# nsp5488/go_raytracer

Measured on AMD Instinct MI355X. Metric: Msamples/sec (pixels×spp/s) + wall-clock, Cornell Box 800×800×1024spp, higher is better.
Workload: dtype f32

## Files before the change

### go_raytracer_amd/__init__.py

```python
import ctypes as C
import weakref

import numpy as np

from . import _lib
from ._lib import (RT_FT_ALL, RT_FT_BOX, RT_NOISE_MARBLE, RT_NOISE_PERLIN,
                   RT_NOISE_TURBULENT, RtAccumInfo, RtAov, RtCamera, RtDenoiseOpts,
                   RtDenoiseVarOpts, RtCameraDerived, RtError, RtRenderOpts, RtSceneInfo, RtStats, RtTreeView,
                   check, lib)

__all__ = ["Tree", "Camera", "Scene", "Accumulator", "quantize", "format_ppm", "device_count", "RtError",
           "tune", "untune", "tuning", "tune_knobs", "tune_from_env",
           "demo_scene", "DEMO_SCENES", "LoadObjOptions", "DefaultLoadOptions", "quantize_device",
           "format_ppm_device", "denoise", "denoise_device", "denoise_var", "denoise_var_device",
           "RtDenoiseVarOpts"]

DEMO_SCENES = ("book1", "book2", "book3", "simple_light", "quads", "cornell", "cornell_smoke",
               "model")


def _d3(v):
    return _lib.D3(*[float(x) for x in v])


# ... 250 lines not shown
        self.MaxDepth = 0
        self.MaxThreads = 0
        self.VerticalFOV = 0.0
        self.DefocusAngle = 0.0
        self.FocusDistance = 0.0
        self.Background = (0.0, 0.0, 0.0)
        self.MaxContribution = 0.0
        self._pos = None
        for k, v in kw.items():
            if k not in self._FIELDS:
                raise AttributeError(k)
            setattr(self, k, v)

    def PositionCamera(self, lookFrom=None, lookAt=None, vup=None):
        self._pos = (tuple(lookFrom) if lookFrom is not None else (0.0, 0.0, 0.0),
                     tuple(lookAt) if lookAt is not None else (0.0, 0.0, -1.0),
                     tuple(vup) if vup is not None else (0.0, 1.0, 0.0))

    def to_c(self):
        c = RtCamera()
        c.aspect_ratio = self.AspectRatio
        c.width = int(self.Width)
        c.samples_per_pixel = int(self.SamplesPerPixel)
        c.max_depth = int(self.MaxDepth)
        c.max_threads = int(self.MaxThreads)
        c.vertical_fov = self.VerticalFOV
        c.defocus_angle = self.DefocusAngle
        c.focus_distance = self.FocusDistance
        c.background = _d3(self.Background)
        c.max_contribution = self.MaxContribution
        if self._pos is not None:
            c.positioned = 1
            c.look_from, c.look_at, c.vup = (_d3(x) for x in self._pos)
        return c

    @classmethod
    def from_c(cls, c):
        cam = cls()
        cam.AspectRatio = c.aspect_ratio
        cam.Width = c.width
        cam.SamplesPerPixel = c.samples_per_pixel
        cam.MaxDepth = c.max_depth
        cam.MaxThreads = c.max_threads
        cam.VerticalFOV = c.vertical_fov
        cam.DefocusAngle = c.defocus_angle
        cam.FocusDistance = c.focus_distance
        cam.Background = tuple(c.background)
        cam.MaxContribution = c.max_contribution
        if c.positioned:
            cam._pos = (tuple(c.look_from), tuple(c.look_at), tuple(c.vup))
        return cam

    def derived(self):
        d = RtCameraDerived()
        c = self.to_c()
        check(lib().rt_camera_derive(C.byref(c), C.byref(d)))
        return d

    def image_size(self):
        d = self.derived()
        return d.width, d.height, d.spp_sqrt

    def Render(self, tree, world, lights, seed=1, device=0):
        with Scene(tree, world, lights) as sc:
            img, _ = sc.render(self, seed=seed, device=device)
        return img


class Scene:

    def __init__(self, tree, world, lights=-1):
        p = C.c_void_p()
        check(lib().rt_scene_create(tree.ptr, world, lights, C.byref(p)))
        self._p = p
        self._destroy = lib().rt_scene_destroy
        self.tree = tree
        self._accums = weakref.WeakSet()

    def close(self):
        if getattr(self, "_p", None):
            for a in list(self._accums):
                a._p = None
            self._destroy(self._p)
            self._p = None

    __del__ = close

    def __enter__(self):
        return self

    def __exit__(self, *a):
        self.close()

    def progress(self):
        d, t = C.c_uint64(0), C.c_uint64(0)
        check(lib().rt_progress(self._p, C.byref(d), C.byref(t)))
        return d.value, t.value

    def info(self):
        i = RtSceneInfo()
        check(lib().rt_scene_info_get(self._p, C.byref(i)))
        return {f: getattr(i, f) for f, _ in RtSceneInfo._fields_}

    def export_bvh(self):
        nn, nr, root = C.c_int32(), C.c_int32(), C.c_uint32()
        check(lib().rt_scene_export_bvh(self._p, None, C.byref(nn), None, C.byref(nr), C.byref(root)))
        nodes = np.zeros((max(nn.value, 0), 16), np.float32)
        refs = np.zeros(max(nr.value, 0), np.uint32)
        check(lib().rt_scene_export_bvh(self._p, nodes.ctypes.data or None, C.byref(nn),
                                        refs.ctypes.data or None, C.byref(nr), C.byref(root)))
        n = C.c_int32()
        check(lib().rt_scene_export_prim_bounds(self._p, None, C.byref(n)))
        bounds = np.zeros((n.value, 6), np.float32)
        check(lib().rt_scene_export_prim_bounds(self._p, bounds.ctypes.data or None, C.byref(n)))
        return nodes, refs, int(root.value), bounds

    def export_bvh8(self):
        nn, nr = C.c_int32(), C.c_int32()
        check(lib().rt_scene_export_bvh8(self._p, None, C.byref(nn), None, C.byref(nr)))
        nodes = np.zeros((max(nn.value, 0), 32), np.uint32)
        refs = np.zeros(max(nr.value, 0), np.uint32)
        check(lib().rt_scene_export_bvh8(self._p, nodes.ctypes.data or None, C.byref(nn),
                                         refs.ctypes.data or None, C.byref(nr)))
        return nodes, refs

    def export_qbvh(self):
        ni, nn, root = C.c_int32(), C.c_int32(), C.c_uint32()
        check(lib().rt_scene_export_qbvh(self._p, None, C.byref(ni), None, C.byref(nn), C.byref(root)))
        items = np.zeros((max(ni.value, 0), 16), np.uint32)
        nodes = np.zeros((max(nn.value, 0), 32), np.uint32)
        check(lib().rt_scene_export_qbvh(self._p, items.ctypes.data or None, C.byref(ni),
                                         nodes.ctypes.data or None, C.byref(nn), C.byref(root)))
        return items, nodes, int(root.value)

    def export_records(self, fill=True):
        ns, sn, nb, counts = C.c_int32(), C.c_int32(), C.c_int32(), (C.c_int32 * 7)()
        check(lib().rt_scene_export_records(self._p, None, C.byref(ns), counts, C.byref(sn), C.byref(nb)))
        pairs = np.zeros((4 * ns.value + sn.value, 4), np.uint32)
        if fill:
            check(lib().rt_scene_export_records(self._p, pairs.ctypes.data or None, C.byref(ns), counts,
                                                C.byref(sn), C.byref(nb)))
        return pairs, ns.value, tuple(counts), sn.value, nb.value

    def lean_light(self):
        k, n = C.c_int32(), C.c_int32()
        check(lib().rt_scene_lean_light(self._p, C.byref(k), None, C.byref(n)))
        block = np.zeros(n.value, np.uint32)
        check(lib().rt_scene_lean_light(self._p, C.byref(k), block.ctypes.data or None, C.byref(n)))
        return k.value, block

    def plan_light(self, device=0):
        k = C.c_int32()
        check(lib().rt_scene_plan_light(self._p, device, C.byref(k)))
        return k.value

    MODES = {"auto": 0, "wavefront": 1, "fused": 2}

    @staticmethod
    def _opts(seed, device, rank, nranks, path_slots, chunk, profile, stream, mode="auto"):
        o = RtRenderOpts()
        o.mode = Scene.MODES[mode]
        o.seed = seed
        o.device = device
        o.rank = rank
        o.nranks = nranks
        o.path_slots = path_slots
        o.chunk = chunk
        o.flags = _lib.RT_FLAG_PROFILE if profile else 0
        o.stream = stream
        return o

    def render(self, camera, seed=1, device=0, rank=0, nranks=1, path_slots=0, chunk=0,
               profile=False, trace=None, mode="auto", progress_slices=0):
        d = camera.derived()
        rows = len(range(rank, d.height, nranks))
        out = np.zeros((rows, d.width, 3), np.float32)
        st = RtStats()
        c = camera.to_c()
        o = self._opts(seed, device, rank, nranks, path_slots, chunk, profile, None, mode)
        o.progress_slices = progress_slices
        tbuf = None
        if trace is not None:
            tbuf = np.zeros((d.max_depth + 1, 12), np.float32)
            o.trace_pixel, o.trace_sample = int(trace[0]), int(trace[1])
            o.trace_cap = tbuf.shape[0]
            o.trace_out = tbuf.ctypes.data
        check(lib().rt_render(self._p, C.byref(c), C.byref(o), out.ctypes.data, C.byref(st)))
        res = {f: getattr(st, f) for f, _ in RtStats._fields_}
        if tbuf is not None:
            res["trace"] = tbuf[tbuf[:, 7] >= 0]
        return out, res

    def render_multi(self, camera, devices, seed=1, path_slots=0, chunk=0, profile=False,
                     mode="auto", rccl=False):
        d = camera.derived()
        out = np.zeros((d.height, d.width, 3), np.float32)
        st = _multi(self, camera, devices, (out.ctypes.data, False), seed, path_slots, chunk,
                    profile, mode, rccl)
        return out, st

    def render_multi_device(self, camera, devices, out_ptr, seed=1, path_slots=0, chunk=0,
                            profile=False, mode="auto", rccl=False):
        return _multi(self, camera, devices, (out_ptr, True), seed, path_slots, chunk, profile,
                      mode, rccl)

    def render_device(self, camera, out_ptr, seed=1, device=0, rank=0, nranks=1, path_slots=0,
                      chunk=0, profile=False, stream=None, mode="auto"):
        st = RtStats()
        c = camera.to_c()
        o = self._opts(seed, device, rank, nranks, path_slots, chunk, profile, stream, mode)
        check(lib().rt_render_device(self._p, C.byref(c), C.byref(o), C.c_void_p(out_ptr),
                                     C.byref(st)))
        return {f: getattr(st, f) for f, _ in RtStats._fields_}

    def render_aov(self, camera, n_samples=1, seed=1, device=0, rank=0, nranks=1):
        d = camera.derived()
        rows = len(range(rank, d.height, nranks))
        res = {"albedo": np.zeros((rows, d.width, 3), np.float32),
               "normal": np.zeros((rows, d.width, 3), np.float32),
               "depth": np.zeros((rows, d.width), np.float32),
               "material": np.full((rows, d.width), -1, np.int32)}
        a = RtAov(*[res[k].ctypes.data for k in ("albedo", "normal", "depth", "material")])
        st = RtStats()
        c = camera.to_c()
        o = self._opts(seed, device, rank, nranks, 0, 0, False, None)
        check(lib().rt_render_aov(self._p, C.byref(c), C.byref(o), n_samples, C.byref(a),
                                  C.byref(st)))
        res["stats"] = {f: getattr(st, f) for f, _ in RtStats._fields_}
        return res

    def render_aov_device(self, camera, albedo=None, normal=None, depth=None, material=None,
                          n_samples=1, seed=1, device=0, rank=0, nranks=1, stream=None):
        a = RtAov(albedo, normal, depth, material)
        st = RtStats()
        c = camera.to_c()
        o = self._opts(seed, device, rank, nranks, 0, 0, False, stream)
        check(lib().rt_render_aov_device(self._p, C.byref(c), C.byref(o), n_samples, C.byref(a),
                                         C.byref(st)))
        return {f: getattr(st, f) for f, _ in RtStats._fields_}

    def accumulator(self, camera, max_passes=0, device=0, rank=0, nranks=1, path_slots=0, chunk=0,
                    profile=False, stream=None, mode="auto", progress_slices=0):
        return Accumulator(self, camera, max_passes, device, rank, nranks, path_slots, chunk,
                           profile, stream, mode, progress_slices)


class Accumulator:

    def __init__(self, scene, camera, max_passes=0, device=0, rank=0, nranks=1, path_slots=0,
                 chunk=0, profile=False, stream=None, mode="auto", progress_slices=0):
        self._p = None
        self._device, self._mean, self._var = device, None, None
        d = camera.derived()
        self.shape = (len(range(rank, d.height, nranks)), d.width)
        c = camera.to_c()
        o = Scene._opts(0, device, rank, nranks, path_slots, chunk, profile, stream, mode)
        o.progress_slices = progress_slices
        p = C.c_void_p()
        check(lib().rt_accum_create(scene._p, C.byref(c), C.byref(o), max_passes, C.byref(p)))
        self._p = p
        self._destroy = lib().rt_accum_destroy
        self.scene = scene
        scene._accums.add(self)

    def close(self):
        if getattr(self, "_p", None):
            self._destroy(self._p)
            self._p = None

    __del__ = close

    def __enter__(self):
        return self

    def __exit__(self, *a):
        self.close()

    def _h(self):
        if not self._p:
            raise ValueError("Accumulator is closed")
        return self._p

    def add(self, seed):
        st = RtStats()
        check(lib().rt_accum_add(self._h(), seed, C.byref(st)))
        return {f: getattr(st, f) for f, _ in RtStats._fields_}

    def resolve(self):
        rgb = np.zeros(self.shape + (3,), np.float32)
        var = np.zeros(self.shape, np.float32)
        check(lib().rt_accum_resolve(self._h(), rgb.ctypes.data, var.ctypes.data))
        return rgb, var

    def resolve_device(self, rgb_tensor, var_tensor=None):
        import torch
        for t, shape in ((rgb_tensor, self.shape + (3,)), (var_tensor, self.shape)):
            if t is not None and (t.dtype != torch.float32 or not t.is_contiguous()
                                  or tuple(t.shape) != shape or not t.is_cuda):
                raise ValueError(f"resolve_device: needs a contiguous float32 device tensor of shape {shape}")
        check(lib().rt_accum_resolve_device(
            self._h(), None if rgb_tensor is None else rgb_tensor.data_ptr(),
            None if var_tensor is None else var_tensor.data_ptr()))

    def denoise_device(self, aov, out=None, var_out=None, **opts):
        import torch
        if self.passes < 2:
# ... 318 lines not shown
```

### go_raytracer_amd/_lib.py

```python
import ctypes as C
import os

_HERE = os.path.dirname(os.path.abspath(__file__))
LIB_PATH = os.environ.get("RT_AMD_LIB") or os.path.join(_HERE, "librt_amd.so")

RT_OK = 0
RT_ERR_INVALID = -1
RT_ERR_UNSUPPORTED = -2
RT_ERR_DEVICE = -3
RT_ERR_OOM = -4
RT_ERR_IO = -5

RT_TEX_SOLID, RT_TEX_CHECKER, RT_TEX_IMAGE, RT_TEX_NOISE = range(4)
RT_NOISE_PERLIN, RT_NOISE_MARBLE, RT_NOISE_TURBULENT = 1, 2, 3
(RT_MAT_LAMBERTIAN, RT_MAT_METAL, RT_MAT_DIELECTRIC, RT_MAT_DIFFUSE_LIGHT,
 RT_MAT_ISOTROPIC) = range(5)
(RT_NODE_LIST, RT_NODE_BVH, RT_NODE_SPHERE, RT_NODE_QUAD, RT_NODE_TRIANGLE,
 RT_NODE_TRANSLATE, RT_NODE_ROTATE_Y, RT_NODE_MEDIUM) = range(8)
RT_FLAG_PROFILE = 1
RT_FLAG_GATHER_RCCL = 2
RT_FT_SPHERE, RT_FT_TRI, RT_FT_METAL, RT_FT_DIEL = 1, 2, 4, 8
RT_FT_MEDIA, RT_FT_CHECKER, RT_FT_IMAGE, RT_FT_NOISE = 16, 32, 64, 128
RT_FT_BOX = 256
RT_FT_ALL = 511
# ... 42 lines not shown
        ("trace_pixel", C.c_int64), ("trace_sample", C.c_int32), ("trace_cap", C.c_int32),
        ("trace_out", C.c_void_p), ("progress_slices", C.c_int32), ("_pad3", C.c_int32),
    ]


class RtStats(C.Structure):
    _fields_ = [
        ("samples", C.c_uint64), ("segments", C.c_uint64),
        ("stack_pushes", C.c_uint64), ("extend_rays", C.c_uint64),
        ("shade_rays", C.c_uint64), ("ms_total", C.c_double),
        ("ms_extend", C.c_double), ("ms_shade", C.c_double),
        ("ms_other", C.c_double), ("n_extend_launches", C.c_int32),
        ("n_shade_launches", C.c_int32), ("iterations", C.c_int32),
        ("rows", C.c_int32), ("mode", C.c_int32), ("path_slots", C.c_int32),
        ("ms_fused", C.c_double),
        ("kernel_features", C.c_int32), ("scene_features", C.c_int32),
        ("tree_width", C.c_int32), ("lds_scene", C.c_int32),
        ("chunk_samples", C.c_int32), ("record_boxes", C.c_int32),
        ("overflow_samples", C.c_uint64),
        ("tuned", C.c_int32), ("chunk_records", C.c_int32),
    ]


class RtAov(C.Structure):
    _fields_ = [("albedo", C.c_void_p), ("normal", C.c_void_p), ("depth", C.c_void_p),
                ("material", C.c_void_p)]


class RtDenoiseOpts(C.Structure):
    _fields_ = [("iterations", C.c_int32), ("demodulate", C.c_int32),
                ("sigma_color", C.c_float), ("sigma_normal", C.c_float),
                ("sigma_depth", C.c_float), ("_pad", C.c_int32)]


class RtDenoiseVarOpts(C.Structure):
    _fields_ = [("iterations", C.c_int32), ("demodulate", C.c_int32),
                ("sigma_lum", C.c_float), ("sigma_normal", C.c_float),
                ("sigma_depth", C.c_float), ("_pad", C.c_int32)]


class RtAccumInfo(C.Structure):
    _fields_ = [("passes", C.c_int32), ("max_passes", C.c_int32),
                ("samples_per_pixel", C.c_uint64), ("nonfinite_pixels", C.c_uint64),
                ("rms_std_error", C.c_double), ("mean_luminance", C.c_double),
                ("rel_error", C.c_double)]


class RtAdaptOpts(C.Structure):
    _fields_ = [("rel_error", C.c_double), ("lum_floor", C.c_double),
                ("tile", C.c_int32), ("min_passes", C.c_int32)]


class RtAdaptInfo(C.Structure):
    _fields_ = [("active_pixels", C.c_uint64), ("total_samples", C.c_uint64),
                ("min_count", C.c_int32), ("max_count", C.c_int32),
                ("n_tiles", C.c_int32), ("active_tiles", C.c_int32)]


class RtTreeView(C.Structure):
    _fields_ = [
        ("nodes", C.c_void_p), ("n_nodes", C.c_int32),
        ("children", C.c_void_p), ("n_children", C.c_int32),
        ("tris", C.c_void_p), ("n_tris", C.c_int32),
        ("materials", C.c_void_p), ("n_materials", C.c_int32),
        ("textures", C.c_void_p), ("n_textures", C.c_int32),
        ("images", C.c_void_p), ("n_images", C.c_int32),
        ("perlins", C.c_void_p), ("n_perlins", C.c_int32),
    ]


class RtObjImage(C.Structure):
    _fields_ = [("name", C.c_char_p), ("rgb", C.c_void_p), ("w", C.c_int32), ("h", C.c_int32)]


class RtObjOptions(C.Structure):
    _fields_ = [
        ("scale_factor", C.c_double), ("flip_yz", C.c_int32), ("debug", C.c_int32),
        ("ignore_normals", C.c_int32), ("center", C.c_int32), ("flip_faces", C.c_int32),
        ("default_material", C.c_int32), ("position", D3), ("ignore_mtl", C.c_int32),
        ("find_windows", C.c_int32), ("n_images", C.c_int32), ("_pad", C.c_int32),
        ("images", C.POINTER(RtObjImage)),
    ]


class RtObjInfo(C.Structure):
    _fields_ = [
        ("n_vertices", C.c_int64), ("n_normals", C.c_int64), ("n_texcoords", C.c_int64),
        ("n_triangles", C.c_int64), ("n_lights", C.c_int64), ("n_materials", C.c_int32),
        ("default_material", C.c_int32), ("bounds_min", D3), ("bounds_max", D3), ("center", D3),
    ]


_P = C.c_void_p
_I = C.c_int
_DP = C.POINTER(C.c_double)

SIGNATURES = {
    "rt_last_error": (C.c_char_p, []),
    "rt_abi_version": (_I, []),
    "rt_tune_set": (_I, [C.c_char_p, C.c_char_p]),
    "rt_tune_get": (_I, [C.c_char_p, C.c_char_p, C.c_int32]),
    "rt_tune_list": (_I, [C.c_int32, C.POINTER(C.c_char_p), C.POINTER(C.c_int32)]),
    "rt_brute_shape": (_I, [C.POINTER(C.c_int32)]),
    "rt_tree_create": (_I, [C.POINTER(_P)]),
    "rt_tree_destroy": (_I, [_P]),
    "rt_tree_seed": (_I, [_P, C.c_uint64]),
    "rt_tree_rand": (C.c_double, [_P]),
    "rt_tree_rand_range": (C.c_double, [_P, C.c_double, C.c_double]),
    "rt_tree_randn": (_I, [_P, _I]),
    "rt_tex_solid": (_I, [_P, C.c_double, C.c_double, C.c_double]),
    "rt_tex_checker": (_I, [_P, C.c_double, _I, _I]),
    "rt_tex_image": (_I, [_P, C.c_void_p, _I, _I]),
    "rt_tex_noise": (_I, [_P, C.c_double, _I]),
    "rt_tex_noise_tables": (_I, [_P, C.c_double, _I, _DP, C.POINTER(C.c_int32)]),
    "rt_mat_lambertian": (_I, [_P, _I]),
    "rt_mat_metal": (_I, [_P, C.c_double, C.c_double, C.c_double, C.c_double]),
    "rt_mat_dielectric": (_I, [_P, C.c_double]),
    "rt_mat_diffuse_light": (_I, [_P, _I]),
    "rt_mat_isotropic": (_I, [_P, _I]),
    "rt_new_list": (_I, [_P]),
    "rt_list_add": (_I, [_P, _I, _I]),
    "rt_build_bvh": (_I, [_P, _I]),
    "rt_new_sphere": (_I, [_P, D3, C.c_double, _I]),
    "rt_new_motion_sphere": (_I, [_P, D3, D3, C.c_double, _I]),
    "rt_new_quad": (_I, [_P, D3, D3, D3, _I]),
    "rt_new_box": (_I, [_P, D3, D3, _I]),
    "rt_new_triangle": (_I, [_P, _DP, _DP, _DP, _I]),
    "rt_new_triangles": (_I, [_P, _I, _DP, _DP, _DP, C.POINTER(C.c_int32)]),
    "rt_translate": (_I, [_P, _I, D3]),
    "rt_rotate_y": (_I, [_P, _I, C.c_double]),
    "rt_constant_medium": (_I, [_P, _I, C.c_double, _I]),
    "rt_obj_default_options": (_I, [C.POINTER(RtObjOptions)]),
    "rt_load_obj": (_I, [_P, C.c_char_p, C.POINTER(RtObjOptions), C.POINTER(_I), C.POINTER(_I),
                         C.POINTER(RtObjInfo)]),
    "rt_load_obj_memory": (_I, [_P, C.c_char_p, C.c_size_t, C.c_char_p, C.c_size_t, C.c_char_p,
                                C.POINTER(RtObjOptions), C.POINTER(_I), C.POINTER(_I),
                                C.POINTER(RtObjInfo)]),
    "rt_tree_get_view": (_I, [_P, C.POINTER(RtTreeView)]),
    "rt_camera_derive": (_I, [C.POINTER(RtCamera), C.POINTER(RtCameraDerived)]),
    "rt_scene_create": (_I, [_P, _I, _I, C.POINTER(_P)]),
    "rt_scene_destroy": (_I, [_P]),
    "rt_scene_info_get": (_I, [_P, C.POINTER(RtSceneInfo)]),
    "rt_scene_export_bvh": (_I, [_P, C.c_void_p, C.POINTER(C.c_int32), C.c_void_p,
                                 C.POINTER(C.c_int32), C.POINTER(C.c_uint32)]),
    "rt_scene_export_bvh8": (_I, [_P, C.c_void_p, C.POINTER(C.c_int32), C.c_void_p,
                                  C.POINTER(C.c_int32)]),
    "rt_scene_export_qbvh": (_I, [_P, C.c_void_p, C.POINTER(C.c_int32), C.c_void_p,
                                  C.POINTER(C.c_int32), C.POINTER(C.c_uint32)]),
    "rt_scene_export_records": (_I, [_P, C.c_void_p, C.POINTER(C.c_int32), C.POINTER(C.c_int32),
                                     C.POINTER(C.c_int32), C.POINTER(C.c_int32)]),
    "rt_scene_export_prim_bounds": (_I, [_P, C.c_void_p, C.POINTER(C.c_int32)]),
    "rt_scene_lean_light": (_I, [_P, C.POINTER(C.c_int32), C.c_void_p, C.POINTER(C.c_int32)]),
    "rt_scene_plan_light": (_I, [_P, _I, C.POINTER(C.c_int32)]),
    "rt_render": (_I, [_P, C.POINTER(RtCamera), C.POINTER(RtRenderOpts), C.c_void_p,
                       C.POINTER(RtStats)]),
    "rt_render_device": (_I, [_P, C.POINTER(RtCamera), C.POINTER(RtRenderOpts), C.c_void_p,
                              C.POINTER(RtStats)]),
    "rt_render_multi": (_I, [_P, C.POINTER(RtCamera), C.POINTER(RtRenderOpts),
                             C.POINTER(C.c_int32), C.c_int32, C.c_void_p, C.POINTER(RtStats)]),
    "rt_render_multi_device": (_I, [_P, C.POINTER(RtCamera), C.POINTER(RtRenderOpts),
                                    C.POINTER(C.c_int32), C.c_int32, C.c_void_p,
                                    C.POINTER(RtStats)]),
    "rt_quantize": (_I, [C.c_void_p, C.c_int64, C.c_void_p]),
    "rt_format_ppm": (C.c_int64, [C.c_void_p, _I, _I, C.c_void_p, C.c_int64]),
    "rt_progress": (_I, [_P, C.POINTER(C.c_uint64), C.POINTER(C.c_uint64)]),
    "rt_quantize_device": (_I, [C.c_void_p, C.c_int64, C.c_void_p, _I, C.c_void_p]),
    "rt_format_ppm_device": (C.c_int64, [C.c_void_p, _I, _I, C.c_void_p, C.c_int64, _I,
                                         C.c_void_p]),
    "rt_render_aov": (_I, [_P, C.POINTER(RtCamera), C.POINTER(RtRenderOpts), C.c_int32,
                           C.POINTER(RtAov), C.POINTER(RtStats)]),
    "rt_render_aov_device": (_I, [_P, C.POINTER(RtCamera), C.POINTER(RtRenderOpts), C.c_int32,
                                  C.POINTER(RtAov), C.POINTER(RtStats)]),
    "rt_denoise": (_I, [C.c_void_p, C.POINTER(RtAov), _I, _I, C.POINTER(RtDenoiseOpts),
                        C.c_void_p]),
    "rt_denoise_device": (_I, [C.c_void_p, C.POINTER(RtAov), _I, _I, C.POINTER(RtDenoiseOpts),
                               C.c_void_p, _I, C.c_void_p]),
    "rt_denoise_var": (_I, [C.c_void_p, C.c_void_p, C.POINTER(RtAov), _I, _I,
                            C.POINTER(RtDenoiseVarOpts), C.c_void_p, C.c_void_p]),
    "rt_denoise_var_device": (_I, [C.c_void_p, C.c_void_p, C.POINTER(RtAov), _I, _I,
                                   C.POINTER(RtDenoiseVarOpts), C.c_void_p, C.c_void_p, _I,
                                   C.c_void_p]),
    "rt_accum_create": (_I, [_P, C.POINTER(RtCamera), C.POINTER(RtRenderOpts), C.c_int32,
                             C.POINTER(_P)]),
    "rt_accum_destroy": (_I, [_P]),
    "rt_accum_reset": (_I, [_P]),
    "rt_accum_add": (_I, [_P, C.c_uint64, C.POINTER(RtStats)]),
    "rt_accum_resolve": (_I, [_P, C.c_void_p, C.c_void_p]),
    "rt_accum_resolve_device": (_I, [_P, C.c_void_p, C.c_void_p]),
    "rt_accum_info_get": (_I, [_P, C.POINTER(RtAccumInfo)]),
    "rt_accum_select": (_I, [_P, C.POINTER(RtAdaptOpts), C.POINTER(C.c_uint64)]),
    "rt_accum_set_active": (_I, [_P, C.c_void_p, C.POINTER(C.c_uint64)]),
    "rt_accum_add_active": (_I, [_P, C.c_uint64, C.POINTER(RtStats)]),
    "rt_accum_counts": (_I, [_P, C.c_void_p]),
    "rt_accum_counts_device": (_I, [_P, C.c_void_p]),
    "rt_accum_tile_error": (_I, [_P, C.POINTER(RtAdaptOpts), C.c_void_p, C.POINTER(C.c_int32),
                                C.POINTER(C.c_int32)]),
    "rt_accum_adapt_info": (_I, [_P, C.POINTER(RtAdaptInfo)]),
    "rt_demo_scene": (_I, [_P, C.c_char_p, C.c_char_p, C.POINTER(RtCamera), C.POINTER(_I),
                           C.POINTER(_I)]),
    "rt_demo_scene_name": (_I, [_I, C.POINTER(C.c_char_p)]),
    "rt_substitute_mesh_obj": (C.c_int64, [_I, _I, C.c_void_p, C.c_int64]),
    "rt_device_count": (_I, []),
}

_lib = None


def lib():
    global _lib
    if _lib is None:
        if not os.path.exists(LIB_PATH):
            raise OSError(f"{LIB_PATH} not built: run `make -C go_raytracer_amd/csrc` "
                          "or __graft_entry__.build()")
        L = C.CDLL(LIB_PATH)
        for name, (res, args) in SIGNATURES.items():
            if os.environ.get("RT_AMD_LIB") and not hasattr(L, name):
                continue
            f = getattr(L, name)
            f.restype = res
            f.argtypes = args
        _lib = L
    return _lib


class RtError(RuntimeError):
    def __init__(self, code, msg):
        super().__init__(f"rt error {code}: {msg}")
        self.code = code


def check(rc):
    if rc < 0:
        raise RtError(rc, lib().rt_last_error().decode(errors="replace"))
    return rc
```

### go_raytracer_amd/csrc/host_records.cpp

```cpp
#include <math.h>
#include <string.h>

#include <algorithm>

#include "rt_internal.h"

namespace rt {

void build_leaf_records(const HostScene& h, std::vector<F4>& recs) {
  recs.assign(4 * h.refs.size(), F4{0, 0, 0, 0});
  for (size_t i = 0; i < h.refs.size(); ++i) make_record(h, h.refs[i], &recs[4 * i]);
}
void build_light_records(const HostScene& h, std::vector<F4>& recs) {
  recs.assign(8 * std::max<size_t>(h.lights.size(), 1), F4{0, 0, 0, 0});
  for (size_t i = 0; i < h.lights.size(); ++i) {
    const uint32_t ref = h.lights[i].ref;
    if (ref == PRIM_NONE || (ref >> 30) != PRIM_QUAD) continue;
    make_record(h, ref, &recs[8 * i]);
    const F4* q = &h.quad[5 * (size_t)(ref & 0x3FFFFFFFu)];
    recs[8 * i + 2].w = q[1].w;
    recs[8 * i + 4] = q[0];
    recs[8 * i + 5] = q[1];
    recs[8 * i + 6] = q[2];
  }
// ... 161 lines not shown
          for (size_t m : quads)
            if (m != i && m != j && !in_box[m] && same_face(m, F, tol)) {
              bool dup = false;
              for (int g = 0; g < f; ++g) dup |= b.face[g] == m;
              if (!dup) { hit = m; break; }
            }
        if (hit == (size_t)-1) ok = false;
        else b.face[f] = hit;
      }
      if (!ok) continue;
      for (int c = 0; c < 3; ++c) b.C[c] = C[c], b.ax[c] = ax[c], b.az[c] = az[c];
      b.H = H;
      for (int f = 0; f < 6; ++f) in_box[b.face[f]] = 1;
      boxes.push_back(b);
      break;
    }
  }
  return boxes;
}

struct Groups {
  std::vector<size_t> grp[7];
  std::vector<std::pair<int, size_t>> odd_ax;
};
Groups group_records(const Records& R, const std::vector<size_t>& ord, const std::vector<char>& in_box) {
  Groups g;
  auto& grp = g.grp;
  auto& odd_ax = g.odd_ax;
  for (size_t i : ord) {
    if (in_box[i]) continue;
    const int a = R.axis_of(i);
    const int v = a < 0 ? R.vert_of(i) : -1;
    grp[a >= 0 ? a : v >= 0 ? 4 + v : 3].push_back(i);
  }
  for (int a : {0, 1, 2, 4, 5, 6})
    if (grp[a].size() & 1) {
      if (a < 3 && tune_int("RT_BRUTE_MIXED", 1) != 0) odd_ax.push_back({a, grp[a].back()});
      else grp[3].push_back(grp[a].back());
      grp[a].pop_back();
    }
  if (odd_ax.size() == 3) {
    grp[3].push_back(odd_ax.back().second);
    odd_ax.pop_back();
  }
  if (odd_ax.size() == 1) {
    grp[3].push_back(odd_ax.back().second);
    odd_ax.clear();
  }
  std::stable_sort(grp[3].begin(), grp[3].end(), [&](size_t a, size_t b) { return R.larger(a, b); });
  return g;
}

struct SlotOrder {
  std::vector<long> slots;
  size_t n_general = 0;
  size_t n_loop = 0;
  size_t nbp = 0;
  size_t face0 = 0;
};
SlotOrder order_slots(const Groups& g, const std::vector<BoxRec>& boxes, BruteCounts& bc) {
  SlotOrder so;
  auto& slots = so.slots;
  for (size_t i : g.grp[3]) slots.push_back((long)i);
  if (slots.size() & 1) slots.push_back(-1);
  bc.ng = (int32_t)(slots.size() / 2);
  for (int a = 0; a < 3; ++a)
    for (size_t i : g.grp[4 + a]) slots.push_back((long)i);
  bc.vy = (int32_t)(g.grp[5].size() / 2);
  so.n_general = slots.size();
  for (int a = 0; a < 3; ++a) {
    for (size_t i : g.grp[a]) slots.push_back((long)i);
    bc.ax[a] = (int32_t)(g.grp[a].size() / 2);
  }
  bc.mx = 0;
  if (g.odd_ax.size() == 2) {
    slots.push_back((long)g.odd_ax[0].second);
    slots.push_back((long)g.odd_ax[1].second);
    bc.mx = (g.odd_ax[0].first + 1) | ((g.odd_ax[1].first + 1) << 2);
  }
  so.n_loop = slots.size();
  so.nbp = (boxes.size() + 1) / 2;
  bc.box = (int32_t)so.nbp;
  slots.insert(slots.end(), 2 * so.nbp, -2);
  so.face0 = slots.size();
  for (const BoxRec& b : boxes)
    for (int f = 0; f < 6; ++f) slots.push_back((long)b.face[f]);
  if (slots.empty()) {
    slots.assign(2, -1);
    bc.ng = 1;
  }
  return so;
}

std::vector<F4> interleave_pairs(const Records& R, const SlotOrder& so, const std::vector<BoxRec>& boxes) {
  const auto& slots = so.slots;
  std::vector<F4> pairs(4 * slots.size(), F4{0, 0, 0, 0});
  for (size_t k = 0; k < 2 * so.nbp; ++k) {
    const BoxRec& b = boxes[std::min(k, boxes.size() - 1)];
    float* f = (float*)&pairs[4 * (so.n_loop + k - (k & 1))] + (k & 1);
    const double a2 = b.ax[0] * b.ax[0] + b.ax[2] * b.ax[2], z2 = b.az[0] * b.az[0] + b.az[2] * b.az[2];
    const double y0 = b.C[1], y1 = b.C[1] + b.H;
    const float v[8] = {(float)b.C[0], (float)b.C[2], (float)(b.ax[0] / a2), (float)(b.ax[2] / a2),
                        (float)(b.az[0] / z2), (float)(b.az[2] / z2), (float)std::min(y0, y1),
                        (float)std::max(y0, y1)};
    for (int e = 0; e < 8; ++e) f[2 * e] = v[e];
    for (int fc = 0; fc < 6; ++fc) {
      const int src = (fc >> 1) == 1 && b.H < 0 ? (fc ^ 1) : fc;
      const uint32_t slot = (uint32_t)(so.face0 + 6 * std::min(k, boxes.size() - 1) + src);
      memcpy(&f[2 * (8 + fc)], &slot, 4);
    }
  }
  for (size_t i = 0; i < slots.size(); ++i) {
    if (slots[i] < 0) continue;
    const F4* r = &R.recs[4 * (size_t)slots[i]];
    float* f = (float*)&pairs[8 * (i / 2)] + (i & 1);
    float kb;
    const uint32_t k = (uint32_t)i;
    memcpy(&kb, &k, 4);
    const int a = i >= so.n_general && i < so.n_loop ? R.axis_of((size_t)slots[i]) : -1;
    const float na = a == 0 ? r[1].x : a == 1 ? r[1].y : r[1].z;
    const float Dp = a < 0 ? r[1].w : na * r[1].w;
    const float v[15] = {r[1].x, r[1].y, r[1].z, Dp,     r[0].x, r[0].y, r[0].z, r[2].x,
                         r[2].y, r[2].z, r[3].x, r[3].y, r[3].z, kb,     r[0].w};
    for (int e = 0; e < 15; ++e) f[2 * e] = v[e];
  }
  return pairs;
}

std::vector<F4> shade_table(const HostScene& h) {
  const size_t nq = h.quad.size() / 5;
  std::vector<F4> tab(2 * nq);
  bool ok = nq > 0;
  for (size_t qi = 0; qi < nq && ok; ++qi) {
    const F4* q = &h.quad[5 * qi];
    uint32_t mb;
    memcpy(&mb, &q[2].w, 4);
    ok = mb < h.mats.size();
    if (!ok) break;
    const DevMaterial& m = h.mats[mb];
    ok = (m.kind == RT_MAT_LAMBERTIAN || m.kind == RT_MAT_DIFFUSE_LIGHT) && m.tex >= 0 &&
         (size_t)m.tex < h.texs.size() && h.texs[m.tex].kind == RT_TEX_SOLID;
    if (!ok) break;
    float kb;
    const uint32_t kind = (uint32_t)m.kind;
    memcpy(&kb, &kind, 4);
    tab[2 * qi] = {q[3].x, q[3].y, q[3].z, kb};
    const F4 col = h.texs[m.tex].color;
    tab[2 * qi + 1] = {col.x, col.y, col.z, q[0].w};
  }
  if (!ok || tune_int("RT_SHADE_LDS", 1) == 0) tab.clear();
  return tab;
}

}

RecordPack pack_records(const HostScene& h) {
  RecordPack out;
  if (!tiny_scene(h)) return out;
  Records R{h, {}, tune_int("RT_BRUTE_AXIS", 1) != 0, tune_int("RT_BRUTE_VERT", 1) != 0};
  build_leaf_records(h, R.recs);
  std::vector<size_t> ord(h.refs.size());
  for (size_t i = 0; i < ord.size(); ++i) ord[i] = i;
  std::stable_sort(ord.begin(), ord.end(), [&](size_t a, size_t b) { return R.larger(a, b); });
  std::vector<char> in_box(h.refs.size(), 0);
  const std::vector<BoxRec> boxes = find_boxes(h, ord, in_box);
  const Groups groups = group_records(R, ord, in_box);
  const SlotOrder so = order_slots(groups, boxes, out.counts);
  out.pairs = interleave_pairs(R, so, boxes);
  out.n_slots = so.slots.size();
  out.n_boxes = (int32_t)boxes.size();
  out.shape = brute_shape_of(out.counts);
  const std::vector<F4> tab = shade_table(h);
  out.shade_n = (int32_t)tab.size();
  out.pairs.insert(out.pairs.end(), tab.begin(), tab.end());
  return out;
}

int32_t scene_merge_ok(const HostScene& h) {
  for (const auto& t : h.texs)
    if (t.kind == RT_TEX_SOLID && !(t.color.x >= 0.0f && t.color.y >= 0.0f && t.color.z >= 0.0f))
      return 0;
  for (const auto& m : h.mats)
    if (m.kind == RT_MAT_METAL && !(m.albedo.x >= 0.0f && m.albedo.y >= 0.0f && m.albedo.z >= 0.0f))
      return 0;
  return 1;
}
float scene_pdf_floor(const HostScene& h) {
  if (h.lights.empty()) return 0.0f;
  for (const auto& e : h.lights)
    if (e.ref == PRIM_NONE) return 0.0f;
  return 1e-30f;
}

int lean_light_of(const HostScene& h, LeanLight* block) {
  if (block) *block = LeanLight{};
  if (pick_ft_set(h.features) != 0u || h.lights.size() != 1) return 0;
  const DevLight& e = h.lights[0];
  if (e.ref == PRIM_NONE || (e.ref >> 30) != PRIM_QUAD || e.weight != 1.0f) return 0;
  if (scene_merge_ok(h) != 1 || scene_pdf_floor(h) != 1e-30f) return 0;
  std::vector<F4> lr;
  build_light_records(h, lr);
  const float n[3] = {lr[1].x, lr[1].y, lr[1].z}, Q[3] = {lr[0].x, lr[0].y, lr[0].z},
              A[3] = {lr[2].x, lr[2].y, lr[2].z}, B[3] = {lr[3].x, lr[3].y, lr[3].z};
  for (int kind = 1; kind < kLeanLightCount; ++kind) {
    const int a = lean_light_axis(kind);
    if (a < 0) continue;
    const int b = (a + 1) % 3, c = (a + 2) % 3;
    if (!((n[a] == 1.0f || n[a] == -1.0f) && n[b] == 0.0f && n[c] == 0.0f && A[a] == 0.0f &&
          B[a] == 0.0f))
      continue;
    if (block) {
      const float f[kLeanLightFloats] = {
          Q[0],    Q[1],    Q[2],    n[a] * lr[1].w, A[0],    A[1],    A[2],    lr[2].w, B[0],    B[1],
          B[2],    0.0f,    lr[5].x, lr[5].y,        lr[5].z, 0.0f,    lr[6].x, lr[6].y, lr[6].z, 0.0f};
      memcpy(block->f, f, sizeof f);
    }
    return kind;
  }
  return 0;
}

}
```

### go_raytracer_amd/csrc/host_tune.cpp

```cpp
#include <errno.h>
#include <stdlib.h>
#include <string.h>

#include <algorithm>
#include <map>
#include <mutex>
#include <string>

#include "rt_internal.h"

namespace rt {
namespace {

struct Knob {
  const char* name;
  bool bits;
  char kind;
  double lo, hi;
};
constexpr double kBig = 1e30;
constexpr Knob kKnobs[] = {
    {"RT_BOX_LEAVES", true, 'i', 0, 1},
    {"RT_BIG_SPHERE_R", true, 'f', 0, kBig},
    {"RT_BVH_BUILDER", false, 's', 0, 0},
    {"RT_BVH_DEVICE_MIN", false, 'f', 0, kBig},
    {"RT_BVH8", false, 'i', 0, 1},
    {"RT_BVH_LEAF", false, 'i', 1, 64},
    {"RT_BVH_CT", false, 'f', 1e-06, 1000000.0},
    {"RT_BVH_CI", false, 'f', 1e-06, 1000000.0},
    {"RT_BVH_TOP", false, 'i', 1, 1073741824},
    {"RT_THREADS", false, 'i', 1, 1024},
    {"RT_FEATURES_ALL", true, 'i', 0, 1},
    {"RT_BRUTE_MAX", true, 'i', 0, 1048576},
    {"RT_BRUTE_AXIS", false, 'i', 0, 1},
    {"RT_BRUTE_VERT", false, 'i', 0, 1},
    {"RT_BRUTE_BOX", true, 'i', 0, 1},
    {"RT_BRUTE_MIXED", false, 'i', 0, 1},
    {"RT_SHADE_LDS", false, 'i', 0, 1},
    {"RT_TREE", true, 'i', -1, 4},
    {"RT_BRUTE_SMEM", false, 'i', -1, 1},
    {"RT_BRUTE_SHAPE", false, 'i', 0, 1},
    {"RT_LEAN_LIGHT", false, 'i', 0, 1},
    {"RT_QBVH", false, 'i', 0, 1},
    {"RT_CHUNK_NEED", false, 'i', 1, 1048576},
    {"RT_TAIL_FRAC", false, 'i', -1, 1024},
    {"RT_TAIL_K", false, 'i', 1, 4096},
    {"RT_CSUM", false, 'i', 0, 1},
    {"RT_CSUM_MAX_MB", false, 'i', 0, 16777216},
    {"RT_CHUNK_ROWS", false, 'i', -1, 1073741824},
    {"RT_SWEEP", false, 's', 0, 0},
    {"RT_STEP_BUDGET", false, 'i', 1, 1073741824},
    {"RT_SHADE_MIN", false, 'i', 1, 64},
    {"RT_GRAB_MIN", false, 'i', 1, 1048576},
    {"RT_SPLIT_MIN", false, 'i', 0, 1048576},
    {"RT_PARTS_LOG2", false, 'i', 0, 6},
    {"RT_GRAN_LOG2", false, 'i', 0, 20},
    {"RT_WAVE_TIMES", false, 's', 0, 0},
    {"RT_TIMING", false, 'i', 0, 1},
};

std::mutex g_mu;
std::map<std::string, std::string> g_set;

const Knob* find_knob(const char* name) {
  for (const Knob& k : kKnobs)
    if (strcmp(k.name, name) == 0) return &k;
  return nullptr;
}

}

bool tune_str(const char* name, std::string* out) {
  std::lock_guard<std::mutex> lk(g_mu);
  auto it = g_set.find(name);
  if (it == g_set.end()) return false;
  if (out) *out = it->second;
  return true;
}

double tune_num(const char* name, double dflt) {
  std::string v;
  if (!tune_str(name, &v) || v.empty()) return dflt;
  return atof(v.c_str());
}

int tune_int(const char* name, int dflt) {
  std::string v;
  if (!tune_str(name, &v) || v.empty()) return dflt;
  return atoi(v.c_str());
}

int32_t tune_count() {
  std::lock_guard<std::mutex> lk(g_mu);
  return (int32_t)g_set.size();
}

}

extern "C" {

int rt_tune_set(const char* name, const char* value) {
  if (!name) {
    std::lock_guard<std::mutex> lk(rt::g_mu);
    rt::g_set.clear();
    return RT_OK;
  }
  const rt::Knob* k = rt::find_knob(name);
  if (!k) return rt::set_error(RT_ERR_INVALID, "rt_tune_set: unknown knob %s", name);
  if (value && k->kind != 's') {
    char* end = nullptr;
    errno = 0;
    const double v = k->kind == 'i' ? (double)strtoll(value, &end, 10) : strtod(value, &end);
    if (end == value || *end != '\0' || errno == ERANGE || !(v >= k->lo && v <= k->hi))
      return rt::set_error(RT_ERR_INVALID, "rt_tune_set: %s=\"%s\" is not a number in [%g, %g]",
                           name, value, k->lo, k->hi);
  }
  if (value && strcmp(name, "RT_BVH_BUILDER") == 0 && strcmp(value, "host") != 0 &&
      strcmp(value, "device") != 0 && strcmp(value, "auto") != 0 && value[0] != '\0')
    return rt::set_error(RT_ERR_INVALID, "rt_tune_set: RT_BVH_BUILDER=\"%s\" (host | device | auto)",
                         value);
  if (value && strcmp(name, "RT_SWEEP") == 0 && strcmp(value, "forward") != 0 &&
      strcmp(value, "reverse") != 0 && value[0] != '\0')
    return rt::set_error(RT_ERR_INVALID, "rt_tune_set: RT_SWEEP=\"%s\" (forward | reverse)", value);
  std::lock_guard<std::mutex> lk(rt::g_mu);
  if (value) rt::g_set[name] = value;
  else rt::g_set.erase(name);
  return RT_OK;
}

int rt_tune_get(const char* name, char* buf, int32_t cap) {
  if (!name || !rt::find_knob(name)) return rt::set_error(RT_ERR_INVALID, "rt_tune_get: unknown knob %s", name ? name : "(null)");
  std::string v;
  if (!rt::tune_str(name, &v)) return 0;
  if (buf && cap > 0) {
    const size_t n = std::min<size_t>(v.size(), (size_t)cap - 1);
    memcpy(buf, v.data(), n);
    buf[n] = '\0';
  }
  return (int)v.size() + 1;
}

int rt_brute_shape(const int32_t counts[7]) {
  if (!counts) return rt::set_error(RT_ERR_INVALID, "rt_brute_shape: counts is NULL");
  const rt::BruteCounts c = {counts[0], counts[1], {counts[2], counts[3], counts[4]}, counts[5], counts[6]};
  return rt::brute_shape_of(c);
}

int rt_scene_lean_light(const rt_scene* sc, int32_t* kind, float* block, int32_t* n_floats) {
  if (!sc) return rt::set_error(RT_ERR_INVALID, "rt_scene_lean_light: null");
  rt::LeanLight b;
  const int k = rt::lean_light_of(sc->s.h, &b);
  if (kind) *kind = k;
  if (n_floats) *n_floats = rt::kLeanLightFloats;
  if (block) memcpy(block, b.f, sizeof b.f);
  return RT_OK;
}

int rt_tune_list(int32_t i, const char** name, int32_t* changes_bits) {
  const int32_t n = (int32_t)(sizeof(rt::kKnobs) / sizeof(rt::kKnobs[0]));
  if (i < 0) return n;
  if (i >= n) return rt::set_error(RT_ERR_INVALID, "rt_tune_list: index %d of %d", i, n);
  if (name) *name = rt::kKnobs[i].name;
  if (changes_bits) *changes_bits = rt::kKnobs[i].bits ? 1 : 0;
  return n;
}

}
```

### go_raytracer_amd/csrc/rt_fused.h

```cpp
#pragma once
#include "rt_path.h"

namespace rt {

RT_D bool stage_nodes(const Params& P, F4* lnodes, int W) {
  const int nl = min(P.sc.n_nodes, 4 * kLdsNodes / W);
  for (int i = threadIdx.x; i < W * nl; i += blockDim.x) lnodes[i] = P.sc.nodes[i];
  const bool recs = P.recs_lds != 0u;
  if (recs) {
    const int n = 4 * P.sc.n_refs + (P.sc.shade_lds >= 0 ? P.sc.shade_n : 0);
    for (int i = threadIdx.x; i < n; i += blockDim.x) lnodes[W * nl + i] = P.sc.leafprims[i];
  }
  __syncthreads();
  return recs;
}

RT_D void record_trace(const Params& P, const Path& s, const Hit& best) {
  if (s.gpix == P.trace_gpix && s.s0 + s.j == P.trace_sample && (int)s.k < P.trace_cap) {
    P.trace[3 * s.k + 0] = {s.o.x, s.o.y, s.o.z, s.time};
    P.trace[3 * s.k + 1] = {s.d.x, s.d.y, s.d.z, (float)s.k};
    P.trace[3 * s.k + 2] = {best.t, best.u, best.v, bitsf(best.ref)};
  }
}

template <uint32_t FT>
RT_D void finish_hit(const Params& P, const Path& s, Hit& best) {
#ifndef RT_NO_TRI_REFINE
  if (HAS(FT_TRI) && best.ref != PRIM_NONE && (best.ref >> 30) == PRIM_TRI)
    refine_tri_hit(P.sc, best.ref & 0x3FFFFFFFu, s.o, s.d, best.t, best.u, best.v);
#endif
#ifdef RT_SPHERE32_LEAVES
  if (HAS(FT_SPHERE) && best.ref != PRIM_NONE && (best.ref >> 30) == PRIM_SPHERE && best.v >= 0.0f)
    refine_sphere_hit(P.sc, best.ref & 0x3FFFFFFFu, s.o, s.d, s.time, best.t);
#endif
#ifdef ABL_NO_MEDIA
  if (false)
#else
  if (HAS(FT_MEDIA) && P.sc.n_media > 0)
#endif
    trace_media(P, s.o, s.d, s.time, 0.001f, s.gpix, s.s0 + s.j, s.k, s.spare, best);
  if (P.trace) record_trace(P, s, best);
}

#ifndef MESH_WAVES
#define MESH_WAVES 4
#endif
#ifndef TRI_WAVES
#define TRI_WAVES 4
#endif
#ifndef TRI_QWAVES
#define TRI_QWAVES 5
#endif
#ifdef RT_QTOP
#ifndef TRI_QSHORT
#define TRI_QSHORT 12
#endif
#ifndef MESH_QSHORT
#define MESH_QSHORT 12
#endif
#endif
#ifndef TRI_QSHORT
#define TRI_QSHORT 13
#endif
#ifndef MESH_QWAVES
#define MESH_QWAVES 5
#endif
#ifndef MESH_QSHORT
#define MESH_QSHORT 13
#endif
#ifndef FT_TEX_WAVES
#define FT_TEX_WAVES 4
#endif
#ifndef BRUTE_WAVES
#define BRUTE_WAVES 6
#endif
constexpr int kBruteWaves = BRUTE_WAVES;
constexpr int fused_waves(uint32_t ft, int tree = 4) {
  return (tree == 0 && ft == 0u) ? kBruteWaves
         : ft == 0u ? 6
         : ft == FT_MEDIA ? 4
         : ft == (FT_SPHERE | FT_TRI | FT_METAL) ? (tree == 5 ? TRI_QWAVES : TRI_WAVES)
         : ft == (FT_SPHERE | FT_TRI | FT_METAL | FT_DIEL | FT_CHECKER) ? (tree == 5 ? MESH_QWAVES : MESH_WAVES)
         : ft == FT_SET_BOOK2 ? FT_TEX_WAVES
                                                                                  : 3;
}
#ifndef MESH_WLDS
#define MESH_WLDS 4
#endif
#ifndef MESH_SHORT
#define MESH_SHORT 16
#endif
#ifndef TRI_SHORT
#define TRI_SHORT MESH_SHORT
#endif
#ifndef TRI_WLDS
#define TRI_WLDS MESH_WLDS
#endif
#ifndef TEX_SHORT
#define TEX_SHORT 10
#endif
#ifndef TEX_WLDS
#define TEX_WLDS 5
#endif
#ifndef ALL_WLDS
#define ALL_WLDS 4
#endif
#ifndef BRUTE_WLDS
#define BRUTE_WLDS kLdsWMax
#endif
constexpr int fused_wlds(uint32_t ft, int tree = 4) {
  return ft == (FT_SPHERE | FT_TRI | FT_METAL | FT_DIEL | FT_CHECKER) ? MESH_WLDS
         : ft == (FT_SPHERE | FT_TRI | FT_METAL)                    ? TRI_WLDS
         : (ft == 0u && tree != 0)                                  ? 4
         : (ft == 0u && tree == 0)                                  ? BRUTE_WLDS
         : ft == FT_ALL                                             ? ALL_WLDS
         : ft == FT_SET_BOOK2 ? TEX_WLDS
                                                                    : kLdsWMax;
}
constexpr int fused_short(uint32_t ft, int tree = 4) {
  return tree == 0                                                    ? 0
         : ft == 0u                                                   ? kShortStackMin
         : ft == (FT_SPHERE | FT_TRI | FT_METAL | FT_DIEL | FT_CHECKER) ? (tree == 5 ? MESH_QSHORT : MESH_SHORT)
         : ft == (FT_SPHERE | FT_TRI | FT_METAL)                      ? (tree == 5 ? TRI_QSHORT : TRI_SHORT)
         : ft == FT_SET_BOOK2 ? TEX_SHORT
                                                                      : kShortStack;
}
constexpr unsigned fused_static_lds(uint32_t ft, int tree = 4) {
  return (unsigned)(fused_short(ft, tree) * 4 + fused_wlds(ft, tree) * 12 + 24) * 256u +
         ((ft & FT_NOISE) ? 256u * 16u + 768u : 0u);
}
__shared__ unsigned long long g_tstart[4];
#ifdef RT_DRAIN_TIMES
__shared__ unsigned long long g_tdrain[4];
__shared__ unsigned long long g_dinfo[4][3];
#endif
template <bool LDS, uint32_t FT, int TREE, int SHAPE = 0, int LIGHT = 0, bool MAP = false>
__global__ __launch_bounds__(256, fused_waves(FT, TREE)) void k_fused(Params P) {
  static_assert(SHAPE == 0 || (LDS && FT == 0u && TREE == 0), "shapes: the lean LDS record loop only");
  static_assert(LIGHT == 0 || (LDS && FT == 0u && TREE == 0), "light kinds: the lean LDS record loop only");
  static_assert(LIGHT >= 0 && LIGHT < kLeanLightCount, "light kinds: unlisted kind");
  extern __shared__ F4 lnodes[];
  __shared__ uint32_t lstack[(fused_short(FT, TREE) > 0 ? fused_short(FT, TREE) : 1) * 256];
  __shared__ float lw[3 * fused_wlds(FT, TREE) * 256];
  __shared__ unsigned long long lacc[3 * 256];
  for (int ch = 0; ch < 3; ++ch) lacc[ch * 256 + threadIdx.x] = 0ull;
  if constexpr (HAS(FT_NOISE)) stage_perlin(P.sc);
  if constexpr (cam_mode(FT) == 1) stage_camera(P);
  const bool recs_lds = LDS && TREE != 8 && stage_nodes(P, lnodes, TREE == 4 ? 8 : 4);
#ifdef RT_QTOP
  if constexpr (TREE == 5) {
    const uint32_t nq = 4u * (uint32_t)min(RT_QTOP, P.sc.n_nodes);
    for (uint32_t i = threadIdx.x; i < nq; i += blockDim.x) st_lds(&lnodes[i], ld_glb(P.sc.nodes + i));
  }
#endif
  if (!LDS) __syncthreads();
  const uint32_t slot = blockIdx.x * blockDim.x + threadIdx.x;
  const TravStack ts = {&lstack[threadIdx.x], P.ostack + slot, P.stack_cols, fused_short(FT, TREE)
#ifdef RT_COUNT_TRAV_OVF
                        , &P.ctr->pushes
#endif
  };
  const WStack ws = {&lw[threadIdx.x], fused_wlds(FT, TREE)};
  const SampleAcc sa = {&lacc[threadIdx.x]};
  Path s;
  s.pushes = 0;
  if constexpr ((FT == 0u && TREE == 0) || kSplitTrees) {
    s.chunk = s.j = 0u;
    s.flags = 0u;
  }
#ifdef RT_WAVE_SEGS
  uint32_t wave_segs = 0;
#else
  s.segs = 0;
#endif
  Trav tr;
  tr.cur = TRAV_DONE;
  bool has = false;
  WaveBatch b = batch_init(P);
  const uint32_t wave_in_group = (FT == 0u && TREE == 0) ? __builtin_amdgcn_readfirstlane(threadIdx.x >> 6)
                                                         : threadIdx.x >> 6;
  if (P.wave_times && lane_id() == 0u) g_tstart[wave_in_group] = wall_clock64();
#ifdef RT_DRAIN_TIMES
  if (lane_id() == 0u) g_tdrain[wave_in_group] = 0ull;
#endif
#ifdef RT_PHASES
  if (threadIdx.x < 4 * PH_N) (&g_ph[0][0])[threadIdx.x] = 0ull;
  __syncthreads();
#endif
  PH_T(t_loop);
  for (;;) {
    PH_T(t_grab);
    uint32_t c = grab_chunk(P, b, !has), j0 = 0u, n0 = 0u;
    constexpr bool kSplit = (FT == 0u && TREE == 0) || kSplitTrees;
    if constexpr (kSplit)
      if (b.part >= (uint32_t)kMaxParts) split_samples(P, s, has, c, j0, n0);
    if (c != 0xFFFFFFFFu) {
      start_sample<false, cam_mode(FT), FT == 0u && TREE == 0, MAP>(P, slot, s, c, j0);
      if constexpr (kSplit)
        if (j0) s.flags = F_SPLIT | (n0 << kCountShift);
      trav_init<FT>(P.sc, s.o, s.d, s.time, tr);
#ifdef RT_QROOT
      if constexpr (TREE == 5) trav_root_q(ts, s.o, 0.001f, tr);
#endif
      has = true;
    }
    PH_ADD(PH_GRAB, t_grab);
#ifdef RT_DRAIN_TIMES
    if (b.part >= (uint32_t)kMaxParts && __builtin_amdgcn_readfirstlane((uint32_t)(g_tdrain[wave_in_group] != 0ull)) == 0u) {
      uint32_t rem = has ? (s.flags >> kCountShift) - s.j : 0u, act = has ? 1u : 0u;
#ifndef RT_WAVE_SEGS
      uint32_t sg = s.segs;
#else
      uint32_t sg = 0u;
#endif
      for (int off = 32; off > 0; off >>= 1) {
        rem += __shfl_xor(rem, off);
        act += __shfl_xor(act, off);
        sg += __shfl_xor(sg, off);
      }
      if (lane_id() == 0u) {
        g_tdrain[wave_in_group] = wall_clock64();
        g_dinfo[wave_in_group][0] = rem;
        g_dinfo[wave_in_group][1] = act;
        g_dinfo[wave_in_group][2] = sg;
      }
    }
#endif
    if (!__any(has)) break;
    PH_T(t_trav);
    if (has && tr.cur != TRAV_DONE)
    {
      PH_CNT(PH_TRAV_LANES, __popcll(__ballot(1)));
      PH_CNT(PH_TRAV_ROUNDS, 1);
      if constexpr (TREE == 0)
        trav_brute<FT, !LDS, SHAPE>(P.sc, lnodes, s.o, s.d, s.time, 0.001f, tr);
      else if constexpr (TREE == 8)
      {
        const int nsteps = trav_steps8<FT>(P.sc, ts, s.o, s.d, s.time, 0.001f, tr, P.step_budget);
#ifdef RT_PHASES
        ph_steps(nsteps);
#endif
        (void)nsteps;
      }
      else
      {
        const int nsteps = trav_steps<LDS, FT, TREE == 4 || TREE == 5, TREE == 5>(
            P.sc, lnodes, recs_lds, ts, s.o, s.d, s.time, 0.001f, tr, P.step_budget);
        retest_near<FT>(P.sc, s.o, s.d, 0.001f, tr);
#ifdef RT_PHASES
        ph_steps(nsteps);
#endif
        (void)nsteps;
      }
    }
    PH_ADD(PH_TRAV, t_trav);
    const bool ready = has && tr.cur == TRAV_DONE;
    const uint32_t n_ready = (uint32_t)__popcll(__ballot(ready));
    const bool busy = __any(has && !ready);
    if (n_ready >= P.shade_min || !busy) {
#ifdef RT_WAVE_SEGS
      wave_segs += n_ready;
#endif

      if (ready) {
        PH_CNT(PH_SHADE_LANES, n_ready);
        PH_CNT(PH_SHADE_ROUNDS, 1);
        PH_T(t_media);
        Hit best = tr.best;
        finish_hit<FT>(P, s, best);
        PH_ADD(PH_MEDIA, t_media);
#ifndef RT_WAVE_SEGS
        ++s.segs;
#endif
        PH_T(t_shade);
        if (shade_core<false, FT, LIGHT>(P, slot, s, best, ws, sa) == OUT_NEED_CHUNK) has = false;
        else {
          trav_init<FT>(P.sc, s.o, s.d, s.time, tr);
#ifdef RT_QROOT
          if constexpr (TREE == 5) trav_root_q(ts, s.o, 0.001f, tr);
#endif
        }
        PH_ADD(PH_SHADE, t_shade);
      }
    }
  }
  PH_ADD(PH_LOOP, t_loop);
#ifdef RT_WAVE_SEGS
  const uint32_t segs = wave_segs;
#else
  uint32_t segs = s.segs;
  for (int off = 32; off > 0; off >>= 1) segs += __shfl_xor(segs, off);
#endif
  uint32_t pushes = s.pushes;
  for (int off = 32; off > 0; off >>= 1) pushes += __shfl_xor(pushes, off);
  if (lane_id() == 0) {
    atomicAdd(&P.ctr->segments, (unsigned long long)segs);
    atomicAdd(&P.ctr->pushes, (unsigned long long)pushes);
    if (P.wave_times) {
      const size_t w = (size_t)blockIdx.x * 4 + wave_in_group;
      unsigned long long* rec = P.wave_times + kWaveRec * w;
      rec[0] = g_tstart[wave_in_group];
      rec[1] = wall_clock64();
      rec[2] = segs;
#ifdef RT_DRAIN_TIMES
      rec[3] = g_tdrain[wave_in_group];
#else
      rec[3] = 0ull;
#endif
#ifdef RT_PHASES
      for (int i = 0; i < PH_N; ++i) rec[4 + i] = g_ph[wave_in_group][i];
#else
      for (int i = 0; i < PH_N; ++i) rec[4 + i] = 0ull;
#ifdef RT_DRAIN_TIMES
      for (int i = 0; i < 3; ++i) rec[4 + i] = g_dinfo[wave_in_group][i];
#endif
#endif
    }
  }
}

#define RT_FUSED_ILP_KERNELS(X)                                             \
  X(true, (FT_SPHERE | FT_TRI | FT_METAL), 4)                               \
  X(false, (FT_SPHERE | FT_TRI | FT_METAL), 4)                              \
  X(true, (FT_SPHERE | FT_TRI | FT_METAL | FT_DIEL | FT_CHECKER), 4)        \
  X(false, (FT_SPHERE | FT_TRI | FT_METAL | FT_DIEL | FT_CHECKER), 4)

#define RT_FUSED_MAP_KERNELS(X)                                                      \
  X(true, kFtSets[0], 0) X(false, kFtSets[0], 0) X(true, kFtSets[1], 0) X(false, kFtSets[1], 0) \
  X(true, kFtSets[0], 4) X(false, kFtSets[0], 4) X(true, kFtSets[1], 4) X(false, kFtSets[1], 4) \
  X(true, kFtSets[2], 4) X(false, kFtSets[2], 4) X(true, kFtSets[3], 4) X(false, kFtSets[3], 4) \
  X(true, kFtSets[4], 4) X(false, kFtSets[4], 4) X(true, FT_ALL, 4) X(false, FT_ALL, 4)         \
  X(false, kFtSets[2], 5) X(false, kFtSets[3], 5) X(false, kFtSets[4], 5) X(false, FT_ALL, 5)

}
```

### go_raytracer_amd/csrc/rt_internal.h

```cpp
#pragma once
#include <stdint.h>

#include <atomic>
#include <map>
#include <memory>
#include <mutex>
#include <string>
#include <vector>

#include "rt_abi.h"
#include "rt_device.h"

namespace rt {

int set_error(int code, const char* fmt, ...);

bool tune_str(const char* name, std::string* out);
double tune_num(const char* name, double dflt);
int tune_int(const char* name, int dflt);
int32_t tune_count();

struct Tree {
  std::vector<rt_node> nodes;
  std::vector<std::vector<int32_t>> lists;
  std::vector<rt_tri> tris;
  std::vector<rt_material> materials;
  std::vector<rt_texture> textures;
  std::vector<std::vector<uint8_t>> image_data;
  std::vector<rt_image> images;
  std::vector<rt_perlin> perlins;
  uint64_t rng = 0x853c49e6748fea9bull;

  bool dirty = true;
  std::vector<rt_node> v_nodes;
  std::vector<int32_t> v_children;

  double rand01();
  int randn(int n);
  void pack();
};

constexpr double kBigSphereR = 256.0;
struct HostScene {
  std::vector<F4> sph_cr, sph_mv;
  std::vector<F2> sph_uv;
  std::vector<F4> quad;
  std::vector<F4> tri;
  std::vector<F4> tri_attr;
  std::vector<F4> box_recs;
  std::vector<F4> nodes;
  std::vector<F4> nodes4;
  uint32_t root4 = PRIM_NONE;
  std::vector<F4> nodes8;
  std::vector<uint32_t> refs8;
  std::vector<uint32_t> refs;
  uint32_t root = PRIM_NONE;
  std::vector<float> prim_bounds;
  std::vector<DevMedium> media;
  std::vector<uint32_t> medium_refs;
  std::vector<uint32_t> big_refs;
  int32_t medium_draws = 0;
  std::vector<DevLight> lights;
  std::vector<DevMaterial> mats;
  std::vector<DevTexture> texs;
  std::vector<uint8_t> texels;
  std::vector<DevImage> images;
  std::vector<DevPerlin> perlins;
  int32_t n_world_prims = 0;
  int32_t bvh_depth = 0;
  int32_t max_leaf = 0;
  int32_t bvh_builder = 0;
  uint32_t features = 0;
  bool noise_table0 = true;
  int32_t tuned = 0;
};

struct DeviceScene;
struct RenderState;

struct Progress {
  std::mutex mu;
  int busy = 0;
  int device = -1;
  uint64_t total = 0;
  uint64_t done = 0;
  std::vector<void*> events;
  std::vector<uint64_t> cum;
};

struct SlotState {
  std::mutex mu;
  RenderState* st = nullptr;
};

struct DeviceSlot {
  std::mutex mu;
  DeviceScene* ds = nullptr;
};

struct Scene {
  HostScene h;
  std::mutex mu;
  std::map<int, DeviceSlot*> devs;
  std::map<std::pair<int, int>, SlotState*> slots;
  std::mutex multi_mu;
  void* multi_buf = nullptr;
  size_t multi_bytes = 0;
  int multi_dev = -1;
  void* rccl = nullptr;
  Progress prog;
  std::vector<rt_accum*> accums;
  std::mutex qb_mu;
  bool qb_built = false;
  std::vector<F4> qb;
  size_t qb_items = 0;
};

int flatten_scene(const Tree& t, int world, int lights, HostScene& out);
int build_bvh(HostScene& s, const std::vector<F4>& lo, const std::vector<F4>& hi,
              const std::vector<uint32_t>& prims);
constexpr size_t kBvh8MinRefs = 1024;
int build_bvh8(HostScene& s);
int build_qbvh(const HostScene& s, const std::vector<F4>& recs, std::vector<F4>* out,
               size_t* n_items);
void make_record(const HostScene& h, uint32_t ref, F4* r);
void build_leaf_records(const HostScene& h, std::vector<F4>& recs);
void build_light_records(const HostScene& h, std::vector<F4>& recs);
std::vector<DevMaterial> materials_with_uv_flag(const HostScene& h);
bool tiny_scene(const HostScene& h);
struct RecordPack {
  std::vector<F4> pairs;
  size_t n_slots = 0;
  int32_t shade_n = 0;
  int32_t n_boxes = 0;
  BruteCounts counts{};
  int shape = 0;
};
RecordPack pack_records(const HostScene& h);
int32_t scene_merge_ok(const HostScene& h);
float scene_pdf_floor(const HostScene& h);
int lean_light_of(const HostScene& h, LeanLight* block);
int build_bvh_device(HostScene& s, const std::vector<F4>& lo, const std::vector<F4>& hi,
                     const std::vector<uint32_t>& prims, int device);
bool bvh_device_available();
constexpr size_t kBoxLeafMinPrims = 256;
uint32_t scene_features(const HostScene& h, bool* noise_table0 = nullptr);
void release_device(Scene* s);
void release_accums(Scene* s);
struct AovView {
  DevScene sc;
  int tree;
};
int aov_view(Scene* s, int device, AovView* out);

}

struct rt_tree {
  rt::Tree t;
};
struct rt_scene {
  rt::Scene s;
};
```

### go_raytracer_amd/csrc/rt_path.h

```cpp
#pragma once
#include "rt_kernels.h"

namespace rt {

constexpr int kLdsNodes = 384;
constexpr int kLdsWMax = 6;
constexpr int kStack = 64;
constexpr int kShortStack = 12;
constexpr int kShortStackMin = 6;
constexpr int kMaxIt = 1 << 16;
constexpr int kXcd = 8;
constexpr int kMaxParts = 64;
constexpr int kPartStride = 64;

enum : uint32_t { F_PEND = 1u, F_PRE = 2u, F_NONFINITE = 4u };
constexpr uint32_t kCountShift = 8;
constexpr uint32_t F_SPLIT = 0x80u;

#ifdef RT_NO_SPLIT_TREES
constexpr bool kSplitTrees = false;
#else
constexpr bool kSplitTrees = true;
#endif
enum { OUT_DEAD = 0, OUT_ALIVE = 1, OUT_NEED_CHUNK = 2 };
// ... 890 lines not shown
  }
}
template <int I> RT_D v2f pair_q(const v4f* r) { return I == 0 ? r[2].xy : I == 1 ? r[2].zw : r[3].xy; }
template <int I> RT_D v2f pair_a(const v4f* r) { return I == 0 ? r[3].zw : I == 1 ? r[4].xy : r[4].zw; }
template <int I> RT_D v2f pair_b(const v4f* r) { return I == 0 ? r[5].xy : I == 1 ? r[5].zw : r[6].xy; }
template <int AX, bool SMEM>
RT_D void brute_axis(const DevScene& sc, const F4* lrec, int p0, int p1, const v2f* O,
                     const v2f* Dv, float tmin, float& best, uint32_t& bk) {
  constexpr int B0 = AX == 0 ? 1 : 0, B1 = AX == 2 ? 1 : 2;
  const float da = Dv[AX].x;
  const float ia = bitsf(pick_by(fbits(rcp(da)), 0x7FC00000u, neg_mask(fabsf(da) - 1e-8f)));
  const v2f inv = {ia, ia};
  for (int p = p0; p < p1; ++p) {
    v4f r[7];
    load_pair<SMEM>(sc, lrec, p, r);
    const uint32_t k0 = __float_as_uint(r[6].z), k1 = __float_as_uint(r[6].w);
    const v2f t = (r[1].zw - O[AX]) * inv;
    const v2f pb = pfma(Dv[B0], t, O[B0]) - pair_q<B0>(r);
    const v2f pc = pfma(Dv[B1], t, O[B1]) - pair_q<B1>(r);
    const v2f a = pfma(pc, pair_a<B1>(r), pb * pair_a<B0>(r));
    const v2f b = pfma(pc, pair_b<B1>(r), pb * pair_b<B0>(r));
    const uint32_t m0 = rec_reject_t(t.x, tmin, best, a.x, b.x);
    best = bitsf(pick_by(fbits(t.x), fbits(best), m0));
    bk = pick_by(k0, bk, m0);
    const uint32_t m1 = rec_reject_t(t.y, tmin, best, a.y, b.y);
    best = bitsf(pick_by(fbits(t.y), fbits(best), m1));
    bk = pick_by(k1, bk, m1);
  }
}
template <int I> RT_D float comp(f3 v) { return I == 0 ? v.x : I == 1 ? v.y : v.z; }
template <int A, int H>
RT_D void brute_half(const v4f* r, f3 o, f3 d, float tmin, float& best, uint32_t& bk) {
  constexpr int B0 = A == 0 ? 1 : 0, B1 = A == 2 ? 1 : 2;
  const float da = comp<A>(d);
  const float ia = bitsf(pick_by(fbits(rcp(da)), 0x7FC00000u, neg_mask(fabsf(da) - 1e-8f)));
  const float t = ((H ? r[1].w : r[1].z) - comp<A>(o)) * ia;
  const float pb = fmaf(comp<B0>(d), t, comp<B0>(o)) - (H ? pair_q<B0>(r).y : pair_q<B0>(r).x);
  const float pc = fmaf(comp<B1>(d), t, comp<B1>(o)) - (H ? pair_q<B1>(r).y : pair_q<B1>(r).x);
  const float a = fmaf(pc, H ? pair_a<B1>(r).y : pair_a<B1>(r).x, pb * (H ? pair_a<B0>(r).y : pair_a<B0>(r).x));
  const float b = fmaf(pc, H ? pair_b<B1>(r).y : pair_b<B1>(r).x, pb * (H ? pair_b<B0>(r).y : pair_b<B0>(r).x));
  const uint32_t m = rec_reject_t(t, tmin, best, a, b);
  best = bitsf(pick_by(fbits(t), fbits(best), m));
  bk = pick_by(__float_as_uint(H ? r[6].w : r[6].z), bk, m);
}
template <int A0, int A1, bool SMEM>
RT_D void brute_mixed(const DevScene& sc, const F4* lrec, int p, f3 o, f3 d, float tmin,
                      float& best, uint32_t& bk) {
  v4f r[7];
  load_pair<SMEM>(sc, lrec, p, r);
  brute_half<A0, 0>(r, o, d, tmin, best, bk);
  brute_half<A1, 1>(r, o, d, tmin, best, bk);
}
template <int I> RT_D v2f pair_n(const v4f* r) { return I == 0 ? r[0].xy : I == 1 ? r[0].zw : r[1].xy; }
template <int AX, bool SMEM>
RT_D void brute_vert(const DevScene& sc, const F4* lrec, int p0, int p1, const v2f* O,
                     const v2f* Dv, float tmin, float& best, uint32_t& bk) {
  constexpr int B0 = AX == 0 ? 1 : 0, B1 = AX == 2 ? 1 : 2;
  for (int p = p0; p < p1; ++p) {
    v4f r[7];
    load_pair<SMEM>(sc, lrec, p, r);
    const uint32_t k0 = __float_as_uint(r[6].z), k1 = __float_as_uint(r[6].w);
    const v2f D = r[1].zw;
    const v2f den = pfma(pair_n<B1>(r), Dv[B1], pair_n<B0>(r) * Dv[B0]);
    const v2f num = D - pfma(pair_n<B1>(r), O[B1], pair_n<B0>(r) * O[B0]);
    const v2f t = num * v2f{rcp(den.x), rcp(den.y)};
    const v2f pa = pfma(Dv[AX], t, O[AX]) - pair_q<AX>(r);
    const v2f p0v = pfma(Dv[B0], t, O[B0]) - pair_q<B0>(r);
    const v2f p1v = pfma(Dv[B1], t, O[B1]) - pair_q<B1>(r);
    const v2f a = pfma(p1v, pair_a<B1>(r), p0v * pair_a<B0>(r));
    const v2f b = pa * pair_b<AX>(r);
    const uint32_t m0 = rec_reject(den.x, t.x, tmin, best, a.x, b.x);
    best = bitsf(pick_by(fbits(t.x), fbits(best), m0));
    bk = pick_by(k0, bk, m0);
    const uint32_t m1 = rec_reject(den.y, t.y, tmin, best, a.y, b.y);
    best = bitsf(pick_by(fbits(t.y), fbits(best), m1));
    bk = pick_by(k1, bk, m1);
  }
}
constexpr uint32_t kBoxCode = 0x40000000u;
template <bool SMEM>
RT_D void brute_box(const DevScene& sc, const F4* lrec, int p0, int p1, const v2f* O,
                    const v2f* Dv, float iy1, float tmin, float& best, uint32_t& bk) {
  const v2f iy = {iy1, iy1};
  for (int p = p0; p < p1; ++p) {
    v4f r[4];
    if (SMEM) {
      typedef __attribute__((address_space(4))) const v4f cst_v4;
      const cst_v4* q = (const cst_v4*)sc.leafprims + 8 * __builtin_amdgcn_readfirstlane(p);
#pragma unroll
      for (int e = 0; e < 4; ++e) r[e] = q[e];
    } else {
      const lds_v4* q = (const lds_v4*)lrec + 8 * p;
#pragma unroll
      for (int e = 0; e < 4; ++e) r[e] = q[e];
    }
    const v2f ex = O[0] - r[0].xy, ez = O[2] - r[0].zw;
    const v2f lx = pfma(ez, r[1].zw, ex * r[1].xy), lz = pfma(ez, r[2].zw, ex * r[2].xy);
    const v2f vx = pfma(Dv[2], r[1].zw, Dv[0] * r[1].xy), vz = pfma(Dv[2], r[2].zw, Dv[0] * r[2].xy);
    const v2f ix = {rcp(vx.x), rcp(vx.y)}, iz = {rcp(vz.x), rcp(vz.y)};
    const v2f tx0 = -lx * ix, tx1 = pfma(-lx, ix, ix);
    const v2f tz0 = -lz * iz, tz1 = pfma(-lz, iz, iz);
    const v2f ty0 = (r[3].xy - O[1]) * iy, ty1 = (r[3].zw - O[1]) * iy;
#pragma unroll
    for (int h = 0; h < 2; ++h) {
      const float ax0 = h ? tx0.y : tx0.x, ax1 = h ? tx1.y : tx1.x;
      const float ay0 = h ? ty0.y : ty0.x, ay1 = h ? ty1.y : ty1.x;
      const float az0 = h ? tz0.y : tz0.x, az1 = h ? tz1.y : tz1.x;
      const float tn = fmaxf(fmaxf(fminf(ax0, ax1), fminf(ay0, ay1)), fminf(az0, az1));
      const float tf = fminf(fminf(fmaxf(ax0, ax1), fmaxf(ay0, ay1)), fmaxf(az0, az1));
      const uint32_t leave = neg_mask(tn - tmin);
      const float t = bitsf(pick_by(fbits(tn), fbits(tf), leave));
      const uint32_t rej = (uint32_t)((int32_t)__builtin_amdgcn_bitop3_b32(
                               fbits(tf - tn), fbits(t - tmin), fbits(best - t), 0xFE) >> 31);
      best = bitsf(pick_by(fbits(t), fbits(best), rej));
      bk = pick_by(kBoxCode | ((uint32_t)p << 2) | ((uint32_t)h << 1) | (leave & 1u), bk, rej);
    }
  }
}
template <bool SMEM>
RT_D uint32_t box_face(const DevScene& sc, const F4* lrec, uint32_t code, f3 o, f3 d, float iy,
                       float best) {
  const uint32_t base = 32u * ((code & ~kBoxCode) >> 2) + ((code >> 1) & 1u);
  float f[8];
  if (SMEM) {
    const float* g = (const float*)sc.leafprims + base;
#pragma unroll
    for (int e = 0; e < 8; ++e) f[e] = *(const __attribute__((address_space(1))) float*)(g + 2 * e);
  } else {
    const lds_f32* l = (const lds_f32*)lrec + base;
#pragma unroll
    for (int e = 0; e < 8; ++e) f[e] = l[2 * e];
  }
  const float ex = o.x - f[0], ez = o.z - f[1];
  const float lx = fmaf(ez, f[3], ex * f[2]), lz = fmaf(ez, f[5], ex * f[4]);
  const float ix = rcp(fmaf(d.z, f[3], d.x * f[2])), iz = rcp(fmaf(d.z, f[5], d.x * f[4]));
  const float t[6] = {-lx * ix, fmaf(-lx, ix, ix), (f[6] - o.y) * iy, (f[7] - o.y) * iy,
                      -lz * iz, fmaf(-lz, iz, iz)};
  const uint32_t flip = (code & 1u) ? 0xFFFFFFFFu : 0u;
  uint32_t slot = 0u;
  float err = kInf;
#pragma unroll
  for (int a = 0; a < 3; ++a) {
    const uint32_t m = neg_mask(t[2 * a + 1] - t[2 * a]) ^ flip;
    const float e = fminf(fabsf(bitsf(pick_by(fbits(t[2 * a]), fbits(t[2 * a + 1]), m)) - best), kInf);
    const uint32_t nearer = neg_mask(e - err);
    slot = pick_by(slot, 2u * (uint32_t)a + (m & 1u), nearer);
    err = bitsf(pick_by(fbits(err), fbits(e), nearer));
  }
  if (SMEM)
    return *(const __attribute__((address_space(1))) uint32_t*)((const float*)sc.leafprims + base +
                                                                 2 * (8 + slot));
  return ((const lds_u32*)lrec)[base + 2 * (8 + slot)];
}
template <uint32_t FT, bool SMEM, int SHAPE = 0>
RT_D void trav_brute(const DevScene& sc, const F4* lrec, f3 o, f3 d, float time, float tmin,
                     Trav& tr) {
  static_assert(!HAS(FT_SPHERE | FT_TRI), "record loop: quad-only feature sets");
  static_assert(SHAPE >= 0 && SHAPE < kBruteShapeCount, "record loop: unlisted shape");
  const cst_params* kp = SHAPE == 0 ? kparams() : nullptr;
  BruteCounts bc = brute_shape(SHAPE);
  if constexpr (SHAPE == 0) {
    bc.ax[0] = kp->sc.brute_ax[0], bc.ax[1] = kp->sc.brute_ax[1], bc.ax[2] = kp->sc.brute_ax[2];
    bc.vy = kp->sc.brute_vt[1];
    bc.ng = kp->sc.brute_ng;
  }
  const int nax = bc.ax[0], nay = bc.ax[1], naz = bc.ax[2];
  const int nvy = bc.vy;
  const int ng = bc.ng;
  const v2f ox = {o.x, o.x}, oy = {o.y, o.y}, oz = {o.z, o.z};
  const v2f dx = {d.x, d.x}, dy = {d.y, d.y}, dz = {d.z, d.z};
  float best = tr.best.t;
  uint32_t bk = 0xFFFFFFFFu;
  for (int p = 0; p < ng; ++p) {
    v4f r[7];
    load_pair<SMEM>(sc, lrec, p, r);
    const uint32_t k0 = __float_as_uint(r[6].z), k1 = __float_as_uint(r[6].w);
    const v2f nx = r[0].xy, ny = r[0].zw, nz = r[1].xy, D = r[1].zw;
    const v2f den = pfma(nz, dz, pfma(ny, dy, nx * dx));
    const v2f num = D - pfma(nz, oz, pfma(ny, oy, nx * ox));
    const v2f t = num * v2f{rcp(den.x), rcp(den.y)};
    const v2f px = pfma(dx, t, ox) - r[2].xy;
    const v2f py = pfma(dy, t, oy) - r[2].zw;
    const v2f pz = pfma(dz, t, oz) - r[3].xy;
    const v2f a = pfma(pz, r[4].zw, pfma(py, r[4].xy, px * r[3].zw));
    const v2f b = pfma(pz, r[6].xy, pfma(py, r[5].zw, px * r[5].xy));
    const uint32_t m0 = rec_reject(den.x, t.x, tmin, best, a.x, b.x);
    best = bitsf(pick_by(fbits(t.x), fbits(best), m0));
    bk = pick_by(k0, bk, m0);
    const uint32_t m1 = rec_reject(den.y, t.y, tmin, best, a.y, b.y);
    best = bitsf(pick_by(fbits(t.y), fbits(best), m1));
    bk = pick_by(k1, bk, m1);
  }
  const v2f O[3] = {ox, oy, oz}, Dv[3] = {dx, dy, dz};
  const int q = ng + nvy;
  brute_vert<1, SMEM>(sc, lrec, ng, q, O, Dv, tmin, best, bk);
  brute_axis<0, SMEM>(sc, lrec, q, q + nax, O, Dv, tmin, best, bk);
  brute_axis<1, SMEM>(sc, lrec, q + nax, q + nax + nay, O, Dv, tmin, best, bk);
  brute_axis<2, SMEM>(sc, lrec, q + nax + nay, q + nax + nay + naz, O, Dv, tmin, best, bk);
  const int qm = q + nax + nay + naz, mx = SHAPE == 0 ? kp->sc.brute_mx : bc.mx;
  if (mx == (1 | (2 << 2))) brute_mixed<0, 1, SMEM>(sc, lrec, qm, o, d, tmin, best, bk);
  else if (mx == (1 | (3 << 2))) brute_mixed<0, 2, SMEM>(sc, lrec, qm, o, d, tmin, best, bk);
  else if (mx == (2 | (3 << 2))) brute_mixed<1, 2, SMEM>(sc, lrec, qm, o, d, tmin, best, bk);
  const int qb = qm + (mx != 0 ? 1 : 0);
  const float iy = rcp(d.y);
  brute_box<SMEM>(sc, lrec, qb, qb + (SHAPE == 0 ? kp->sc.brute_box : bc.box), O, Dv, iy, tmin, best, bk);
  if (bk != 0xFFFFFFFFu) {
    if (bk & kBoxCode) bk = box_face<SMEM>(sc, lrec, bk, o, d, iy, best);
    const uint32_t base = 32u * (bk >> 1) + (bk & 1u);
    float f[10];
    if (SMEM) {
      const float* g = (const float*)sc.leafprims + base + 8;
#pragma unroll
      for (int e = 0; e < 10; ++e)
        f[e] = *(const __attribute__((address_space(1))) float*)(g + 2 * e + (e == 9 ? 2 : 0));
    } else {
      const lds_f32* l = (const lds_f32*)lrec + base + 8;
#pragma unroll
      for (int e = 0; e < 10; ++e) f[e] = l[2 * e + (e == 9 ? 2 : 0)];
    }
    const float px = fmaf(d.x, best, o.x) - f[0];
    const float py = fmaf(d.y, best, o.y) - f[1];
    const float pz = fmaf(d.z, best, o.z) - f[2];
    tr.best.t = best;
    tr.best.u = fmaf(pz, f[5], fmaf(py, f[4], px * f[3]));
    tr.best.v = fmaf(pz, f[8], fmaf(py, f[7], px * f[6]));
    tr.best.ref = __float_as_uint(f[9]);
  }
  tr.cur = TRAV_DONE;
}

template <bool LDS, uint32_t FT>
RT_D void trace_world(const DevScene& sc, const F4* lnodes, bool recs_lds, const TravStack& stack,
                      f3 o, f3 d, float time, float tmin, Hit& best) {
  Trav tr;
  trav_init<FT>(sc, o, d, time, tr);
  do {
    trav_steps<LDS, FT>(sc, lnodes, recs_lds, stack, o, d, time, tmin, tr, 0x7FFFFFFF);
    retest_near<FT>(sc, o, d, tmin, tr);
  } while (tr.cur != TRAV_DONE);
  best = tr.best;
}

RT_D bool boundary_hit(const DevScene& sc, const DevMedium& m, f3 o, f3 d, float time, double lo,
                       double hi, double& t_out) {
  bool any = false;
  double best = hi;
  for (uint32_t k = 0; k < m.bcount; ++k) {
    double t;
    if (hit_prim_d(sc, sc.medium_refs[m.bfirst + k], o, d, time, lo, best, t)) {
      any = true;
      best = t;
    }
  }
  t_out = best;
  return any;
}

RT_D void trace_media(const Params& P, f3 o, f3 d, float time, float tmin, uint32_t gpix,
                      uint32_t sample, uint32_t vertex, uint32_t spare, Hit& best) {
  const DevScene& sc = P.sc;
  rt_u32x4 r = {{0, 0, 0, 0}};
  int cached_group = -1;
  const float ray_len = length(d);
  for (int mi = 0; mi < sc.n_media; ++mi) {
    static_assert(sizeof(DevMedium) == 32, "DevMedium: two 16-B scalar loads");
    const F4* mr = (const F4*)(sc.media + __builtin_amdgcn_readfirstlane(mi));
    const F4 ma = ld_cst(mr), mb = ld_cst(mr + 1);
    DevMedium m;
    m.bfirst = fbits(ma.x);
    m.bcount = fbits(ma.y);
    m.neg_inv_density = ma.z;
    m.phase_mat = (int32_t)fbits(ma.w);
    m.draw_base = (int32_t)fbits(mb.x);
    m.mult = (int32_t)fbits(mb.y);
    float hd = kInf;
    for (int k = 0; k < m.mult; ++k) {
      int draw = m.draw_base + k;
      float u;
      if (draw == sc.medium_draws - 1) {
        u = rt_unit_f(spare);
      } else {
        int group = 1 + (draw >> 2);
        if (group != cached_group) {
          r = rt_rng_draw(P.seed, gpix, sample, RT_STREAM(vertex, group));
          cached_group = group;
        }
        u = rt_unit_f(r.v[draw & 3]);
      }
      hd = fminf(hd, m.neg_inv_density * logf(u));
    }
    const float hd_t = hd / ray_len;
#ifndef RT_NO_MEDIA_SKIP
    if (!(hd_t < best.t)) continue;
#endif
    double t1, t2;
    typedef __attribute__((address_space(4))) const uint32_t cst_u32;
    const uint32_t b0 = m.bcount == 1 ? *(const cst_u32*)(sc.medium_refs + m.bfirst) : PRIM_NONE;
    if ((b0 >> 30) == PRIM_SPHERE && b0 != PRIM_NONE) {
      double r0, r1;
      const uint32_t bi = b0 & 0x3FFFFFFFu;
      if (!sphere_roots_cm(ld_cst(sc.sph_cr + bi), ld_cst(sc.sph_mv + bi), o, d, time, r0, r1))
        continue;
      t1 = r0;
      if (!(t1 + 0.0001 < r1 && r1 < (double)kInf)) continue;
      t2 = r1;
    } else {
      if (!boundary_hit(sc, m, o, d, time, -(double)kInf, (double)kInf, t1)) continue;
      if (!boundary_hit(sc, m, o, d, time, t1 + 0.0001, (double)kInf, t2)) continue;
    }
    t1 = fmax(t1, (double)tmin);
    if (t1 >= t2) continue;
    t1 = fmax(0.0, t1);
    double inside = (t2 - t1) * (double)ray_len;
    if ((double)hd > inside) continue;
    float tm = (float)(t1 + (double)hd_t);
    if (tm < best.t) {
      best.t = tm;
      best.u = 0.0f;
      best.v = 0.0f;
      best.ref = prim_ref(PRIM_MEDIUM, (uint32_t)mi);
    }
  }
}

__shared__ DevPerlin g_perlin;

RT_D void stage_perlin(const DevScene& sc) {
  if (sc.n_perlins <= 0) return;
  const F4* src = (const F4*)sc.perlins;
  F4* dst = (F4*)&g_perlin;
  for (int i = threadIdx.x; i < (int)(sizeof(DevPerlin) / 16); i += blockDim.x) dst[i] = src[i];
}

typedef __attribute__((address_space(3))) const DevPerlin* LdsPerlin;
template <typename PL>
RT_D float perlin_noise(PL pl, f3 p) {
  float fx = floorf(p.x), fy = floorf(p.y), fz = floorf(p.z);
  float u = p.x - fx, v = p.y - fy, w = p.z - fz;
  int i = (int)fx, j = (int)fy, k = (int)fz;
  float uu = u * u * (3 - 2 * u), vv = v * v * (3 - 2 * v), ww = w * w * (3 - 2 * w);
  const int pi[2] = {pl->perm[0][i & 255], pl->perm[0][(i + 1) & 255]},
            pj[2] = {pl->perm[1][j & 255], pl->perm[1][(j + 1) & 255]},
            pk[2] = {pl->perm[2][k & 255], pl->perm[2][(k + 1) & 255]};
  const float wx[2] = {1 - uu, uu}, wy[2] = {1 - vv, vv}, wz[2] = {1 - ww, ww};
  float accum = 0.0f;
  for (int di = 0; di < 2; ++di)
    for (int dj = 0; dj < 2; ++dj)
      for (int dk = 0; dk < 2; ++dk) {
        const int gi = pi[di] ^ pj[dj] ^ pk[dk];
        const F4 g = {pl->ranvec[gi].x, pl->ranvec[gi].y, pl->ranvec[gi].z, 0.0f};
        f3 wt = mk3(u - (float)di, v - (float)dj, w - (float)dk);
        accum += wx[di] * wy[dj] * wz[dk] * dot(xyz(g), wt);
      }
  return accum;
}
template <typename PL>
RT_D float perlin_turb(PL pl, f3 p, int depth) {
  float accum = 0.0f, weight = 1.0f;
#pragma unroll 1
  for (int i = 0; i < depth; ++i) {
    accum += weight * perlin_noise(pl, p);
    weight *= 0.5f;
    p = p * 2.0f;
  }
  return fabsf(accum);
}

template <uint32_t FT>
RT_D f3 tex_value(const DevScene& sc, int tex, float u, float v, f3 p) {
#ifdef ABL_NO_TEX
  return xyz(sc.texs[tex].color);
#endif
  for (int guard = 0; guard < 64; ++guard) {
    const DevTexture T = sc.texs[tex];
    if (!HAS(FT_CHECKER | FT_IMAGE | FT_NOISE) || T.kind == RT_TEX_SOLID) return xyz(T.color);
    if (HAS(FT_CHECKER) && T.kind == RT_TEX_CHECKER) {
      float inv = T.color.w;
      int x = (int)floorf(inv * p.x), y = (int)floorf(inv * p.y), z = (int)floorf(inv * p.z);
      tex = ((x + y + z) % 2 == 0) ? T.a : T.b;
      continue;
    }
// ... 301 lines not shown
  else s.pre = v;
}

struct WStack {
  float* lds;
  int nlds;
  RT_D void put(const Params& P, uint32_t slot, uint32_t k, F4 v) const {
    if ((int)k < nlds) {
      lds_f32* q = (lds_f32*)lds + k * 256;
      q[0] = v.x;
      q[nlds * 256] = v.y;
      q[2 * nlds * 256] = v.z;
    } else {
      st_glb(hbm_entry(P, slot, k), v);
    }
  }
  RT_D f3 mul(const Params& P, uint32_t slot, uint32_t k, f3 w) const {
    f3 r;
    if ((int)k < nlds) {
      lds_f32* q = (lds_f32*)lds + k * 256;
      r = mk3(q[0] * w.x, q[nlds * 256] * w.y, q[2 * nlds * 256] * w.z);
      q[0] = r.x;
      q[nlds * 256] = r.y;
      q[2 * nlds * 256] = r.z;
    } else {
      F4* e = hbm_entry(P, slot, k);
      const F4 v = ld_glb(e);
      r = mk3(v.x * w.x, v.y * w.y, v.z * w.z);
      st_glb(e, {r.x, r.y, r.z, 0.0f});
    }
    return r;
  }
  RT_D F4* hbm_entry(const Params& P, uint32_t slot, uint32_t k) const {
    const cst_params* kp = kparams();
#ifdef WSTACK_SLOT_MAJOR
    return kp->stack + ((size_t)slot * (kp->max_depth + 1) + (k - nlds));
#else
    return kp->stack + ((size_t)(k - nlds) * kp->P + slot);
#endif
  }
  RT_D size_t hbm_index(const Params& P, uint32_t slot, uint32_t k) const {
#ifdef WSTACK_SLOT_MAJOR
    return (size_t)slot * (P.max_depth + 1) + (k - nlds);
#else
    return (size_t)(k - nlds) * P.P + slot;
#endif
  }
  RT_D void fold_max(const Params& P, uint32_t slot, uint32_t nst, f3& v, float& maxI) const {
    int k = (int)nst - 1;
#ifndef RT_FOLD_ONE_LOAD
    for (; k - 1 >= nlds; k -= 2) {
      const F4 a = ld_glb(hbm_entry(P, slot, (uint32_t)k));
      const F4 b = ld_glb(hbm_entry(P, slot, (uint32_t)(k - 1)));
      v = xyz(a) * v;
      maxI = fmaxf(maxI, v.x + v.y + v.z);
      v = xyz(b) * v;
      maxI = fmaxf(maxI, v.x + v.y + v.z);
    }
#endif
    for (; k >= nlds; --k) {
      v = xyz(ld_glb(hbm_entry(P, slot, (uint32_t)k))) * v;
      maxI = fmaxf(maxI, v.x + v.y + v.z);
    }
    if (nlds > 0 && nst > 0) {
      const lds_f32* q = (const lds_f32*)lds;
      f3 e[kLdsWMax];
#pragma unroll
      for (int i = 0; i < kLdsWMax; ++i)
        if (i < nlds)
          e[i] = mk3(q[i * 256], q[(nlds + i) * 256], q[(2 * nlds + i) * 256]);
#pragma unroll
      for (int i = kLdsWMax - 1; i >= 0; --i)
        if (i < nlds && i < (int)nst) {
          v = e[i] * v;
          maxI = fmaxf(maxI, v.x + v.y + v.z);
        }
    }
  }
  RT_D f3 fold(const Params& P, uint32_t slot, uint32_t nst, f3 L) const {
    for (int k = (int)nst - 1; k >= nlds; --k)
      L = clamp_contribution(xyz(ld_glb(hbm_entry(P, slot, (uint32_t)k))) * L, P.maxc);
    if (nlds > 0 && nst > 0) {
      const lds_f32* q = (const lds_f32*)lds;
      f3 e[kLdsWMax];
#pragma unroll
      for (int i = 0; i < kLdsWMax; ++i)
        if (i < nlds)
          e[i] = mk3(q[i * 256], q[(nlds + i) * 256], q[(2 * nlds + i) * 256]);
#pragma unroll
      for (int i = kLdsWMax - 1; i >= 0; --i)
        if (i < nlds && i < (int)nst) L = clamp_contribution(e[i] * L, P.maxc);
    }
    return L;
  }
};

template <bool SOA>
RT_D void store_ray(const Params& P, uint32_t slot, const Path& s) {
  if (SOA) {
    P.ray_o[slot] = {s.o.x, s.o.y, s.o.z, s.time};
    P.ray_d[slot] = {s.d.x, s.d.y, s.d.z, bitsf(s.spare)};
    P.path[slot] = make_uint2(s.chunk, pack_path(s.j, s.k, s.nst, s.flags));
  }
}

RT_D void load_path(const Params& P, uint32_t slot, Path& s) {
  const F4 ro = P.ray_o[slot], rd = P.ray_d[slot];
  const uint2 ps = P.path[slot];
  s.o = xyz(ro);
  s.time = ro.w;
  s.d = xyz(rd);
  s.spare = fbits(rd.w);
  s.chunk = ps.x;
  const Ids id = chunk_ids(P, s.chunk);
  s.gpix = id.gpix;
  s.s0 = id.sample0;
  s.j = ps.y & 0xFFFu;
  s.k = (ps.y >> 12) & 0xFFu;
  s.nst = (ps.y >> 20) & 0xFFu;
  s.flags = (ps.y >> 28) | (id.count << kCountShift);
}

template <bool SOA, int CAM = 0>
RT_D void next_sample(const Params& P, uint32_t slot, Path& s, uint32_t j, const rt_u32x4& r) {
  Ids id;
  id.gpix = s.gpix;
  id.row = fdiv(s.gpix, P.fd_width);
  id.col = s.gpix - id.row * (uint32_t)P.width;
  camera_ray_r<CAM>(P, id, s.s0 + j, r, s.o, s.d, s.time);
  s.spare = rt_spare24(r);
  s.j = j;
  s.k = 0;
  s.nst = 0;
  s.flags &= ~(F_SPLIT - 1u);
  store_ray<SOA>(P, slot, s);
}

template <bool SOA, int CAM = 0, bool ONE = false, bool MAP = false>
RT_D void start_sample(const Params& P, uint32_t slot, Path& s, uint32_t chunk, uint32_t j) {
  Ids id = chunk_ids<ONE, MAP>(P, chunk);
  const rt_u32x4 r = rt_rng_draw(P.seed, id.gpix, id.sample0 + j, RT_STREAM_CAMERA);
  camera_ray_r<CAM>(P, id, id.sample0 + j, r, s.o, s.d, s.time);
  s.spare = rt_spare24(r);
  s.chunk = chunk;
  s.gpix = id.gpix;
  s.s0 = id.sample0;
  s.j = j;
  s.k = 0;
  s.nst = 0;
  s.flags = id.count << kCountShift;
  store_ray<SOA>(P, slot, s);
}

template <bool SOA, uint32_t FT, int LIGHT = 0>
RT_D int shade_core(const Params& P, uint32_t slot, Path& s, const Hit& h, const WStack& ws,
                    const SampleAcc& sa) {
  const DevScene& sc = P.sc;
  const f3 o = s.o, d = s.d;
  const float time = s.time;
  const uint32_t ref = h.ref;
  f3 lterm = mk3(0, 0, 0);
  bool term = false;
  rt_u32x4 rcam;
  bool have_rcam = false;
  f3 p = mk3(0, 0, 0), n = mk3(0, 0, 0);
  float u = h.u, v = h.v;
  bool ff = true;
  DevMaterial M;
  bool scat = false;
  bool ltab = false;
  f3 lcol = mk3(0, 0, 0);
  float eta = 0.0f;
  if (ref != PRIM_NONE) {
    const float t = h.t;
    p = o + d * t;
    const uint32_t type = ref >> 30, idx = ref & 0x3FFFFFFFu;
    f3 nout;
    int mat;
    if (HAS(FT_SPHERE) && type == PRIM_SPHERE) {
      const F4 cr = sc.sph_cr[idx], mv = sc.sph_mv[idx];
      f3 cc = xyz(cr) + xyz(mv) * time;
      {
        const double cx = (double)cr.x + (double)time * (double)mv.x;
        const double cy = (double)cr.y + (double)time * (double)mv.y;
        const double cz = (double)cr.z + (double)time * (double)mv.z;
        const double ex = (double)p.x - cx, ey = (double)p.y - cy, ez = (double)p.z - cz;
        const double rr = (double)cr.w;
        const float dn = (float)(rr * rr - (ex * ex + ey * ey + ez * ez));
        const f3 e = p - cc;
        const float le = length(e);
        const f3 nu = e * rcp(le);
        p = p + nu * (dn * rcp(fabsf(cr.w) + le));
        nout = cr.w < 0.0f ? -nu : nu;
        eta = 0x1p-22f * (fabsf(p.x * nu.x) + fabsf(p.y * nu.y) + fabsf(p.z * nu.z));
      }
      mat = (int)fbits(mv.w);
      ff = dot(d, nout) < 0;
      n = ff ? nout : -nout;
      if (HAS(FT_IMAGE) && sc.mats[mat]._pad != 0.0f) {
        const F2 rs = sc.sph_uv[idx];
        f3 no = mk3(rs.x * nout.x - rs.y * nout.z, nout.y, rs.y * nout.x + rs.x * nout.z);
        float theta = acosf(-no.y);
        float phi = atan2f(-no.z, no.x) + kPi;
        u = phi * (0.5f * kInvPi);
        v = theta * kInvPi;
      }
    } else if (FT == 0u && sc.shade_lds >= 0) {
      const F4* tab = g_dyn_lds + sc.shade_lds + 2 * idx;
      const F4 a = ld_lds(tab), b = ld_lds(tab + 1);
      lcol = xyz(b);
      nout = xyz(a);
#ifndef RT_NO_LEAN_SNAP
      p = p - nout * (dot(nout, p) - b.w);
#endif
      mat = (int)fbits(a.w);
      ltab = true;
      ff = dot(d, nout) < 0;
      n = ff ? nout : -nout;
    } else if (!HAS(FT_TRI | FT_MEDIA) || type == PRIM_QUAD) {
      const F4* q = sc.quad + 5 * (size_t)idx;
      nout = xyz(q[3]);
      p = p - nout * (dot(nout, p) - q[0].w);
      mat = (int)fbits(q[2].w);
      ff = dot(d, nout) < 0;
      n = ff ? nout : -nout;
      if (HAS(FT_BOX) && u < 0.0f) {
        if (HAS(FT_IMAGE) && sc.mats[mat]._pad != 0.0f) {
          const f3 pp = p - xyz(q[0]), w = xyz(q[4]);
          u = dot(w, cross(pp, xyz(q[2])));
          v = dot(w, cross(xyz(q[1]), pp));
        } else {
          u = v = 0.0f;
        }
      }
    } else if (HAS(FT_TRI) && (!HAS(FT_MEDIA) || type == PRIM_TRI)) {
      nout = tri_normal(sc, idx, u, v);
      mat = (int)fbits(sc.tri[3 * (size_t)idx].w);
      ff = dot(d, nout) < 0;
      n = ff ? nout : -nout;
      uint32_t tf = fbits(sc.tri[3 * (size_t)idx + 2].w);
      if (tf & TRI_HAS_UV) {
        const F4* at = sc.tri_attr + 6 * (size_t)idx;
        float w = 1.0f - u - v;
        float tu = w * at[4].x + u * at[4].z + v * at[5].x;
        float tv = w * at[4].y + u * at[4].w + v * at[5].y;
        u = tu;
        v = tv;
      }
    } else {
      mat = sc.media[idx].phase_mat;
      n = mk3(1, 0, 0);
      ff = true;
      u = v = 0.0f;
    }
    if (ltab)
      M.kind = mat;
    else
      M = sc.mats[mat];
    scat = M.kind != RT_MAT_DIFFUSE_LIGHT;
  }
  constexpr bool kMergeDraws = FT != FT_ALL;
  rt_u32x4 r;
  if (kMergeDraws)
    r = rt_rng_draw(P.seed, s.gpix, s.s0 + s.j + (scat ? 0u : 1u),
                    scat ? RT_STREAM(s.k, 0) : RT_STREAM_CAMERA);
  if (!scat) {
    if (ref == PRIM_NONE)
      lterm = mk3(P.bg[0], P.bg[1], P.bg[2]);
    else
      lterm = ff ? (ltab ? lcol : tex_value<FT>(sc, M.tex, u, v, p)) : mk3(0, 0, 0);
    term = true;
    if (kMergeDraws) {
      rcam = r;
      have_rcam = true;
    }
  } else {
    if (!kMergeDraws) r = rt_rng_draw(P.seed, s.gpix, s.s0 + s.j, RT_STREAM(s.k, 0));
    {
      f3 ndir;
      bool clamp_vertex = false;
      f3 weight;
      if (HAS(FT_METAL) && M.kind == RT_MAT_METAL) {
        f3 refl = unit(reflect(d, n));
        ndir = refl + uniform_sphere(rt_unit_f(r.v[2]), rt_unit_f(r.v[3])) * M.param;
        weight = xyz(M.albedo);
      } else if (HAS(FT_DIEL) && M.kind == RT_MAT_DIELECTRIC) {
        float ior = M.param;
        float ri = ff ? rcp(ior) : ior;
        f3 ud = unit(d);
        float cs = fminf(dot(-ud, n), 1.0f);
        float sn = fsqrt(1.0f - cs * cs);
        bool cannot = ri * sn > 1.0f;
        bool refl = cannot;
        if (!cannot) {
          float r0 = (1.0f - ior) * rcp(1.0f + ior);
          r0 = r0 * r0;
          const float x = 1.0f - cs, x2 = x * x;
          float refl_p = r0 + (1.0f - r0) * (x2 * x2 * x);
          refl = refl_p > rt_unit_f(r.v[0]);
        }
        ndir = refl ? reflect(ud, n) : refract(ud, n, ri);
        weight = mk3(1, 1, 1);
      } else {
        const bool iso = HAS(FT_MEDIA) && M.kind == RT_MAT_ISOTROPIC;
        PH_T(t_tex);
        f3 att = ltab ? lcol : tex_value<FT>(sc, M.tex, u, v, p);
        PH_ADD(PH_TEX, t_tex);
        PH_T(t_light);
        LeanLightRegs lean;
        if constexpr (LIGHT != 0) lean = lean_light_load();
        Onb b;
        if (!iso) b = make_onb_unit(n);
        if (rt_unit_f(r.v[0]) < 0.5f) {
          if constexpr (LIGHT != 0) ndir = lean_light_random(lean, p, r);
          else ndir = lights_random<FT>(sc, p, r);
        } else if (iso) {
          ndir = uniform_sphere(rt_unit_f(r.v[2]), rt_unit_f(r.v[3]));
        } else {
          ndir = onb_transform(b, cosine_direction(rt_unit_f(r.v[2]), rt_unit_f(r.v[3])));
        }
        float bsdf_pdf, spdf;
        if (iso) {
          bsdf_pdf = 1.0f / (4.0f * kPi);
          spdf = 1.0f / (4.0f * kPi);
        } else {
          f3 ud = unit(ndir);
          bsdf_pdf = fmaxf(0.0f, dot(ud, b.w) * kInvPi);
          float ct = dot(n, ud);
          spdf = fmaxf(0.0f, ct * kInvPi);
        }
#ifdef ABL_NO_LIGHTPDF
        float pdf = 0.5f * 0.01f + 0.5f * bsdf_pdf;
#else
        float lpdf;
        if constexpr (LIGHT != 0) lpdf = lean_light_pdf<LIGHT>(lean, p, ndir);
        else lpdf = lights_pdf<FT>(sc, p, ndir);
        float pdf = 0.5f * lpdf + 0.5f * bsdf_pdf;
#endif
        PH_ADD(PH_LIGHT, t_light);
        weight = (att * spdf) * rcp(fmaxf(pdf, LIGHT != 0 ? 1e-30f : sc.pdf_floor));
        clamp_vertex = true;
      }
      if (clamp_vertex) {
        if (s.flags & F_PEND) {
          const f3 pv = get_pend<SOA>(P, slot, s);
#ifndef RT_NO_WEIGHT_MERGE
          const bool merge = (LIGHT != 0 || kparams()->sc.merge_ok) && s.nst > 0 && pv.x >= 0.0f && pv.y >= 0.0f &&
                             pv.z >= 0.0f && pv.x <= 1.0f && pv.y <= 1.0f && pv.z <= 1.0f;
#else
          const bool merge = false;
#endif
          if (merge) {
            f3 top = ws.mul(P, slot, s.nst - 1, pv);
            if (HAS(FT_MEDIA))
              while (s.nst >= 2 && top.x >= 0.0f && top.y >= 0.0f && top.z >= 0.0f &&
                     top.x <= 1.0f && top.y <= 1.0f && top.z <= 1.0f) {
                top = ws.mul(P, slot, s.nst - 2, top);
                --s.nst;
              }
          } else {
            ws.put(P, slot, s.nst, {pv.x, pv.y, pv.z, 0.0f});
            ++s.nst;
#ifdef RT_COUNT_PUSHES
            ++s.pushes;
#elif defined(RT_COUNT_HBM_PUSHES)
            if ((int)s.nst > ws.nlds) ++s.pushes;
#endif
          }
        }
        set_pend<SOA>(P, slot, s, weight);
        s.flags |= F_PEND;
      } else if (s.flags & F_PEND) {
        set_pend<SOA>(P, slot, s, get_pend<SOA>(P, slot, s) * weight);
      } else {
        f3 w = (s.flags & F_PRE) ? get_pre<SOA>(P, slot, s) : mk3(1, 1, 1);
        set_pre<SOA>(P, slot, s, w * weight);
        s.flags |= F_PRE;
      }
      if (!finite3(weight)) s.flags |= F_NONFINITE;
      ++s.k;
      if ((int)s.k > P.max_depth) {
        term = true;
        lterm = mk3(0, 0, 0);
      } else {
        if (HAS(FT_SPHERE)) p = p + n * copysignf(eta, dot(ndir, n));
        s.o = p;
        s.d = ndir;
        s.spare = rt_spare24(r);
        store_ray<SOA>(P, slot, s);
        return OUT_ALIVE;
      }
    }
  }
  PH_T(t_term);
  f3 L = lterm;
  const bool zero = lterm.x == 0.0f && lterm.y == 0.0f && lterm.z == 0.0f;
  if (!(zero && !(s.flags & F_NONFINITE))) {
#ifdef RT_FOLD_STEPWISE
    if (s.flags & F_PEND) L = clamp_contribution(get_pend<SOA>(P, slot, s) * L, P.maxc);
    L = ws.fold(P, slot, s.nst, L);
#elif !defined(ABL_NO_FOLD)
    float maxI = 0.0f;
    if (s.flags & F_PEND) {
      L = get_pend<SOA>(P, slot, s) * L;
      maxI = L.x + L.y + L.z;
      ws.fold_max(P, slot, s.nst, L, maxI);
    }
    L = L * fminf(1.0f, P.maxc * rcp(maxI));
#endif
    if (s.flags & F_PRE) L = get_pre<SOA>(P, slot, s) * L;
  } else {
    L = mk3(0, 0, 0);
  }
#ifdef RT_NAN_DEBUG
  if (isnan(L.x) || isnan(L.y) || isnan(L.z)) printf("NAN gpix %u sample %u\n", s.gpix, s.s0 + s.j);
#endif
// ... 121 lines not shown
```

### go_raytracer_amd/csrc/rt_render.hip

```cpp
#include <hip/hip_runtime.h>
#include <math.h>
#include <stddef.h>
#include <stdio.h>
#include <stdlib.h>
#include <string.h>

#include <algorithm>
#include <chrono>
#include <string>
#include <thread>
#include <vector>

#include <rccl/rccl.h>

#include "rt_hip_util.h"
#include "rt_path.h"
#include "rt_fused.h"
#include "rt_resolve.h"

namespace rt {

RT_D uint32_t queue_slot(const Params& P, const uint32_t* q, const uint32_t* cnt, uint32_t i) {
  uint32_t x = 0;
  while (x + 1 < (uint32_t)kXcd && i >= cnt[x]) {
    i -= cnt[x];
    ++x;
  }
  return q[(size_t)x * P.P + i];
}

template <bool LDS>
__global__ __launch_bounds__(256) void k_extend(Params P, int it) {
  __shared__ F4 lnodes[LDS ? 4 * kLdsNodes : 4];
  __shared__ uint32_t lstack[kShortStack * 256];
  const bool recs_lds = LDS && stage_nodes(P, lnodes, 8);
  const uint32_t gtid = blockIdx.x * blockDim.x + threadIdx.x;
  const TravStack ts = {&lstack[threadIdx.x], P.ostack + gtid, P.stack_cols, kShortStack};
  const uint32_t sel = (uint32_t)it & 1u;
  uint32_t cnt[kXcd];
  uint32_t n = 0;
  for (int x = 0; x < kXcd; ++x) {
    cnt[x] = P.ctr->cnt[it % kMaxIt][x];
    n += cnt[x];
  }
  const uint32_t* q = P.queue[sel];
  const uint32_t stride = gridDim.x * blockDim.x;
  for (uint32_t i = blockIdx.x * blockDim.x + threadIdx.x; i < n; i += stride) {
    const uint32_t slot = queue_slot(P, q, cnt, i);
    Path s;
    load_path(P, slot, s);
    Hit best;
    trace_world<LDS, FT_ALL>(P.sc, lnodes, recs_lds, ts, s.o, s.d, s.time, 0.001f, best);
    finish_hit<FT_ALL>(P, s, best);
    P.hit[slot] = {best.t, best.u, best.v, bitsf(best.ref)};
  }
  if (blockIdx.x == 0 && threadIdx.x == 0) atomicAdd(&P.ctr->segments, (unsigned long long)n);
}

__global__ __launch_bounds__(256) void k_shade(Params P, int it) {
  __shared__ uint32_t wave_cnt[4], wave_base[4], block_base;
  stage_perlin(P.sc);
  __syncthreads();
  const uint32_t sel = (uint32_t)it & 1u;
  uint32_t cnt[kXcd];
  uint32_t n = 0;
  for (int x = 0; x < kXcd; ++x) {
    cnt[x] = P.ctr->cnt[it % kMaxIt][x];
    n += cnt[x];
  }
  const uint32_t i = blockIdx.x * blockDim.x + threadIdx.x;
  const bool active = i < n;
  const uint32_t slot = active ? queue_slot(P, P.queue[sel], cnt, i) : 0u;
  bool alive = false;
  if (active) {
    Path s;
    load_path(P, slot, s);
    const F4 hv = P.hit[slot];
    const Hit h = {hv.x, hv.y, hv.z, fbits(hv.w)};
    const WStack ws = {nullptr, 0};
    const SampleAcc sa = {nullptr};
    int out = shade_core<true, FT_ALL>(P, slot, s, h, ws, sa);
    if (out == OUT_NEED_CHUNK) {
      const uint32_t c = s.chunk + P.P;
      if (c < P.n_chunks) {
        start_sample<true>(P, slot, s, c, 0);
        out = OUT_ALIVE;
      }
    }
    alive = out == OUT_ALIVE;
  }
  const unsigned long long am = __ballot(alive);
  const uint32_t w = threadIdx.x >> 6, lane = lane_id();
  if (lane == 0) wave_cnt[w] = (uint32_t)__popcll(am);
  __syncthreads();
  if (threadIdx.x == 0) {
    uint32_t tot = 0;
    for (int k = 0; k < 4; ++k) {
      wave_base[k] = tot;
      tot += wave_cnt[k];
    }
    const uint32_t x = blockIdx.x % kXcd;
    block_base = tot ? atomicAdd(&P.ctr->cnt[(it + 1) % kMaxIt][x], tot) : 0u;
  }
  __syncthreads();
  if (alive) {
    const uint32_t x = blockIdx.x % kXcd;
    P.queue[sel ^ 1u][(size_t)x * P.P + block_base + wave_base[w] + prefix_count(am)] = slot;
  }
}

__global__ __launch_bounds__(256) void k_init(Params P) {
  const uint32_t slot = blockIdx.x * blockDim.x + threadIdx.x;
  if (slot >= P.P) return;
  if (slot < P.n_chunks) {
    Path s;
    start_sample<true>(P, slot, s, slot, 0);
    P.queue[0][slot] = slot;
  }
  if (slot == 0) {
    P.ctr->cnt[0][0] = min(P.P, P.n_chunks);
    P.ctr->chunk_head = P.P;
  }
}

__global__ __launch_bounds__(256) void k_resolve(Params P, float* out, double scale) {
  const uint32_t lp = blockIdx.x * blockDim.x + threadIdx.x;
  if (lp >= P.npix) return;
  const uint32_t f = P.pflags[lp];
  unsigned long long cs[3] = {0ull, 0ull, 0ull};
  chunk_record_sums(P, lp, cs);
  for (int ch = 0; ch < 3; ++ch) {
    const bool nan = (f & (1u << ch)) != 0, pinf = (f & (8u << ch)) != 0,
               ninf = (f & (64u << ch)) != 0;
    float v;
    if (nan || (pinf && ninf)) {
      v = __builtin_nanf("");
    } else if (pinf || ninf) {
      v = pinf ? kInf : -kInf;
    } else {
      const size_t i = (size_t)ch * P.npix + lp;
      const long long sum = (long long)(P.accum[i] + cs[ch]);
      v = (float)(((double)sum * 2.3283064365386963e-10 + P.side[i]) * scale);
    }
    out[3 * (size_t)lp + ch] = v;
  }
}

struct DeviceScene {
  int device = -1;
  std::vector<void*> allocs;
  DevScene d{};
  const F4* nodes2 = nullptr;
  const F4* brute_pairs = nullptr;
  size_t brute_slots = 0;
  int32_t shade_n = 0;
  int32_t brute_boxes = 0;
  int brute_shape = 0;
  int lean_light = 0;
  LeanLight light_block{};
  uint32_t root2 = PRIM_NONE;
  int32_t n_nodes2 = 0;
  const F4* qnodes = nullptr;
  size_t qitems = 0;
  std::mutex qmu;
  bool q_done = false;
  ~DeviceScene() {
    for (void* p : allocs) (void)hipFree(p);
  }
};

struct RenderState {
  int device = -1;
  uint32_t P = 0;
  int depth_cap = 0;
  uint32_t npix = 0;
  hipStream_t own_stream = nullptr;
  std::vector<void*> allocs;
  F4 *ray_o = nullptr, *ray_d = nullptr, *hit = nullptr, *pend = nullptr, *pre = nullptr,
     *stack = nullptr;
  uint2* path = nullptr;
  uint32_t* queue[2] = {nullptr, nullptr};
  Counters* ctr = nullptr;
  unsigned long long* accum = nullptr;
  unsigned long long* csum = nullptr;
  size_t csum_chunks = 0;
  double* side = nullptr;
  uint32_t* pflags = nullptr;
  uint32_t* ostack = nullptr;
  uint32_t ostack_cols = 0;
  float* out = nullptr;
  uint32_t out_cap = 0;
  std::vector<hipEvent_t> events;
  std::vector<hipEvent_t> prog_events;
  int resident_blocks = 0;
  void free_all() {
    for (void* p : allocs) (void)hipFree(p);
    allocs.clear();
  }
  ~RenderState() {
    free_all();
    for (auto e : events) (void)hipEventDestroy(e);
    for (auto e : prog_events) (void)hipEventDestroy(e);
    if (own_stream) (void)hipStreamDestroy(own_stream);
  }
};

struct RcclGather {
  std::vector<int> devs;
  std::vector<ncclComm_t> comms;
  std::vector<hipStream_t> streams;
  std::vector<float*> send;
  size_t send_floats = 0;
  void release() {
    for (size_t i = 0; i < comms.size(); ++i) {
      (void)hipSetDevice(devs[i]);
      if (send.size() > i && send[i]) (void)hipFree(send[i]);
      if (streams.size() > i && streams[i]) (void)hipStreamDestroy(streams[i]);
      (void)ncclCommDestroy(comms[i]);
    }
    devs.clear();
    comms.clear();
    streams.clear();
    send.clear();
    send_floats = 0;
  }
};

void release_device(Scene* s) {
  DeviceGuard dg;
  release_accums(s);
  if (s->rccl) {
    static_cast<RcclGather*>(s->rccl)->release();
    delete static_cast<RcclGather*>(s->rccl);
    s->rccl = nullptr;
  }
  std::lock_guard<std::mutex> lk(s->mu);
  for (auto& kv : s->slots) {
    if (kv.second->st) {
      (void)hipSetDevice(kv.first.first);
      delete kv.second->st;
    }
    delete kv.second;
  }
  s->slots.clear();
  for (auto& kv : s->devs) {
    if (kv.second->ds) {
      (void)hipSetDevice(kv.first);
      delete kv.second->ds;
    }
    delete kv.second;
  }
  s->devs.clear();
  if (s->multi_buf) {
    (void)hipSetDevice(s->multi_dev);
    (void)hipFree(s->multi_buf);
    s->multi_buf = nullptr;
  }
}

template <typename T>
static int upload(DeviceScene* ds, const std::vector<T>& v, const T** out) {
  *out = nullptr;
  if (v.empty()) return RT_OK;
  void* p = nullptr;
  HIP_OK(hipMalloc(&p, v.size() * sizeof(T)));
  ds->allocs.push_back(p);
  HIP_OK(hipMemcpy(p, v.data(), v.size() * sizeof(T), hipMemcpyHostToDevice));
  *out = (const T*)p;
  return RT_OK;
}

static int env_int(const char* name, int dflt) { return tune_int(name, dflt); }


FastDiv make_fastdiv(uint32_t d) {
  FastDiv f{1u, 0u, 0u, d};
  if (d <= 1) return f;
  const uint32_t l = 32u - (uint32_t)__builtin_clz(d - 1u);
  f.m = (uint32_t)((((uint64_t)1 << 32) * (((uint64_t)1 << l) - d)) / d + 1u);
  f.s1 = 1u;
  f.s2 = l - 1u;
  return f;
}

static int upload_scene(const Scene* s, DeviceScene* ds);
static int ensure_scene(Scene* s, int device, DeviceScene** out) {
  DeviceSlot* slot;
  {
    std::lock_guard<std::mutex> lk(s->mu);
    DeviceSlot*& sl = s->devs[device];
    if (!sl) sl = new DeviceSlot();
    slot = sl;
  }
  std::lock_guard<std::mutex> up(slot->mu);
  if (slot->ds) {
    *out = slot->ds;
    return RT_OK;
  }
  DeviceScene* ds = new DeviceScene();
  ds->device = device;
  const auto t0 = std::chrono::steady_clock::now();
  const int rc = upload_scene(s, ds);
  if (tune_int("RT_TIMING", 0))
    fprintf(stderr, "[rt] scene upload to device %d %.3f s\n", device,
            std::chrono::duration<double>(std::chrono::steady_clock::now() - t0).count());
  if (rc != RT_OK) {
    delete ds;
    return rc;
  }
  slot->ds = ds;
  *out = ds;
  return RT_OK;
}
static int upload_scene(const Scene* s, DeviceScene* ds) {
  const HostScene& h = s->h;
  DevScene& d = ds->d;
  const std::vector<DevMaterial> mats = materials_with_uv_flag(h);
  int rc;
#define UP(vec, field)                                      \
  if ((rc = upload(ds, vec, &d.field)) != RT_OK) return rc;
  UP(h.sph_cr, sph_cr);
  UP(h.sph_mv, sph_mv);
  UP(h.sph_uv, sph_uv);
  UP(h.quad, quad);
  UP(h.tri, tri);
  UP(h.tri_attr, tri_attr);
  std::vector<F4> recs;
  build_leaf_records(h, recs);
  {
    std::vector<F4> tree_buf(h.nodes4);
    tree_buf.resize((tree_buf.size() + 15) / 16 * 16, F4{0, 0, 0, 0});
    const size_t rec0 = tree_buf.size();
    if ((rec0 + recs.size()) * sizeof(F4) >= ((size_t)1 << 32))
      return set_error(RT_ERR_UNSUPPORTED, "scene: BVH nodes + leaf records exceed 4 GiB");
    tree_buf.insert(tree_buf.end(), recs.begin(), recs.end());
    const F4* base = nullptr;
    if ((rc = upload(ds, tree_buf, &base)) != RT_OK) return rc;
    d.nodes = base;
    d.leafprims = base ? base + rec0 : nullptr;
  }
  const bool small = tiny_scene(h);
  if (small && (rc = upload(ds, h.nodes, &ds->nodes2)) != RT_OK) return rc;
  ds->root2 = h.root;
  ds->n_nodes2 = small ? (int32_t)(h.nodes.size() / 4) : 0;
  UP(h.refs, refs);
  {
    std::vector<F4> lrecs;
    if (!h.refs8.empty()) {
      std::vector<F4> r8(4 * h.refs8.size());
      for (size_t i = 0; i < h.refs8.size(); ++i) make_record(h, h.refs8[i], &r8[4 * i]);
      UP(r8, recs8);
      UP(h.nodes8, nodes8);
    }
    build_light_records(h, lrecs);
    UP(lrecs, light_recs);
  }
  if (small) {
    const RecordPack rp = pack_records(h);
    d.brute_ng = rp.counts.ng;
    d.brute_vt[1] = rp.counts.vy;
    for (int a = 0; a < 3; ++a) d.brute_ax[a] = rp.counts.ax[a];
    d.brute_mx = rp.counts.mx;
    d.brute_box = rp.counts.box;
    ds->brute_slots = rp.n_slots;
    ds->shade_n = rp.shade_n;
    ds->brute_boxes = rp.n_boxes;
    ds->brute_shape = rp.shape;
    if ((rc = upload(ds, rp.pairs, &ds->brute_pairs)) != RT_OK) return rc;
  }
  UP(h.media, media);
  UP(h.medium_refs, medium_refs);
  {
    std::vector<F4> br(4 * h.big_refs.size());
    for (size_t i = 0; i < h.big_refs.size(); ++i) make_record(h, h.big_refs[i], &br[4 * i]);
    UP(br, big_recs);
    d.n_big = (int32_t)h.big_refs.size();
  }
  UP(h.lights, lights);
  UP(mats, mats);
  UP(h.texs, texs);
  UP(h.texels, texels);
  UP(h.images, images);
  UP(h.perlins, perlins);
#undef UP
  d.root = h.root4;
  d.n_nodes = (int32_t)(h.nodes4.size() / 8);
  d.n_media = (int32_t)h.media.size();
  d.medium_draws = h.medium_draws;
  d.n_lights = (int32_t)h.lights.size();
  d.pdf_floor = scene_pdf_floor(h);
  d.n_refs = (int32_t)h.refs.size();
  d.n_perlins = (int32_t)h.perlins.size();
  d.shade_lds = -1;
  d.shade_n = 0;
  d.merge_ok = scene_merge_ok(h);
  ds->lean_light = lean_light_of(h, &ds->light_block);
  return RT_OK;
}

template <typename T>
static int dalloc(RenderState* st, T** p, size_t count) {
  void* q = nullptr;
  HIP_OK(hipMalloc(&q, std::max<size_t>(count, 1) * sizeof(T)));
  st->allocs.push_back(q);
  *p = (T*)q;
  return RT_OK;
}

static int ensure_state(SlotState* slot, int device, uint32_t P, int depth_cap, uint32_t npix,
                        bool soa) {
  RenderState* st = slot->st;
  if (st && (st->device != device || st->P < P || st->depth_cap < depth_cap || st->npix < npix ||
             (soa && !st->ray_o))) {
    delete st;
    st = slot->st = nullptr;
  }
  if (st) return RT_OK;
  st = slot->st = new RenderState();
  st->device = device;
  st->P = P;
  st->depth_cap = depth_cap;
  st->npix = npix;
  int rc;
  if ((rc = dalloc(st, &st->stack, (size_t)P * depth_cap)) || (rc = dalloc(st, &st->ctr, 1)) ||
      (rc = dalloc(st, &st->accum, 3 * (size_t)npix)) || (rc = dalloc(st, &st->side, 3 * (size_t)npix)) ||
      (rc = dalloc(st, &st->pflags, npix)) ||
      (rc = dalloc(st, &st->out, 3 * (size_t)npix)))
    return rc;
  if (soa &&
      ((rc = dalloc(st, &st->ray_o, P)) || (rc = dalloc(st, &st->ray_d, P)) ||
       (rc = dalloc(st, &st->hit, P)) || (rc = dalloc(st, &st->pend, P)) ||
       (rc = dalloc(st, &st->pre, P)) ||
       (rc = dalloc(st, &st->path, P)) || (rc = dalloc(st, &st->queue[0], (size_t)kXcd * P)) ||
       (rc = dalloc(st, &st->queue[1], (size_t)kXcd * P))))
    return rc;
  return RT_OK;
}

template <typename T>
static int dfree(RenderState* st, T** p) {
  if (!*p) return RT_OK;
  HIP_OK(hipFree(*p));
  st->allocs.erase(std::find(st->allocs.begin(), st->allocs.end(), (void*)*p));
  *p = nullptr;
  return RT_OK;
}

static int ensure_ostack(RenderState* st, uint32_t cols) {
  if (st->ostack_cols >= cols) return RT_OK;
  int rc;
  if ((rc = dfree(st, &st->ostack))) return rc;
  if ((rc = dalloc(st, &st->ostack, (size_t)(kStack - kShortStackMin) * cols))) return rc;
  st->ostack_cols = cols;
  return RT_OK;
}

static int ensure_csum(RenderState* st, uint32_t n_chunks, bool* use_csum_io, bool keep = false) {
  int rc;
  bool use_csum = *use_csum_io;
  if (keep) {
    *use_csum_io = use_csum && st->csum && st->csum_chunks >= n_chunks;
    return RT_OK;
  }
  {
    const size_t need_b = 32 * (size_t)n_chunks;
    auto drop_csum = [&]() -> int {
      st->csum_chunks = 0;
      return dfree(st, &st->csum);
    };
    if (st->csum && (!use_csum || (st->csum_chunks > 4 * (size_t)n_chunks &&
                                   32 * st->csum_chunks > ((size_t)256 << 20))))
      if ((rc = drop_csum())) return rc;
    if (use_csum && st->csum_chunks < n_chunks) {
      if ((rc = drop_csum())) return rc;
      size_t free_b = 0, total_b = 0;
      const size_t cap_b = (size_t)std::max(0, env_int("RT_CSUM_MAX_MB", 16384)) << 20;
      if (hipMemGetInfo(&free_b, &total_b) != hipSuccess) free_b = 0;
      void* q = nullptr;
      if (need_b <= cap_b && need_b <= free_b / 2 && hipMalloc(&q, std::max<size_t>(need_b, 32)) == hipSuccess) {
        st->allocs.push_back(q);
        st->csum = (unsigned long long*)q;
        st->csum_chunks = n_chunks;
      } else {
        (void)hipGetLastError();
        use_csum = false;
      }
    }
  }
  *use_csum_io = use_csum;
  return RT_OK;
}

static int occupancy_blocks(const void* kernel, int device, int* out, size_t dyn_lds = 0) {
  int per_cu = 0, cus = 0;
  HIP_OK(hipOccupancyMaxActiveBlocksPerMultiprocessor(&per_cu, kernel, 256, dyn_lds));
  HIP_OK(hipDeviceGetAttribute(&cus, hipDeviceAttributeMultiprocessorCount, device));
  *out = std::max(1, per_cu) * std::max(1, cus);
  return RT_OK;
}

static_assert(FT_SPHERE == RT_FT_SPHERE && FT_TRI == RT_FT_TRI && FT_METAL == RT_FT_METAL &&
                  FT_DIEL == RT_FT_DIEL && FT_MEDIA == RT_FT_MEDIA && FT_CHECKER == RT_FT_CHECKER &&
                  FT_IMAGE == RT_FT_IMAGE && FT_NOISE == RT_FT_NOISE && FT_BOX == RT_FT_BOX,
              "feature bits: rt_device.h and rt_abi.h disagree");

#define RT_FUSED_EXTERN(L, F, T) extern template __global__ void k_fused<L, F, T>(Params);
RT_FUSED_ILP_KERNELS(RT_FUSED_EXTERN)
#undef RT_FUSED_EXTERN
#define RT_FUSED_EXTERN(L, F, T) extern template __global__ void k_fused<L, F, T, 0, 0, true>(Params);
RT_FUSED_MAP_KERNELS(RT_FUSED_EXTERN)
#undef RT_FUSED_EXTERN

template <bool LDS>
static const void* fused_for(uint32_t set) {
  switch (set) {
    case kFtSets[0]: return (const void*)k_fused<LDS, kFtSets[0], 4>;
    case kFtSets[1]: return (const void*)k_fused<LDS, kFtSets[1], 4>;
    case kFtSets[2]: return (const void*)k_fused<LDS, kFtSets[2], 4>;
    case kFtSets[3]: return (const void*)k_fused<LDS, kFtSets[3], 4>;
    case kFtSets[4]: return (const void*)k_fused<LDS, kFtSets[4], 4>;
    default: return (const void*)k_fused<LDS, FT_ALL, 4>;
  }
}
static uint32_t pick_set(uint32_t feats) { return pick_ft_set(feats); }
static const void* pick_fused(bool lds, uint32_t set, int tree, int shape = 0, int light = 0) {
  static_assert(kBruteShapeCount == 3, "pick_fused: one kernel per listed shape");
  static_assert(kLeanLightCount == 2, "pick_fused: one kernel per listed shape and light kind");
  if (light != 0) {
    if (!(tree == 0 && lds && set == kFtSets[0] && light == 1)) return nullptr;
    if (shape == 1) return (const void*)k_fused<true, kFtSets[0], 0, 1, 1>;
    if (shape == 2) return (const void*)k_fused<true, kFtSets[0], 0, 2, 1>;
    return nullptr;
  }
  if (tree == 0 && lds && set == kFtSets[0] && shape == 1) return (const void*)k_fused<true, kFtSets[0], 0, 1>;
  if (tree == 0 && lds && set == kFtSets[0] && shape == 2) return (const void*)k_fused<true, kFtSets[0], 0, 2>;
  if (tree == 0 && lds && set == kFtSets[0]) return (const void*)k_fused<true, kFtSets[0], 0>;
  if (tree == 0 && lds && set == kFtSets[1]) return (const void*)k_fused<true, kFtSets[1], 0>;
  if (tree == 0 && !lds && set == kFtSets[0]) return (const void*)k_fused<false, kFtSets[0], 0>;
  if (tree == 0 && !lds && set == kFtSets[1]) return (const void*)k_fused<false, kFtSets[1], 0>;
  if (tree == 2 && lds && set == kFtSets[0]) return (const void*)k_fused<true, kFtSets[0], 2>;
  if (tree == 2 && lds && set == kFtSets[1]) return (const void*)k_fused<true, kFtSets[1], 2>;
  if (tree == 8) {
#ifdef RT_BVH8_KERNELS
    if (!lds && set == kFtSets[2]) return (const void*)k_fused<false, kFtSets[2], 8>;
    if (!lds && set == kFtSets[3]) return (const void*)k_fused<false, kFtSets[3], 8>;
    if (!lds && set == kFtSets[4]) return (const void*)k_fused<false, kFtSets[4], 8>;
#endif
    return nullptr;
  }
  if (tree == 5) {
    if (lds) return nullptr;
    switch (set) {
      case kFtSets[2]: return (const void*)k_fused<false, kFtSets[2], 5>;
      case kFtSets[3]: return (const void*)k_fused<false, kFtSets[3], 5>;
      case kFtSets[4]: return (const void*)k_fused<false, kFtSets[4], 5>;
      case FT_ALL: return (const void*)k_fused<false, FT_ALL, 5>;
      default: return nullptr;
    }
  }
  if (tree != 4) return nullptr;
  return lds ? fused_for<true>(set) : fused_for<false>(set);
}

static const void* pick_fused_map(bool lds, uint32_t set, int tree) {
#define RT_FUSED_PICK(L, F, T) \
  if (lds == L && set == (F) && tree == T) return (const void*)k_fused<L, F, T, 0, 0, true>;
  RT_FUSED_MAP_KERNELS(RT_FUSED_PICK)
#undef RT_FUSED_PICK
  return nullptr;
}

struct Gather {
  float* dst;
  int dst_device;
};

static int ensure_qbvh(Scene* s, DeviceScene* ds) {
  std::lock_guard<std::mutex> lk(ds->qmu);
  if (ds->q_done) return RT_OK;
  {
    std::lock_guard<std::mutex> hk(s->qb_mu);
    if (!s->qb_built) {
      std::vector<F4> recs;
      build_leaf_records(s->h, recs);
      int rc = build_qbvh(s->h, recs, &s->qb, &s->qb_items);
      if (rc != RT_OK) return rc;
      s->qb_built = true;
    }
  }
  if (s->qb_items) {
    const int rc = upload(ds, s->qb, &ds->qnodes);
    if (rc != RT_OK) return rc;
    ds->qitems = s->qb_items;
  }
  ds->q_done = true;
  return RT_OK;
}

static size_t fused_lds_slots(uint32_t ft_set, int tr) {
  return std::min<size_t>(kLdsNodes, (160u * 1024u / (unsigned)fused_waves(ft_set, tr) -
                                      fused_static_lds(ft_set, tr) - 512u) / 64u);
}
static uint32_t scene_ft_set(const Scene* s) {
  const uint32_t feats = s->h.features;
  return (feats & FT_NOISE) && !s->h.noise_table0 ? FT_ALL : pick_set(feats);
}
static int fused_base_tree(const Scene* s, uint32_t ft_set) {
  const size_t n_refs = s->h.refs.size();
  const bool small_set = ft_set == kFtSets[0] || ft_set == kFtSets[1];
  const int env_tree = env_int("RT_TREE", -1);
  const size_t brute_max = (size_t)env_int("RT_BRUTE_MAX", kBruteMax);
  const bool fits2 = !s->h.nodes.empty() && s->h.nodes.size() / 4 + n_refs <= fused_lds_slots(ft_set, 2);
  int tree = 4;
  if (small_set && n_refs > 0 && n_refs <= brute_max) tree = 0;
  else if (small_set && n_refs <= 64 && fits2) tree = 2;
  if (small_set && (env_tree == 4 || (env_tree == 2 && fits2))) tree = env_tree;
  return tree;
}
static bool wants_qbvh(uint32_t ft_set) {
  return env_int("RT_QBVH", 1) != 0 && pick_fused(false, ft_set, 5) != nullptr;
}

struct StructurePlan {
  int tree;
  bool f_lds;
  bool f_recs;
  bool shade_tab;
  int shape;
  int light;
  const void* kernel;
  size_t lds_bytes;
  bool wants_qbvh;
};
static int plan_structure(const Scene* s, const DeviceScene* ds, uint32_t ft_set, int mode,
                          StructurePlan* out, bool no_default_bvh2 = false) {
  const size_t n_refs = s->h.refs.size();
  auto slots_for = [&](int tr) { return fused_lds_slots(ft_set, tr); };
  const int env_tree = env_int("RT_TREE", -1);
  int tree = mode == RT_MODE_FUSED ? fused_base_tree(s, ft_set) : 4;
  if (tree == 0 && !ds->brute_pairs) tree = 4;
  if (tree == 2 && !ds->nodes2) tree = 4;
  if (tree == 2 && no_default_bvh2 && env_tree != 2) tree = 4;
  const size_t lds_slots = slots_for(tree);
  const size_t brute_slots = ds->brute_slots;
  const int smem_env = env_int("RT_BRUTE_SMEM", -1);
  const bool brute_smem =
      tree == 0 && (smem_env >= 0 ? smem_env != 0 : brute_slots > lds_slots);
  const bool w4 = tree == 4;
  const size_t n_nodes = tree == 4 ? s->h.nodes4.size() / 8 : tree == 2 ? s->h.nodes.size() / 4 : 0;
  const size_t node_slots = w4 ? 2 : 1;
  const bool f_lds = node_slots * n_nodes <= lds_slots && !brute_smem;
  bool shade_tab = tree == 0 && ft_set == 0u && ds->shade_n > 0;
  if (shade_tab && f_lds && brute_slots + (size_t)(ds->shade_n + 3) / 4 > lds_slots) shade_tab = false;
  const size_t rec_slots = tree == 0 ? brute_slots + (shade_tab ? (size_t)(ds->shade_n + 3) / 4 : 0) : n_refs;
  const bool f_recs = f_lds && node_slots * n_nodes + rec_slots <= lds_slots;
  if (tree == 0 && f_lds && !f_recs)
    return set_error(RT_ERR_UNSUPPORTED, "internal: record loop in LDS without its records");
  const bool through_l2 = mode == RT_MODE_FUSED && tree == 4 && !f_lds;
  out->wants_qbvh = through_l2 && wants_qbvh(ft_set);
  if (through_l2 && !s->h.nodes8.empty() && env_tree != 4 && pick_fused(false, ft_set, 8)) tree = 8;
  const int brute_shape_id = tree == 0 && f_lds && ft_set == kFtSets[0] && env_int("RT_BRUTE_SHAPE", 1) != 0
                                 ? ds->brute_shape : 0;
  int light = tree == 0 && f_lds && ft_set == kFtSets[0] && env_int("RT_LEAN_LIGHT", 1) != 0
                  ? ds->lean_light : 0;
  if (light != 0 && !pick_fused(f_lds, ft_set, tree, brute_shape_id, light)) light = 0;
  const void* fused_kernel = pick_fused(f_lds, ft_set, tree, brute_shape_id, light);
  if (!fused_kernel) return set_error(RT_ERR_UNSUPPORTED, "internal: no fused kernel for this scene");
  const size_t fused_lds = f_lds ? 64 * (node_slots * n_nodes + (f_recs ? rec_slots : 0)) : 0;
  out->tree = tree;
  out->f_lds = f_lds;
  out->f_recs = f_recs;
  out->shade_tab = shade_tab;
  out->shape = brute_shape_id;
  out->light = light;
  out->kernel = fused_kernel;
  out->lds_bytes = fused_lds;
  return RT_OK;
}
static int take_qbvh(Scene* s, DeviceScene* ds, uint32_t ft_set, StructurePlan* sp) {
  const int rc = ensure_qbvh(s, ds);
  if (rc || !ds->qnodes) return rc;
  sp->tree = 5;
  sp->kernel = pick_fused(false, ft_set, 5);
#ifdef RT_QTOP
  sp->lds_bytes = 64 * std::min<size_t>(RT_QTOP, ds->qitems);
#endif
  return RT_OK;
}

static DevScene scene_for_tree(const DeviceScene* ds, int tree) {
  DevScene sc = ds->d;
  if (tree == 2) {
    sc.nodes = ds->nodes2;
    sc.root = ds->root2;
    sc.n_nodes = ds->n_nodes2;
  } else if (tree == 5) {
    sc.nodes = ds->qnodes;
    sc.root = 0;
    sc.n_nodes = (int32_t)std::min<size_t>(ds->qitems, 0x7FFFFFFF);
  } else if (tree == 8) {
    sc.root = 0;
  } else if (tree == 0) {
    sc.n_nodes = 0;
    sc.leafprims = ds->brute_pairs;
    sc.n_refs = (int32_t)ds->brute_slots;
  }
  return sc;
}

int aov_view(Scene* s, int device, AovView* out) {
  DeviceScene* ds = nullptr;
  int rc = ensure_scene(s, device, &ds);
  if (rc) return rc;
  const uint32_t ft_set = scene_ft_set(s);
  StructurePlan sp;
  if ((rc = plan_structure(s, ds, ft_set, RT_MODE_FUSED, &sp))) return rc;
  if (sp.tree == 8) sp.tree = 4;
  if (sp.tree == 4 && sp.wants_qbvh && (rc = take_qbvh(s, ds, ft_set, &sp))) return rc;
  out->sc = scene_for_tree(ds, sp.tree);
  out->tree = sp.tree;
  return RT_OK;
}

void set_camera_params(Params& p, const rt_camera_derived& cd, const rt_render_opts& o, uint32_t npix) {
  for (int i = 0; i < 3; ++i) {
    p.p00r[i] = (float)(cd.pixel00[i] - cd.center[i]);
    p.du[i] = (float)cd.delta_u[i];
    p.dv[i] = (float)cd.delta_v[i];
    p.cc[i] = (float)cd.center[i];
    p.dku[i] = (float)cd.defocus_u[i];
    p.dkv[i] = (float)cd.defocus_v[i];
    p.bg[i] = (float)cd.background[i];
  }
  p.recip_s = (float)cd.recip_spp_sqrt;
  p.maxc = (float)cd.max_contribution;
  p.s = cd.spp_sqrt;
  p.defocus = cd.defocus_angle > 0 ? 1 : 0;
  p.max_depth = cd.max_depth;
  p.width = cd.width;
  p.rank = o.rank;
  p.nranks = o.nranks;
  p.npix = npix;
  p.ss = (uint32_t)cd.spp_sqrt * (uint32_t)cd.spp_sqrt;
  p.seed = o.seed;
  p.fd_width = make_fastdiv((uint32_t)cd.width);
  p.fd_s = make_fastdiv((uint32_t)cd.spp_sqrt);
}
uint32_t rank_rows(uint32_t H, int rank, int nranks) {
  return H > (uint32_t)rank ? (H - (uint32_t)rank + nranks - 1) / nranks : 0;
}

struct ChunkPlan {
  uint32_t K, K2, S1;
  uint32_t cpp1;
  uint32_t n_chunks;
  uint32_t n_groups;
  FastDiv fd_gpix, fd_gchunks, fd_gchunks2;
};
static int plan_chunks(uint32_t npix, uint32_t rows, uint32_t W, uint32_t ss, uint32_t P, int chunk,
                       uint32_t ft_set, int tree, bool f_lds, int mode, ChunkPlan* out) {
  uint32_t K = 32u;
  if (chunk > 0) {
    K = (uint32_t)chunk;
  } else if (mode == RT_MODE_FUSED) {
    const bool book1_set = ft_set == (FT_SPHERE | FT_TRI | FT_METAL | FT_DIEL | FT_CHECKER);
    const int need_dflt = f_lds ? 12 : ft_set == (FT_SPHERE | FT_TRI | FT_METAL) ? 200 : book1_set ? 50 : 100;
    const uint64_t work = (uint64_t)npix * ss,
                   need = (uint64_t)std::max(1, env_int("RT_CHUNK_NEED", need_dflt)) * P;
    K = f_lds ? 8u : 4u;
    if (tree == 0 && ft_set == 0u && work / 64u >= need) {
      K = 64u;
    } else {
      for (uint32_t k : {32u, 24u, 16u, 8u})
        if ((k != 24u || book1_set) && work / k >= need) {
          K = k;
          break;
        }
    }
  }
  K = std::max<uint32_t>(1u, std::min<uint32_t>(std::min(K, ss), 4096u));
  uint32_t S1 = ss, K2 = K;
  {
    const bool one_phase = tree == 0 && ft_set == 0u;
    const bool few = mode == RT_MODE_FUSED && !one_phase &&
                     (uint64_t)npix * ss / std::max<uint32_t>(K, 1u) < 40ull * P;
    const int tf_env = env_int("RT_TAIL_FRAC", -1);
    const int tf = tf_env >= 0 ? tf_env : (few && chunk <= 0 ? 4 : 0);
    if (mode == RT_MODE_FUSED && !one_phase && tf > 1 && K >= 8u) {
      K2 = std::max<uint32_t>(1u, (uint32_t)env_int("RT_TAIL_K", (int)std::max<uint32_t>(4u, K / 4)));
      const uint32_t s1 = (uint32_t)((uint64_t)ss * (uint32_t)(tf - 1) / (uint32_t)tf) / K * K;
      if (s1 > 0 && s1 < ss && K2 < K) S1 = s1;
      else K2 = K;
    }
  }
  const uint32_t cpp1 = S1 / K + (S1 == ss && ss % K ? 1u : 0u);
  const uint32_t cpp2 = S1 < ss ? (ss - S1 + K2 - 1) / K2 : 0u;
  const uint32_t cpp = cpp1 + cpp2;
  const uint64_t n_chunks64 = (uint64_t)npix * cpp;
  if (n_chunks64 >= 0xF0000000ull) return set_error(RT_ERR_UNSUPPORTED, "too many work chunks");
  const uint32_t n_chunks = (uint32_t)n_chunks64;
  {
    const int env_rows = env_int("RT_CHUNK_ROWS", -1);
    uint32_t grows = env_rows > 0 ? (uint32_t)env_rows : 4u;
    grows = std::max<uint32_t>(1u, std::min<uint32_t>(grows, std::max<uint32_t>(rows, 1u)));
    while (rows % grows) --grows;
    const uint32_t gpix = std::max<uint32_t>(1u, grows * W);
    out->fd_gpix = make_fastdiv(gpix);
    out->fd_gchunks = make_fastdiv(gpix * cpp1);
    out->fd_gchunks2 = make_fastdiv(std::max<uint32_t>(1u, gpix * cpp2));
    out->n_groups = rows / grows;
  }
  out->K = K;
  out->K2 = K2;
  out->S1 = S1;
  out->cpp1 = cpp1;
  out->n_chunks = n_chunks;
  return RT_OK;
}

struct SchedPlan {
  int step_budget;
  uint32_t shade_min, grab_min, split_min, parts_log2, gran_log2;
};
static SchedPlan plan_sched(uint32_t ft_set, int tree, bool f_lds, uint32_t K, size_t n_nodes4) {
  SchedPlan sd;
  const bool big_tree = n_nodes4 >= 1024;
  const bool long_shade = ft_set == FT_ALL || (ft_set & FT_NOISE);
// ... 87 lines not shown
    if (slices > 1) HIP_OK(hipEventRecord(st->prog_events[sl], stream));
  }
  p.n_chunks = n_chunks;
  if (wt) {
    std::vector<unsigned long long> h(kWaveRec * n_waves);
    HIP_OK(hipMemcpyAsync(h.data(), wt, h.size() * sizeof(h[0]), hipMemcpyDeviceToHost, stream));
    HIP_OK(hipStreamSynchronize(stream));
    HIP_OK(hipFree(wt));
    p.wave_times = nullptr;
    if (FILE* f = fopen(wt_path, "wb")) {
      fwrite(h.data(), sizeof(h[0]), h.size(), f);
      fclose(f);
    }
  }
  if (ev.on) {
    HIP_OK(hipEventRecord(e1, stream));
    ev.fused.push_back({ev.used - 2, ev.used - 1});
  }
  return RT_OK;
}

static int launch_wavefront(Params& p, RenderState* st, hipStream_t stream, const void* extend_kernel,
                            ProfEvents& ev, int* iterations_out) {
  const uint32_t P = p.P, n_chunks = p.n_chunks;
  int rc, iterations = 0;
  hipLaunchKernelGGL(k_init, dim3((P + 255) / 256), dim3(256), 0, stream, p);
  HIP_OK(hipGetLastError());
  uint32_t n_est = std::min(P, n_chunks);
  const int kBatch = 4;
  while (n_est > 0) {
    for (int b = 0; b < kBatch; ++b) {
      if (iterations + 1 >= kMaxIt)
        return set_error(RT_ERR_UNSUPPORTED, "more than %d wavefront iterations", kMaxIt);
      const uint32_t ext_blocks = std::max<uint32_t>(
          1u, std::min<uint32_t>((n_est + 255) / 256, (uint32_t)st->resident_blocks));
      hipEvent_t e0 = nullptr, e1 = nullptr, e2 = nullptr;
      if (ev.on) {
        if ((rc = ev.next(&e0)) || (rc = ev.next(&e1)) || (rc = ev.next(&e2))) return rc;
        HIP_OK(hipEventRecord(e0, stream));
      }
      int it_arg = iterations;
      void* eargs[] = {&p, &it_arg};
      HIP_OK(hipLaunchKernel(extend_kernel, dim3(ext_blocks), dim3(256), eargs, 0, stream));
      if (ev.on) HIP_OK(hipEventRecord(e1, stream));
      hipLaunchKernelGGL(k_shade, dim3((n_est + 255) / 256), dim3(256), 0, stream, p,
                         iterations);
      if (ev.on) {
        HIP_OK(hipEventRecord(e2, stream));
        ev.ext.push_back({ev.used - 3, ev.used - 2});
        ev.shade.push_back({ev.used - 2, ev.used - 1});
      }
      HIP_OK(hipGetLastError());
      ++iterations;
    }
    uint32_t n_now[kXcd];
    HIP_OK(hipMemcpyAsync(n_now, &st->ctr->cnt[iterations % kMaxIt][0], sizeof n_now,
                          hipMemcpyDeviceToHost, stream));
    HIP_OK(hipStreamSynchronize(stream));
    n_est = 0;
    for (int x = 0; x < kXcd; ++x) n_est += n_now[x];
  }
  *iterations_out = iterations;
  return RT_OK;
}

static bool extend_in_lds(const Scene* s) { return s->h.nodes4.size() / 8 <= (size_t)kLdsNodes / 2; }

static int fill_stats(rt_stats* stats, const Scene* s, const DeviceScene* ds, const RenderState* st,
                      const Params& p, const StructurePlan& sp, int mode, uint32_t ft_set,
                      uint32_t rows, int iterations, const ProfEvents& ev) {
  const int tree = sp.tree;
  int rc;
  memset(stats, 0, sizeof *stats);
  Counters hc;
  HIP_OK(hipMemcpy(&hc, st->ctr, offsetof(Counters, cnt), hipMemcpyDeviceToHost));
  stats->samples = (uint64_t)p.npix * p.ss;
  stats->segments = hc.segments;
  stats->stack_pushes = hc.pushes;
  stats->overflow_samples = hc.overflow;
  stats->extend_rays = hc.segments;
  stats->shade_rays = hc.segments;
  stats->n_extend_launches = mode == RT_MODE_FUSED ? 0 : iterations;
  stats->n_shade_launches = stats->n_extend_launches;
  stats->iterations = iterations;
  stats->rows = (int32_t)rows;
  stats->mode = mode;
  stats->path_slots = (int32_t)p.P;
  stats->kernel_features = mode == RT_MODE_FUSED ? (int32_t)ft_set : (int32_t)FT_ALL;
  stats->scene_features = (int32_t)s->h.features;
  stats->tree_width = tree;
  stats->chunk_samples = (int32_t)p.K;
  stats->record_boxes = tree == 0 ? ds->brute_boxes : 0;
  stats->chunk_records = p.csum ? 1 : 0;
  stats->lds_scene = mode == RT_MODE_FUSED ? (sp.f_lds ? 1 : 0) : (extend_in_lds(s) ? 1 : 0);
  if (ev.on) {
    if ((rc = ev.sum_ms(ev.ext, &stats->ms_extend)) || (rc = ev.sum_ms(ev.shade, &stats->ms_shade)) ||
        (rc = ev.sum_ms(ev.fused, &stats->ms_fused)))
      return rc;
  }
  return RT_OK;
}


static int render_impl(rt_scene* scene, const rt_camera* cam, const rt_render_opts* opts,
                       float* out_host, float* out_dev, rt_stats* stats, int slot_id = 0,
                       const Gather* gather = nullptr, const PassSink* sink = nullptr,
                       const PixelMap* map = nullptr) {
  if (!scene || !cam) return set_error(RT_ERR_INVALID, "rt_render: null scene/camera");
  rt_render_opts o{};
  if (opts) o = *opts;
  if (o.nranks <= 0) o.nranks = 1;
  if (o.rank < 0 || o.rank >= o.nranks) return set_error(RT_ERR_INVALID, "rt_render: bad rank");
  rt_camera_derived cd;
  int rc = rt_camera_derive(cam, &cd);
  if (rc) return rc;
  auto t_start = std::chrono::steady_clock::now();
  const int32_t tuned = tune_count();

  if ((rc = device_ok("rt_render", o.device))) return rc;
  DeviceGuard dg;
  HIP_OK(hipSetDevice(o.device));
  Scene* s = &scene->s;
  DeviceScene* ds = nullptr;
  if ((rc = ensure_scene(s, o.device, &ds))) return rc;
  SlotState* slot = nullptr;
  {
    std::lock_guard<std::mutex> lk(s->mu);
    SlotState*& sl = s->slots[{o.device, slot_id}];
    if (!sl) sl = new SlotState();
    slot = sl;
  }
  std::lock_guard<std::mutex> inflight(slot->mu);

  const uint32_t W = (uint32_t)cd.width, H = (uint32_t)cd.height;
  const uint32_t rows = rank_rows(H, o.rank, o.nranks);
  const uint32_t npix_share = rows * W;
  if (map && (!map->pixels || map->n == 0 || map->n > npix_share))
    return set_error(RT_ERR_INVALID, "rt_render: a pixel map of %u of %u pixels", map->n, npix_share);
  const uint32_t npix = map ? map->n : npix_share;
  const uint32_t ss = (uint32_t)cd.spp_sqrt * (uint32_t)cd.spp_sqrt;
  int mode = o.mode;
  if (map && mode == RT_MODE_WAVEFRONT)
    return set_error(RT_ERR_UNSUPPORTED, "an active-pixel pass runs the fused kernel only (mode wavefront)");
  if (mode != RT_MODE_WAVEFRONT && mode != RT_MODE_FUSED) mode = RT_MODE_FUSED;
  const int depth_cap = cd.max_depth + 1;
  const uint32_t ft_set = scene_ft_set(s);

  StructurePlan sp;
  if ((rc = plan_structure(s, ds, ft_set, mode, &sp, map != nullptr))) return rc;
  if (sp.tree == 4 && sp.wants_qbvh && (rc = take_qbvh(s, ds, ft_set, &sp))) return rc;
  if (sp.light != 0 && !((float)cd.background[0] >= 0.0f && (float)cd.background[1] >= 0.0f &&
                         (float)cd.background[2] >= 0.0f)) {
    sp.light = 0;
    sp.kernel = pick_fused(sp.f_lds, ft_set, sp.tree, sp.shape, 0);
  }
  if (map) {
    sp.shape = sp.light = 0;
    sp.kernel = pick_fused_map(sp.f_lds, ft_set, sp.tree);
    if (!sp.kernel)
      return set_error(RT_ERR_UNSUPPORTED, "an active-pixel pass has no kernel for tree %d, chosen by RT_TREE / RT_BVH8", sp.tree);
  }
  uint32_t P = 0;
  int fused_blocks = 0;
  if (mode == RT_MODE_FUSED) {
    if ((rc = occupancy_blocks(sp.kernel, o.device, &fused_blocks, sp.lds_bytes))) return rc;
    if (o.path_slots > 0) fused_blocks = std::max(1, std::min(fused_blocks, (o.path_slots + 255) / 256));
    P = (uint32_t)fused_blocks * 256u;
  }
  ChunkPlan cp;
  if ((rc = plan_chunks(npix, map ? 1u : rows, map ? npix : W, ss, P, o.chunk, ft_set, sp.tree, sp.f_lds, mode, &cp)))
    return rc;
  const uint32_t n_chunks = cp.n_chunks;
  if (mode != RT_MODE_FUSED) {
    P = o.path_slots > 0 ? (uint32_t)o.path_slots : (1u << 20);
    P = std::max<uint32_t>(256u, std::min<uint32_t>(P, std::max<uint32_t>(n_chunks, 256u)));
    P = (P + 255u) & ~255u;
  }
  if ((rc = ensure_state(slot, o.device, P, depth_cap, std::max<uint32_t>(npix_share, 1),
                         mode == RT_MODE_WAVEFRONT)))
    return rc;
  RenderState* st = slot->st;
  const void* extend_kernel =
      extend_in_lds(s) ? (const void*)k_extend<true> : (const void*)k_extend<false>;
  if (mode == RT_MODE_WAVEFRONT && st->resident_blocks == 0 &&
      (rc = occupancy_blocks(extend_kernel, o.device, &st->resident_blocks)))
    return rc;
  if ((rc = ensure_ostack(st, mode == RT_MODE_FUSED ? P : (uint32_t)st->resident_blocks * 256u))) return rc;
  bool use_csum = mode == RT_MODE_FUSED && env_int("RT_CSUM", 1) != 0;
  if ((rc = ensure_csum(st, n_chunks, &use_csum, map != nullptr))) return rc;

  hipStream_t stream = (hipStream_t)o.stream;
  if (!stream) {
    if (!st->own_stream) HIP_OK(hipStreamCreateWithFlags(&st->own_stream, hipStreamNonBlocking));
    stream = st->own_stream;
  }

  Params p{};
  p.sc = scene_for_tree(ds, sp.tree);
  if (sp.tree == 0 && sp.shade_tab && sp.f_recs) {
    p.sc.shade_lds = (int32_t)(4 * ds->brute_slots);
    p.sc.shade_n = ds->shade_n;
  }
  set_camera_params(p, cd, o, npix);
  if (!(p.bg[0] >= 0.0f && p.bg[1] >= 0.0f && p.bg[2] >= 0.0f)) p.sc.merge_ok = 0;
  if (sp.light != 0) {
    if (!p.sc.merge_ok) return set_error(RT_ERR_UNSUPPORTED, "internal: lean light kernel without merge_ok");
    p.ll = ds->light_block;
  }
  p.pixmap = map ? map->pixels : nullptr;
  p.K = cp.K;
  p.K2 = cp.K2;
  p.S1 = cp.S1;
  p.n1 = npix * cp.cpp1;
  p.n_chunks = n_chunks;
  p.P = P;
  p.fd_gpix = cp.fd_gpix;
  p.fd_gchunks = cp.fd_gchunks;
  p.fd_gchunks2 = cp.fd_gchunks2;
#ifdef RT_SWEEP_ORDER
  p.gflip = p.gbase = 0u;
#endif
  {
    std::string v;
    if (tune_str("RT_SWEEP", &v) && v == "reverse") {
#ifdef RT_SWEEP_ORDER
      if (mode == RT_MODE_FUSED && ft_set != 0u && cp.n_groups > 1 && npix > 0) {
        p.gflip = ~0u;
        p.gbase = cp.n_groups;
      }
#else
      return set_error(RT_ERR_UNSUPPORTED, "RT_SWEEP=reverse needs a library built with -DRT_SWEEP_ORDER");
#endif
    }
  }
  const SchedPlan sd = plan_sched(ft_set, sp.tree, sp.f_lds, cp.K, s->h.nodes4.size() / 8);
  p.step_budget = sd.step_budget;
  p.shade_min = sd.shade_min;
  p.grab_min = sd.grab_min;
  p.split_min = sd.split_min;
  p.parts_log2 = sd.parts_log2;
  p.gran_log2 = sd.gran_log2;
  p.wave_times = nullptr;
  p.recs_lds = sp.f_recs ? 1u : 0u;
  p.ray_o = st->ray_o;
  p.ray_d = st->ray_d;
  p.hit = st->hit;
  p.path = st->path;
  p.pend = st->pend;
  p.pre = st->pre;

  p.stack = st->stack;
  p.queue[0] = st->queue[0];
  p.queue[1] = st->queue[1];
  p.ctr = st->ctr;
  p.accum = st->accum;
  p.csum = use_csum ? st->csum : nullptr;
  p.side = st->side;
  p.vlim = std::nextafter((float)(2147483648.0 / (double)((uint64_t)std::max<uint32_t>(ss, 1u) *
                                                          (sink ? std::max<uint32_t>(sink->max_passes, 1u) : 1u))),
                          0.0f);
  p.pflags = st->pflags;
  p.ostack = st->ostack;
  p.stack_cols = st->ostack_cols;

  F4* dtrace = nullptr;
  if (o.trace_out && o.trace_cap > 0) {
    HIP_OK(hipMalloc(&dtrace, (size_t)o.trace_cap * 3 * sizeof(F4)));
    std::vector<float> init((size_t)o.trace_cap * 12, 0.0f);
    for (int v = 0; v < o.trace_cap; ++v) init[12 * v + 7] = -1.0f;
    HIP_OK(hipMemcpy(dtrace, init.data(), init.size() * 4, hipMemcpyHostToDevice));
    p.trace = dtrace;
    p.trace_gpix = (uint32_t)o.trace_pixel;
    p.trace_sample = (uint32_t)o.trace_sample;
    p.trace_cap = o.trace_cap;
  }
  ProfEvents ev{st, (o.flags & RT_FLAG_PROFILE) != 0};

  HIP_OK(hipMemsetAsync(st->ctr, 0, sizeof(Counters), stream));
  if (npix > 0) {
    HIP_OK(hipMemsetAsync(st->accum, 0, 3 * (size_t)npix * sizeof(unsigned long long), stream));
    HIP_OK(hipMemsetAsync(st->side, 0, 3 * (size_t)npix * sizeof(double), stream));
    HIP_OK(hipMemsetAsync(st->pflags, 0, (size_t)npix * sizeof(uint32_t), stream));
  }
  int iterations = 0;
  const int slices = (mode == RT_MODE_FUSED && n_chunks > 0)
                         ? std::max(1, std::min(o.progress_slices, 1024))
                         : 1;
  if (slices > 1) p.parts_log2 = 0;
  while ((int)st->prog_events.size() < slices) {
    hipEvent_t e;
    HIP_OK(hipEventCreateWithFlags(&e, hipEventDisableTiming));
    st->prog_events.push_back(e);
  }
  ProgressDone prog_done{s->prog, slot_id == 0 && claim_progress(s->prog, (uint64_t)npix * ss, o.device)};
  if (prog_done.track && slices > 1) {
    std::lock_guard<std::mutex> lk(s->prog.mu);
    for (int sl = 0; sl < slices; ++sl) {
      s->prog.events.push_back((void*)st->prog_events[sl]);
      s->prog.cum.push_back((uint64_t)((double)s->prog.total *
                                       (double)((uint64_t)n_chunks * (sl + 1) / slices) /
                                       (double)n_chunks));
    }
  }
  if (n_chunks > 0 && mode == RT_MODE_FUSED) {
    if ((rc = launch_fused(p, st, stream, sp, fused_blocks, slices, ev))) return rc;
    iterations = 1;
  } else if (n_chunks > 0) {
    if ((rc = launch_wavefront(p, st, stream, extend_kernel, ev, &iterations))) return rc;
  }
  float* dst = out_dev ? out_dev : st->out;
  if (npix > 0 && sink) {
    if ((rc = sink->fold(sink->ctx, p, cd.pixel_samples_scale, stream))) return rc;
  } else if (npix > 0) {
    hipLaunchKernelGGL(k_resolve, dim3((npix + 255) / 256), dim3(256), 0, stream, p, dst,
                       cd.pixel_samples_scale);
    HIP_OK(hipGetLastError());
  }
  if (out_host && npix > 0)
    HIP_OK(hipMemcpyAsync(out_host, dst, 3 * (size_t)npix * sizeof(float), hipMemcpyDeviceToHost,
                          stream));
  if (gather && npix > 0)
    HIP_OK(hipMemcpyPeerAsync(gather->dst, gather->dst_device, dst, o.device,
                              3 * (size_t)npix * sizeof(float), stream));
  HIP_OK(hipStreamSynchronize(stream));
  prog_done.ok = true;
  auto t_end = std::chrono::steady_clock::now();
  if (dtrace) {
    HIP_OK(hipMemcpy(o.trace_out, dtrace, (size_t)o.trace_cap * 3 * sizeof(F4), hipMemcpyDeviceToHost));
    HIP_OK(hipFree(dtrace));
  }

  if (stats) {
    if ((rc = fill_stats(stats, s, ds, st, p, sp, mode, ft_set, rows, iterations, ev))) return rc;
    stats->ms_total = std::chrono::duration<double, std::milli>(t_end - t_start).count();
    stats->tuned = tuned;
  }
  return RT_OK;
}

int render_pass(rt_scene* scene, const rt_camera* cam, const rt_render_opts* opts, rt_stats* stats,
                const PassSink* sink, const PixelMap* map) {
  return render_impl(scene, cam, opts, nullptr, nullptr, stats, 0, nullptr, sink, map);
}

__global__ __launch_bounds__(256) void k_deinterleave(const float* gather, float* out, uint32_t H,
                                                      uint32_t W, uint32_t n, uint32_t rows_per) {
  const uint64_t i = (uint64_t)blockIdx.x * blockDim.x + threadIdx.x;
  const uint64_t row_floats = 3ull * W;
  if (i >= (uint64_t)H * row_floats) return;
  const uint32_t r = (uint32_t)(i / row_floats);
  const uint64_t x = i - (uint64_t)r * row_floats;
  out[i] = gather[((uint64_t)(r % n) * rows_per + r / n) * row_floats + x];
}

static int render_multi(rt_scene* scene, const rt_camera* cam, const rt_render_opts* opts,
                        const int32_t* devices, int32_t n, float* out_host, float* out_dev,
                        rt_stats* stats) {
  if (!scene || !cam || !devices || n <= 0)
    return set_error(RT_ERR_INVALID, "rt_render_multi: null argument or n <= 0");
  rt_render_opts o{};
// ... 76 lines not shown
        HIP_OK(hipSetDevice(devices[i]));
        HIP_OK(hipStreamCreateWithFlags(&rg->streams[i], hipStreamNonBlocking));
      }
    }
    if (rg->send_floats < share_floats) {
      for (int i = 0; i < n; ++i) {
        HIP_OK(hipSetDevice(devices[i]));
        if (rg->send[i]) HIP_OK(hipFree(rg->send[i]));
        rg->send[i] = nullptr;
        HIP_OK(hipMalloc(&rg->send[i], std::max<size_t>(share_floats, 1) * sizeof(float)));
      }
      rg->send_floats = share_floats;
    }
    HIP_OK(hipSetDevice(d0));
  }
  const bool track = claim_progress(s->prog, (uint64_t)H * W * cd.spp_sqrt * cd.spp_sqrt, d0);
  ProgressDone prog_done{s->prog, track};
  std::vector<rt_stats> st(n);
  std::vector<int> rcs(n, RT_OK);
  std::vector<std::string> errs(n);
  std::vector<std::thread> th;
  for (int i = 0; i < n; ++i)
    th.emplace_back([&, i] {
      rt_render_opts oi = o;
      oi.device = devices[i];
      oi.rank = i;
      oi.nranks = n;
      oi.progress_slices = 0;
      const Gather g = {gbuf + (size_t)i * rows_per * W * 3, d0};
      if (rg)
        rcs[i] = render_impl(scene, cam, &oi, nullptr, rg->send[i], &st[i], 1 + i, nullptr);
      else
        rcs[i] = render_impl(scene, cam, &oi, nullptr, nullptr, &st[i], 1 + i, &g);
      if (rcs[i] != RT_OK) {
        errs[i] = rt_last_error();
      } else if (track) {
        std::lock_guard<std::mutex> lk(s->prog.mu);
        s->prog.done = std::min(s->prog.total, s->prog.done + st[i].samples);
      }
    });
  for (auto& t : th) t.join();
  for (int i = 0; i < n; ++i)
    if (rcs[i] != RT_OK) return set_error(rcs[i], "rt_render_multi share %d: %s", i, errs[i].c_str());
  if (rg && share_floats > 0) {
    ncclResult_t r = ncclGroupStart();
    for (int i = 0; r == ncclSuccess && i < n; ++i) {
      HIP_OK(hipSetDevice(devices[i]));
      r = ncclGather(rg->send[i], i == 0 ? (void*)gbuf : nullptr, share_floats, ncclFloat32, 0,
                     rg->comms[i], rg->streams[i]);
    }
    const ncclResult_t r2 = ncclGroupEnd();
    if (r == ncclSuccess) r = r2;
    if (r != ncclSuccess)
      return set_error(RT_ERR_DEVICE, "rt_render_multi: ncclGather: %s", ncclGetErrorString(r));
    for (int i = 0; i < n; ++i) {
      HIP_OK(hipSetDevice(devices[i]));
      HIP_OK(hipStreamSynchronize(rg->streams[i]));
    }
  }
  HIP_OK(hipSetDevice(d0));
  if (img_floats > 0) {
    hipLaunchKernelGGL(k_deinterleave, dim3((unsigned)((img_floats + 255) / 256)), dim3(256), 0,
                       (hipStream_t)0, gbuf, img, H, W, N, rows_per);
    HIP_OK(hipGetLastError());
    if (out_host)
      HIP_OK(hipMemcpy(out_host, img, img_floats * sizeof(float), hipMemcpyDeviceToHost));
  }
  HIP_OK(hipStreamSynchronize((hipStream_t)0));
  prog_done.ok = true;
  if (stats) {
    memset(stats, 0, sizeof *stats);
    *stats = st[0];
    stats->samples = stats->segments = stats->stack_pushes = stats->overflow_samples = 0;
    stats->extend_rays = stats->shade_rays = 0;
    stats->rows = 0;
    stats->ms_fused = stats->ms_extend = stats->ms_shade = 0;
    for (int i = 0; i < n; ++i) {
      stats->samples += st[i].samples;
      stats->segments += st[i].segments;
      stats->stack_pushes += st[i].stack_pushes;
      stats->overflow_samples += st[i].overflow_samples;
      stats->extend_rays += st[i].extend_rays;
      stats->shade_rays += st[i].shade_rays;
      stats->rows += st[i].rows;
      stats->ms_fused = std::max(stats->ms_fused, st[i].ms_fused);
      stats->ms_extend = std::max(stats->ms_extend, st[i].ms_extend);
      stats->ms_shade = std::max(stats->ms_shade, st[i].ms_shade);
    }
    stats->ms_total =
        std::chrono::duration<double, std::milli>(std::chrono::steady_clock::now() - t0).count();
  }
  return RT_OK;
}

}

extern "C" {

int rt_render_multi(rt_scene* s, const rt_camera* cam, const rt_render_opts* opts,
                    const int32_t* devices, int32_t n, float* out_rgb, rt_stats* stats) {
  if (!out_rgb) return rt::set_error(RT_ERR_INVALID, "rt_render_multi: null output");
  return rt::render_multi(s, cam, opts, devices, n, out_rgb, nullptr, stats);
}

int rt_render_multi_device(rt_scene* s, const rt_camera* cam, const rt_render_opts* opts,
                           const int32_t* devices, int32_t n, float* out_rgb_device,
                           rt_stats* stats) {
  if (!out_rgb_device) return rt::set_error(RT_ERR_INVALID, "rt_render_multi_device: null output");
  return rt::render_multi(s, cam, opts, devices, n, nullptr, out_rgb_device, stats);
}


int rt_render(rt_scene* s, const rt_camera* cam, const rt_render_opts* opts, float* out_rgb,
              rt_stats* stats) {
  if (!out_rgb) return rt::set_error(RT_ERR_INVALID, "rt_render: null output");
  return rt::render_impl(s, cam, opts, out_rgb, nullptr, stats);
}

int rt_render_device(rt_scene* s, const rt_camera* cam, const rt_render_opts* opts,
                     float* out_rgb_device, rt_stats* stats) {
  if (!out_rgb_device) return rt::set_error(RT_ERR_INVALID, "rt_render_device: null output");
  return rt::render_impl(s, cam, opts, nullptr, out_rgb_device, stats);
}

int rt_progress(const rt_scene* sc, uint64_t* done, uint64_t* total) {
  if (!sc || !done || !total) return rt::set_error(RT_ERR_INVALID, "rt_progress: null");
  rt::Progress& p = const_cast<rt_scene*>(sc)->s.prog;
  std::lock_guard<std::mutex> lk(p.mu);
  *total = p.total;
  *done = p.done;
  if (!p.busy || p.events.empty()) return RT_OK;
  if (hipSetDevice(p.device) != hipSuccess) return rt::set_error(RT_ERR_DEVICE, "rt_progress");
  for (size_t i = 0; i < p.events.size(); ++i) {
    if (hipEventQuery((hipEvent_t)p.events[i]) != hipSuccess) break;
    *done = p.cum[i];
  }
  return RT_OK;
}

int rt_scene_plan_light(rt_scene* sc, int device, int32_t* kind) {
  if (!sc || !kind) return rt::set_error(RT_ERR_INVALID, "rt_scene_plan_light: null");
  int rc = rt::device_ok("rt_scene_plan_light", device);
  if (rc) return rc;
  rt::DeviceGuard dg;
  if (hipSetDevice(device) != hipSuccess) return rt::set_error(RT_ERR_DEVICE, "rt_scene_plan_light");
  rt::DeviceScene* ds = nullptr;
  if ((rc = rt::ensure_scene(&sc->s, device, &ds))) return rc;
  rt::StructurePlan sp;
  if ((rc = rt::plan_structure(&sc->s, ds, rt::scene_ft_set(&sc->s), RT_MODE_FUSED, &sp))) return rc;
  *kind = sp.light;
  return RT_OK;
}

int rt_device_count(void) {
  int n = 0;
  if (hipGetDeviceCount(&n) != hipSuccess) return 0;
  return n;
}

}
```

### include/rt_abi.h

```cpp
#ifndef RT_ABI_H
#define RT_ABI_H

#include <stddef.h>
#include <stdint.h>

#ifdef __cplusplus
extern "C" {
#endif

#define RT_ABI_VERSION 4

enum {
  RT_OK = 0,
  RT_ERR_INVALID = -1,
  RT_ERR_UNSUPPORTED = -2,
  RT_ERR_DEVICE = -3,
  RT_ERR_OOM = -4,
  RT_ERR_IO = -5
};

const char* rt_last_error(void);
int rt_abi_version(void);

int rt_tune_set(const char* name, const char* value);
// ... 70 lines not shown
  double scale_factor;
  int32_t flip_yz;
  int32_t debug;
  int32_t ignore_normals;
  int32_t center;
  int32_t flip_faces;
  int32_t default_material;
  double position[3];
  int32_t ignore_mtl;
  int32_t find_windows;
  int32_t n_images;
  int32_t _pad;
  const rt_obj_image* images;
} rt_obj_options;

typedef struct {
  int64_t n_vertices, n_normals, n_texcoords, n_triangles, n_lights;
  int32_t n_materials;
  int32_t default_material;
  double bounds_min[3], bounds_max[3], center[3];
} rt_obj_info;

int rt_obj_default_options(rt_obj_options* o);
int rt_load_obj(rt_tree* t, const char* filename, const rt_obj_options* opts, int* model,
                int* lights, rt_obj_info* info);
int rt_load_obj_memory(rt_tree* t, const char* obj_text, size_t obj_len, const char* mtl_text,
                       size_t mtl_len, const char* filename, const rt_obj_options* opts,
                       int* model, int* lights, rt_obj_info* info);

typedef struct {
  int32_t kind;
  int32_t mat;
  int32_t a, b;
  double p[10];
} rt_node;

typedef struct {
  double v[9];
  double n[9];
  double uv[6];
  int32_t flags;
  int32_t mat;
} rt_tri;

typedef struct {
  int32_t kind;
  int32_t tex;
  double albedo[3];
  double fuzz;
  double ior;
} rt_material;

typedef struct {
  int32_t kind;
  int32_t a, b;
  int32_t variant;
  double color[3];
  double scale;
} rt_texture;

typedef struct {
  int32_t w, h;
  const uint8_t* rgb;
} rt_image;

typedef struct {
  double ranvec[256][3];
  int32_t perm[3][256];
} rt_perlin;

typedef struct {
  const rt_node* nodes;
  int32_t n_nodes;
  const int32_t* children;
  int32_t n_children;
  const rt_tri* tris;
  int32_t n_tris;
  const rt_material* materials;
  int32_t n_materials;
  const rt_texture* textures;
  int32_t n_textures;
  const rt_image* images;
  int32_t n_images;
  const rt_perlin* perlins;
  int32_t n_perlins;
} rt_tree_view;

int rt_tree_get_view(const rt_tree* t, rt_tree_view* out);

typedef struct {
  double aspect_ratio;
  int32_t width;
  int32_t samples_per_pixel;
  int32_t max_depth;
  int32_t max_threads;
  double vertical_fov;
  double defocus_angle;
  double focus_distance;
  double background[3];
  double max_contribution;
  double look_from[3];
  double look_at[3];
  double vup[3];
  int32_t positioned;
  int32_t _pad;
} rt_camera;

typedef struct {
  int32_t width, height, spp_sqrt, max_depth;
  double pixel_samples_scale, recip_spp_sqrt;
  double center[3], pixel00[3], delta_u[3], delta_v[3], defocus_u[3], defocus_v[3];
  double defocus_angle, max_contribution;
  double background[3];
} rt_camera_derived;

int rt_camera_derive(const rt_camera* cam, rt_camera_derived* out);

typedef struct rt_scene rt_scene;

int rt_scene_create(const rt_tree* t, int world, int lights, rt_scene** out);
int rt_scene_destroy(rt_scene* s);

typedef struct {
  int32_t n_spheres, n_quads, n_triangles;
  int32_t n_world_prims, n_media, n_lights;
  int32_t n_bvh_nodes, bvh_depth, max_leaf;
  int32_t n_materials, n_textures, n_images, n_perlins;
  int32_t medium_draws;
  int64_t device_bytes;
  int32_t features;
  int32_t bvh_builder;
  int32_t tuned;
  int32_t _pad;
} rt_scene_info;

enum {
  RT_FT_SPHERE = 1, RT_FT_TRI = 2, RT_FT_METAL = 4, RT_FT_DIEL = 8, RT_FT_MEDIA = 16,
  RT_FT_CHECKER = 32, RT_FT_IMAGE = 64, RT_FT_NOISE = 128,
  RT_FT_BOX = 256
};
int rt_scene_info_get(const rt_scene* s, rt_scene_info* out);

int rt_scene_export_bvh(const rt_scene* s, float* nodes, int32_t* n_nodes, uint32_t* prim_refs,
                        int32_t* n_refs, uint32_t* root);
int rt_scene_export_bvh8(const rt_scene* s, float* nodes, int32_t* n_nodes, uint32_t* refs8,
                         int32_t* n_refs8);
int rt_scene_export_prim_bounds(const rt_scene* s, float* bounds, int32_t* n);
int rt_scene_export_qbvh(const rt_scene* s, float* items, int32_t* n_items, float* nodes4,
                         int32_t* n_nodes4, uint32_t* root4);
int rt_scene_export_records(const rt_scene* s, float* pairs, int32_t* n_slots, int32_t counts[7],
                            int32_t* shade_n, int32_t* n_boxes);
int rt_scene_lean_light(const rt_scene* s, int32_t* kind, float* block, int32_t* n_floats);
int rt_scene_plan_light(rt_scene* s, int device, int32_t* kind);

enum {
  RT_FLAG_PROFILE = 1,
  RT_FLAG_GATHER_RCCL = 2
};

enum { RT_MODE_AUTO = 0, RT_MODE_WAVEFRONT = 1, RT_MODE_FUSED = 2 };

typedef struct {
  uint64_t seed;
  int32_t device;
  int32_t rank;
  int32_t nranks;
  int32_t path_slots;
  int32_t chunk;
  int32_t flags;
  int32_t mode;
  void* stream;
  int64_t trace_pixel;
  int32_t trace_sample;
  int32_t trace_cap;
  float* trace_out;
  int32_t progress_slices;
  int32_t _pad3;
} rt_render_opts;

typedef struct {
  uint64_t samples;
  uint64_t segments;
  uint64_t stack_pushes;
  uint64_t extend_rays;
  uint64_t shade_rays;
  double ms_total;
  double ms_extend;
  double ms_shade;
  double ms_other;
  int32_t n_extend_launches;
  int32_t n_shade_launches;
  int32_t iterations;
  int32_t rows;
  int32_t mode;
  int32_t path_slots;
  double ms_fused;
  int32_t kernel_features;
  int32_t scene_features;
  int32_t tree_width;
  int32_t lds_scene;
  int32_t chunk_samples;
  int32_t record_boxes;
  uint64_t overflow_samples;
  int32_t tuned;
  int32_t chunk_records;
} rt_stats;

int rt_render(rt_scene* s, const rt_camera* cam, const rt_render_opts* opts, float* out_rgb,
              rt_stats* stats);
int rt_render_device(rt_scene* s, const rt_camera* cam, const rt_render_opts* opts,
                     float* out_rgb_device, rt_stats* stats);

int rt_render_multi(rt_scene* s, const rt_camera* cam, const rt_render_opts* opts,
                    const int32_t* devices, int32_t n, float* out_rgb, rt_stats* stats);
int rt_render_multi_device(rt_scene* s, const rt_camera* cam, const rt_render_opts* opts,
                           const int32_t* devices, int32_t n, float* out_rgb_device,
                           rt_stats* stats);

int rt_progress(const rt_scene* s, uint64_t* done, uint64_t* total);

int rt_quantize(const float* rgb, int64_t n_pixels, uint8_t* out);
int64_t rt_format_ppm(const float* rgb, int w, int h, char* out, int64_t cap);

int rt_quantize_device(const float* rgb_dev, int64_t n_pixels, uint8_t* out_dev, int device,
                       void* stream);
int64_t rt_format_ppm_device(const float* rgb_dev, int w, int h, char* out_dev, int64_t cap,
                             int device, void* stream);

typedef struct {
  float*   albedo;
  float*   normal;
  float*   depth;
  int32_t* material;
} rt_aov;

int rt_render_aov(rt_scene* s, const rt_camera* cam, const rt_render_opts* opts,
                  int32_t n_samples, const rt_aov* out_host, rt_stats* stats);
int rt_render_aov_device(rt_scene* s, const rt_camera* cam, const rt_render_opts* opts,
                         int32_t n_samples, const rt_aov* out_device, rt_stats* stats);

typedef struct {
  int32_t iterations;
  int32_t demodulate;
  float sigma_color;
  float sigma_normal;
  float sigma_depth;
  int32_t _pad;
} rt_denoise_opts;

int rt_denoise(const float* rgb, const rt_aov* feat, int w, int h, const rt_denoise_opts* opts,
               float* out);
int rt_denoise_device(const float* rgb_dev, const rt_aov* feat_dev, int w, int h,
                      const rt_denoise_opts* opts, float* out_dev, int device, void* stream);

typedef struct {
  int32_t iterations;
  int32_t demodulate;
  float sigma_lum;
  float sigma_normal;
  float sigma_depth;
  int32_t _pad;
} rt_denoise_var_opts;

int rt_denoise_var(const float* rgb, const float* var, const rt_aov* feat, int w, int h,
                   const rt_denoise_var_opts* opts, float* out, float* var_out);
int rt_denoise_var_device(const float* rgb_dev, const float* var_dev, const rt_aov* feat_dev,
                          int w, int h, const rt_denoise_var_opts* opts, float* out_dev,
                          float* var_out_dev, int device, void* stream);

typedef struct rt_accum rt_accum;

int rt_accum_create(rt_scene* s, const rt_camera* cam, const rt_render_opts* opts,
                    int32_t max_passes, rt_accum** out);
int rt_accum_destroy(rt_accum* a);
int rt_accum_reset(rt_accum* a);
int rt_accum_add(rt_accum* a, uint64_t seed, rt_stats* stats);
int rt_accum_resolve(rt_accum* a, float* rgb_host, float* var_host);
int rt_accum_resolve_device(rt_accum* a, float* rgb_dev, float* var_dev);

typedef struct {
  int32_t passes, max_passes;
  uint64_t samples_per_pixel;
  uint64_t nonfinite_pixels;
  double rms_std_error, mean_luminance, rel_error;
} rt_accum_info;
int rt_accum_info_get(rt_accum* a, rt_accum_info* out);

typedef struct {
  double rel_error;
  double lum_floor;
  int32_t tile;
  int32_t min_passes;
} rt_adapt_opts;

int rt_accum_select(rt_accum* a, const rt_adapt_opts* opts, uint64_t* n_active_pixels);
int rt_accum_set_active(rt_accum* a, const uint8_t* mask_host, uint64_t* n_active_pixels);
int rt_accum_add_active(rt_accum* a, uint64_t seed, rt_stats* stats);
int rt_accum_counts(rt_accum* a, int32_t* counts_host);
int rt_accum_counts_device(rt_accum* a, int32_t* counts_dev);
int rt_accum_tile_error(rt_accum* a, const rt_adapt_opts* opts, float* err_host, int32_t* tiles_x,
                        int32_t* tiles_y);

typedef struct {
  uint64_t active_pixels;
  uint64_t total_samples;
  int32_t min_count, max_count;
// ... 17 lines not shown
```

Baseline: 25530.

## Issue the per-vertex RNG draw early in the lean-light brute kernel

Adds an EARLY variant of the fused lean-light kernel for scenes with a single quad emitter in the brute record list (the Cornell box). The brute traversal stops before resolving the hit record, and shade_core decides scatter vs. emit from the raw slot index compared against a stored emitter slot. This lets the random draw start before the record and box-face resolution and the shade-table LDS loads, so their latencies can overlap, and it skips finish_hit. It adds a new kernel instantiation, host detection of the emitter slot, tune and query APIs, and relies on the emitter being uniquely identifiable by slot.

```diff
diff --git a/go_raytracer_amd/__init__.py b/go_raytracer_amd/__init__.py
--- a/go_raytracer_amd/__init__.py
+++ b/go_raytracer_amd/__init__.py
@@ -426,6 +426,16 @@
     def plan_light(self, device=0):
         k = C.c_int32()
         check(lib().rt_scene_plan_light(self._p, device, C.byref(k)))
+        return k.value
+
+    def lean_emitter(self):
+        k = C.c_int32()
+        check(lib().rt_scene_lean_emitter(self._p, C.byref(k)))
+        return k.value
+
+    def plan_early(self, device=0):
+        k = C.c_int32()
+        check(lib().rt_scene_plan_early(self._p, device, C.byref(k)))
         return k.value
 
     MODES = {"auto": 0, "wavefront": 1, "fused": 2}
diff --git a/go_raytracer_amd/_lib.py b/go_raytracer_amd/_lib.py
--- a/go_raytracer_amd/_lib.py
+++ b/go_raytracer_amd/_lib.py
@@ -218,6 +218,8 @@
     "rt_scene_export_prim_bounds": (_I, [_P, C.c_void_p, C.POINTER(C.c_int32)]),
     "rt_scene_lean_light": (_I, [_P, C.POINTER(C.c_int32), C.c_void_p, C.POINTER(C.c_int32)]),
     "rt_scene_plan_light": (_I, [_P, _I, C.POINTER(C.c_int32)]),
+    "rt_scene_lean_emitter": (_I, [_P, C.POINTER(C.c_int32)]),
+    "rt_scene_plan_early": (_I, [_P, _I, C.POINTER(C.c_int32)]),
     "rt_render": (_I, [_P, C.POINTER(RtCamera), C.POINTER(RtRenderOpts), C.c_void_p,
                        C.POINTER(RtStats)]),
     "rt_render_device": (_I, [_P, C.POINTER(RtCamera), C.POINTER(RtRenderOpts), C.c_void_p,
diff --git a/go_raytracer_amd/csrc/host_records.cpp b/go_raytracer_amd/csrc/host_records.cpp
--- a/go_raytracer_amd/csrc/host_records.cpp
+++ b/go_raytracer_amd/csrc/host_records.cpp
@@ -337,6 +337,33 @@
   return tab;
 }
 
+int32_t emitter_slot_of(const HostScene& h, const SlotOrder& so, const std::vector<char>& in_box, int shape) {
+  if (shape == 0 || lean_light_of(h, nullptr) != 1) return -1;
+  auto mat_of = [](const F4* q) {
+    uint32_t mb;
+    memcpy(&mb, &q[2].w, 4);
+    return mb;
+  };
+  long rec = -1;
+  for (size_t i = 0; i < h.refs.size(); ++i) {
+    if ((h.refs[i] >> 30) != PRIM_QUAD) return -1;
+    const uint32_t mb = mat_of(&h.quad[5 * (size_t)(h.refs[i] & 0x3FFFFFFFu)]);
+    if (mb >= h.mats.size()) return -1;
+    if (h.mats[mb].kind != RT_MAT_DIFFUSE_LIGHT) continue;
+    if (rec >= 0) return -1;
+    rec = (long)i;
+  }
+  if (rec < 0 || in_box[(size_t)rec]) return -1;
+  const F4* wq = &h.quad[5 * (size_t)(h.refs[(size_t)rec] & 0x3FFFFFFFu)];
+  const F4* lq = &h.quad[5 * (size_t)(h.lights[0].ref & 0x3FFFFFFFu)];
+  for (int k = 0; k < 3; ++k)
+    if (!(wq[k].x == lq[k].x && wq[k].y == lq[k].y && wq[k].z == lq[k].z)) return -1;
+  if (mat_of(wq) != mat_of(lq)) return -1;
+  for (size_t k = 0; k < so.n_loop; ++k)
+    if (so.slots[k] == rec) return (int32_t)k;
+  return -1;
+}
+
 }
 
 RecordPack pack_records(const HostScene& h) {
@@ -355,6 +382,7 @@
   out.n_slots = so.slots.size();
   out.n_boxes = (int32_t)boxes.size();
   out.shape = brute_shape_of(out.counts);
+  out.emitter_slot = emitter_slot_of(h, so, in_box, out.shape);
   const std::vector<F4> tab = shade_table(h);
   out.shade_n = (int32_t)tab.size();
   out.pairs.insert(out.pairs.end(), tab.begin(), tab.end());
diff --git a/go_raytracer_amd/csrc/host_tune.cpp b/go_raytracer_amd/csrc/host_tune.cpp
--- a/go_raytracer_amd/csrc/host_tune.cpp
+++ b/go_raytracer_amd/csrc/host_tune.cpp
@@ -41,6 +41,7 @@
     {"RT_BRUTE_SMEM", false, 'i', -1, 1},
     {"RT_BRUTE_SHAPE", false, 'i', 0, 1},
     {"RT_LEAN_LIGHT", false, 'i', 0, 1},
+    {"RT_LEAN_EARLY_DRAW", false, 'i', 0, 1},
     {"RT_QBVH", false, 'i', 0, 1},
     {"RT_CHUNK_NEED", false, 'i', 1, 1048576},
     {"RT_TAIL_FRAC", false, 'i', -1, 1024},
@@ -156,6 +157,12 @@
   return RT_OK;
 }
 
+int rt_scene_lean_emitter(const rt_scene* sc, int32_t* slot) {
+  if (!sc) return rt::set_error(RT_ERR_INVALID, "rt_scene_lean_emitter: null");
+  if (slot) *slot = rt::pack_records(sc->s.h).emitter_slot;
+  return RT_OK;
+}
+
 int rt_tune_list(int32_t i, const char** name, int32_t* changes_bits) {
   const int32_t n = (int32_t)(sizeof(rt::kKnobs) / sizeof(rt::kKnobs[0]));
   if (i < 0) return n;
diff --git a/go_raytracer_amd/csrc/rt_fused.h b/go_raytracer_amd/csrc/rt_fused.h
--- a/go_raytracer_amd/csrc/rt_fused.h
+++ b/go_raytracer_amd/csrc/rt_fused.h
@@ -13,14 +13,6 @@
   }
   __syncthreads();
   return recs;
-}
-
-RT_D void record_trace(const Params& P, const Path& s, const Hit& best) {
-  if (s.gpix == P.trace_gpix && s.s0 + s.j == P.trace_sample && (int)s.k < P.trace_cap) {
-    P.trace[3 * s.k + 0] = {s.o.x, s.o.y, s.o.z, s.time};
-    P.trace[3 * s.k + 1] = {s.d.x, s.d.y, s.d.z, (float)s.k};
-    P.trace[3 * s.k + 2] = {best.t, best.u, best.v, bitsf(best.ref)};
-  }
 }
 
 template <uint32_t FT>
@@ -134,8 +126,9 @@
 __shared__ unsigned long long g_tdrain[4];
 __shared__ unsigned long long g_dinfo[4][3];
 #endif
-template <bool LDS, uint32_t FT, int TREE, int SHAPE = 0, int LIGHT = 0, bool MAP = false>
+template <bool LDS, uint32_t FT, int TREE, int SHAPE = 0, int LIGHT = 0, bool MAP = false, bool EARLY = false>
 __global__ __launch_bounds__(256, fused_waves(FT, TREE)) void k_fused(Params P) {
+  static_assert(!EARLY || (SHAPE != 0 && LIGHT != 0 && !MAP), "early draw: a listed shape with a lean light kind");
   static_assert(SHAPE == 0 || (LDS && FT == 0u && TREE == 0), "shapes: the lean LDS record loop only");
   static_assert(LIGHT == 0 || (LDS && FT == 0u && TREE == 0), "light kinds: the lean LDS record loop only");
   static_assert(LIGHT >= 0 && LIGHT < kLeanLightCount, "light kinds: unlisted kind");
@@ -233,7 +226,7 @@
       PH_CNT(PH_TRAV_LANES, __popcll(__ballot(1)));
       PH_CNT(PH_TRAV_ROUNDS, 1);
       if constexpr (TREE == 0)
-        trav_brute<FT, !LDS, SHAPE>(P.sc, lnodes, s.o, s.d, s.time, 0.001f, tr);
+        trav_brute<FT, !LDS, SHAPE, EARLY>(P.sc, lnodes, s.o, s.d, s.time, 0.001f, tr);
       else if constexpr (TREE == 8)
       {
         const int nsteps = trav_steps8<FT>(P.sc, ts, s.o, s.d, s.time, 0.001f, tr, P.step_budget);
@@ -267,13 +260,13 @@
         PH_CNT(PH_SHADE_ROUNDS, 1);
         PH_T(t_media);
         Hit best = tr.best;
-        finish_hit<FT>(P, s, best);
+        if constexpr (!EARLY) finish_hit<FT>(P, s, best);
         PH_ADD(PH_MEDIA, t_media);
 #ifndef RT_WAVE_SEGS
         ++s.segs;
 #endif
         PH_T(t_shade);
-        if (shade_core<false, FT, LIGHT>(P, slot, s, best, ws, sa) == OUT_NEED_CHUNK) has = false;
+        if (shade_core<false, FT, LIGHT, EARLY ? SHAPE : 0>(P, slot, s, best, ws, sa, lnodes) == OUT_NEED_CHUNK) has = false;
         else {
           trav_init<FT>(P.sc, s.o, s.d, s.time, tr);
 #ifdef RT_QROOT
diff --git a/go_raytracer_amd/csrc/rt_internal.h b/go_raytracer_amd/csrc/rt_internal.h
--- a/go_raytracer_amd/csrc/rt_internal.h
+++ b/go_raytracer_amd/csrc/rt_internal.h
@@ -135,6 +135,7 @@
   int32_t n_boxes = 0;
   BruteCounts counts{};
   int shape = 0;
+  int32_t emitter_slot = -1;
 };
 RecordPack pack_records(const HostScene& h);
 int32_t scene_merge_ok(const HostScene& h);
diff --git a/go_raytracer_amd/csrc/rt_path.h b/go_raytracer_amd/csrc/rt_path.h
--- a/go_raytracer_amd/csrc/rt_path.h
+++ b/go_raytracer_amd/csrc/rt_path.h
@@ -1066,7 +1066,7 @@
                                                                  2 * (8 + slot));
   return ((const lds_u32*)lrec)[base + 2 * (8 + slot)];
 }
-template <uint32_t FT, bool SMEM, int SHAPE = 0>
+template <uint32_t FT, bool SMEM, int SHAPE = 0, bool EARLY = false>
 RT_D void trav_brute(const DevScene& sc, const F4* lrec, f3 o, f3 d, float time, float tmin,
                      Trav& tr) {
   static_assert(!HAS(FT_SPHERE | FT_TRI), "record loop: quad-only feature sets");
@@ -1118,6 +1118,13 @@
   const int qb = qm + (mx != 0 ? 1 : 0);
   const float iy = rcp(d.y);
   brute_box<SMEM>(sc, lrec, qb, qb + (SHAPE == 0 ? kp->sc.brute_box : bc.box), O, Dv, iy, tmin, best, bk);
+  if constexpr (EARLY) {
+    static_assert(SHAPE != 0 && !SMEM, "early draw: the listed shapes in LDS only");
+    tr.best.t = best;
+    tr.best.ref = bk;
+    tr.cur = TRAV_DONE;
+    return;
+  }
   if (bk != 0xFFFFFFFFu) {
     if (bk & kBoxCode) bk = box_face<SMEM>(sc, lrec, bk, o, d, iy, best);
     const uint32_t base = 32u * (bk >> 1) + (bk & 1u);
@@ -1141,6 +1148,32 @@
     tr.best.ref = __float_as_uint(f[9]);
   }
   tr.cur = TRAV_DONE;
+}
+template <int SHAPE>
+RT_D uint32_t brute_resolve_early(const DevScene& sc, const F4* lrec, uint32_t bk, f3 o, f3 d,
+                                  float best, uint32_t& ref_raw) {
+  constexpr BruteCounts bc = brute_shape(SHAPE);
+  const uint32_t none = (uint32_t)((int32_t)bk >> 31);
+  uint32_t slot = and_not(bk, none);
+  if constexpr (bc.box > 0) {
+    constexpr uint32_t qb = (uint32_t)(bc.ng + bc.vy + bc.ax[0] + bc.ax[1] + bc.ax[2] + (bc.mx != 0 ? 1 : 0));
+    const uint32_t box = and_not((uint32_t)((int32_t)(bk << 1) >> 31), none);
+    const uint32_t code = pick_by(kBoxCode | (qb << 2), bk, box);
+    slot = pick_by(slot, box_face<false>(sc, lrec, code, o, d, rcp(d.y), best), box);
+  }
+  ref_raw = ((const lds_u32*)lrec)[32u * (slot >> 1) + (slot & 1u) + 28u];
+  return slot;
+}
+RT_D void brute_slot_uv(const F4* lrec, uint32_t slot, f3 o, f3 d, float best, float& u, float& v) {
+  const lds_f32* l = (const lds_f32*)lrec + 32u * (slot >> 1) + (slot & 1u) + 8;
+  float f[9];
+#pragma unroll
+  for (int e = 0; e < 9; ++e) f[e] = l[2 * e];
+  const float px = fmaf(d.x, best, o.x) - f[0];
+  const float py = fmaf(d.y, best, o.y) - f[1];
+  const float pz = fmaf(d.z, best, o.z) - f[2];
+  u = fmaf(pz, f[5], fmaf(py, f[4], px * f[3]));
+  v = fmaf(pz, f[8], fmaf(py, f[7], px * f[6]));
 }
 
 template <bool LDS, uint32_t FT>
@@ -1748,13 +1781,41 @@
   store_ray<SOA>(P, slot, s);
 }
 
-template <bool SOA, uint32_t FT, int LIGHT = 0>
+RT_D void record_trace(const Params& P, const Path& s, const Hit& best) {
+  if (s.gpix == P.trace_gpix && s.s0 + s.j == P.trace_sample && (int)s.k < P.trace_cap) {
+    P.trace[3 * s.k + 0] = {s.o.x, s.o.y, s.o.z, s.time};
+    P.trace[3 * s.k + 1] = {s.d.x, s.d.y, s.d.z, (float)s.k};
+    P.trace[3 * s.k + 2] = {best.t, best.u, best.v, bitsf(best.ref)};
+  }
+}
+
+template <bool SOA, uint32_t FT, int LIGHT = 0, int EARLY_SHAPE = 0>
 RT_D int shade_core(const Params& P, uint32_t slot, Path& s, const Hit& h, const WStack& ws,
-                    const SampleAcc& sa) {
+                    const SampleAcc& sa, const F4* lrec = nullptr) {
+  static_assert(EARLY_SHAPE == 0 || (FT == 0u && LIGHT != 0 && !SOA), "early draw: the lean light kernels only");
   const DevScene& sc = P.sc;
   const f3 o = s.o, d = s.d;
   const float time = s.time;
-  const uint32_t ref = h.ref;
+  rt_u32x4 r;
+  bool scat = false;
+  uint32_t ref = h.ref;
+  F4 etab_a = {0, 0, 0, 0}, etab_b = {0, 0, 0, 0};
+  if constexpr (EARLY_SHAPE != 0) {
+    const uint32_t bk = h.ref;
+    scat = bk != 0xFFFFFFFFu && bk != fbits(kparams()->ll.f[11]);
+    r = rt_rng_draw(P.seed, s.gpix, s.s0 + s.j + (scat ? 0u : 1u),
+                    scat ? RT_STREAM(s.k, 0) : RT_STREAM_CAMERA);
+    uint32_t ref_raw;
+    const uint32_t wslot = brute_resolve_early<EARLY_SHAPE>(sc, lrec, bk, o, d, h.t, ref_raw);
+    const F4* tab = g_dyn_lds + sc.shade_lds + 2 * (ref_raw & 0x3FFFFFFFu);
+    etab_a = ld_lds(tab), etab_b = ld_lds(tab + 1);
+    ref = bk != 0xFFFFFFFFu ? ref_raw : PRIM_NONE;
+    if (P.trace) {
+      Hit th = {h.t, h.u, h.v, ref};
+      if (ref != PRIM_NONE) brute_slot_uv(lrec, wslot, o, d, h.t, th.u, th.v);
+      record_trace(P, s, th);
+    }
+  }
   f3 lterm = mk3(0, 0, 0);
   bool term = false;
   rt_u32x4 rcam;
@@ -1763,7 +1824,6 @@
   float u = h.u, v = h.v;
   bool ff = true;
   DevMaterial M;
-  bool scat = false;
   bool ltab = false;
   f3 lcol = mk3(0, 0, 0);
   float eta = 0.0f;
@@ -1801,9 +1861,9 @@
         u = phi * (0.5f * kInvPi);
         v = theta * kInvPi;
       }
-    } else if (FT == 0u && sc.shade_lds >= 0) {
+    } else if (FT == 0u && (EARLY_SHAPE != 0 || sc.shade_lds >= 0)) {
       const F4* tab = g_dyn_lds + sc.shade_lds + 2 * idx;
-      const F4 a = ld_lds(tab), b = ld_lds(tab + 1);
+      const F4 a = EARLY_SHAPE != 0 ? etab_a : ld_lds(tab), b = EARLY_SHAPE != 0 ? etab_b : ld_lds(tab + 1);
       lcol = xyz(b);
       nout = xyz(a);
 #ifndef RT_NO_LEAN_SNAP
@@ -1853,11 +1913,11 @@
       M.kind = mat;
     else
       M = sc.mats[mat];
-    scat = M.kind != RT_MAT_DIFFUSE_LIGHT;
+    if constexpr (EARLY_SHAPE == 0) scat = M.kind != RT_MAT_DIFFUSE_LIGHT;
   }
   constexpr bool kMergeDraws = FT != FT_ALL;
-  rt_u32x4 r;
-  if (kMergeDraws)
+  static_assert(EARLY_SHAPE == 0 || kMergeDraws, "early draw: the vertex's one merged draw");
+  if (kMergeDraws && EARLY_SHAPE == 0)
     r = rt_rng_draw(P.seed, s.gpix, s.s0 + s.j + (scat ? 0u : 1u),
                     scat ? RT_STREAM(s.k, 0) : RT_STREAM_CAMERA);
   if (!scat) {
diff --git a/go_raytracer_amd/csrc/rt_render.hip b/go_raytracer_amd/csrc/rt_render.hip
--- a/go_raytracer_amd/csrc/rt_render.hip
+++ b/go_raytracer_amd/csrc/rt_render.hip
@@ -158,6 +158,7 @@
   int brute_shape = 0;
   int lean_light = 0;
   LeanLight light_block{};
+  int32_t emitter_slot = -1;
   uint32_t root2 = PRIM_NONE;
   int32_t n_nodes2 = 0;
   const F4* qnodes = nullptr;
@@ -366,6 +367,7 @@
     ds->shade_n = rp.shade_n;
     ds->brute_boxes = rp.n_boxes;
     ds->brute_shape = rp.shape;
+    ds->emitter_slot = rp.emitter_slot;
     if ((rc = upload(ds, rp.pairs, &ds->brute_pairs)) != RT_OK) return rc;
   }
   UP(h.media, media);
@@ -523,15 +525,18 @@
   }
 }
 static uint32_t pick_set(uint32_t feats) { return pick_ft_set(feats); }
-static const void* pick_fused(bool lds, uint32_t set, int tree, int shape = 0, int light = 0) {
+static const void* pick_fused(bool lds, uint32_t set, int tree, int shape = 0, int light = 0,
+                              bool early = false) {
   static_assert(kBruteShapeCount == 3, "pick_fused: one kernel per listed shape");
   static_assert(kLeanLightCount == 2, "pick_fused: one kernel per listed shape and light kind");
   if (light != 0) {
     if (!(tree == 0 && lds && set == kFtSets[0] && light == 1)) return nullptr;
-    if (shape == 1) return (const void*)k_fused<true, kFtSets[0], 0, 1, 1>;
-    if (shape == 2) return (const void*)k_fused<true, kFtSets[0], 0, 2, 1>;
+    if (shape == 1) return early ? (const void*)k_fused<true, kFtSets[0], 0, 1, 1, false, true>
+                                 : (const void*)k_fused<true, kFtSets[0], 0, 1, 1>;
+    if (shape == 2) return early ? nullptr : (const void*)k_fused<true, kFtSets[0], 0, 2, 1>;
     return nullptr;
   }
+  if (early) return nullptr;
   if (tree == 0 && lds && set == kFtSets[0] && shape == 1) return (const void*)k_fused<true, kFtSets[0], 0, 1>;
   if (tree == 0 && lds && set == kFtSets[0] && shape == 2) return (const void*)k_fused<true, kFtSets[0], 0, 2>;
   if (tree == 0 && lds && set == kFtSets[0]) return (const void*)k_fused<true, kFtSets[0], 0>;
@@ -628,6 +633,7 @@
   bool shade_tab;
   int shape;
   int light;
+  bool early;
   const void* kernel;
   size_t lds_bytes;
   bool wants_qbvh;
@@ -664,7 +670,10 @@
   int light = tree == 0 && f_lds && ft_set == kFtSets[0] && env_int("RT_LEAN_LIGHT", 1) != 0
                   ? ds->lean_light : 0;
   if (light != 0 && !pick_fused(f_lds, ft_set, tree, brute_shape_id, light)) light = 0;
-  const void* fused_kernel = pick_fused(f_lds, ft_set, tree, brute_shape_id, light);
+  const bool early = light != 0 && ds->emitter_slot >= 0 && shade_tab && f_recs &&
+                     env_int("RT_LEAN_EARLY_DRAW", 1) != 0 &&
+                     pick_fused(f_lds, ft_set, tree, brute_shape_id, light, true) != nullptr;
+  const void* fused_kernel = pick_fused(f_lds, ft_set, tree, brute_shape_id, light, early);
   if (!fused_kernel) return set_error(RT_ERR_UNSUPPORTED, "internal: no fused kernel for this scene");
   const size_t fused_lds = f_lds ? 64 * (node_slots * n_nodes + (f_recs ? rec_slots : 0)) : 0;
   out->tree = tree;
@@ -673,6 +682,7 @@
   out->shade_tab = shade_tab;
   out->shape = brute_shape_id;
   out->light = light;
+  out->early = early;
   out->kernel = fused_kernel;
   out->lds_bytes = fused_lds;
   return RT_OK;
@@ -1066,10 +1076,12 @@
   if (sp.light != 0 && !((float)cd.background[0] >= 0.0f && (float)cd.background[1] >= 0.0f &&
                          (float)cd.background[2] >= 0.0f)) {
     sp.light = 0;
+    sp.early = false;
     sp.kernel = pick_fused(sp.f_lds, ft_set, sp.tree, sp.shape, 0);
   }
   if (map) {
     sp.shape = sp.light = 0;
+    sp.early = false;
     sp.kernel = pick_fused_map(sp.f_lds, ft_set, sp.tree);
     if (!sp.kernel)
       return set_error(RT_ERR_UNSUPPORTED, "an active-pixel pass has no kernel for tree %d, chosen by RT_TREE / RT_BVH8", sp.tree);
@@ -1120,6 +1132,10 @@
   if (sp.light != 0) {
     if (!p.sc.merge_ok) return set_error(RT_ERR_UNSUPPORTED, "internal: lean light kernel without merge_ok");
     p.ll = ds->light_block;
+    if (sp.early) {
+      const uint32_t es = (uint32_t)ds->emitter_slot;
+      memcpy(&p.ll.f[11], &es, 4);
+    }
   }
   p.pixmap = map ? map->pixels : nullptr;
   p.K = cp.K;
@@ -1502,6 +1518,20 @@
   return RT_OK;
 }
 
+int rt_scene_plan_early(rt_scene* sc, int device, int32_t* early) {
+  if (!sc || !early) return rt::set_error(RT_ERR_INVALID, "rt_scene_plan_early: null");
+  int rc = rt::device_ok("rt_scene_plan_early", device);
+  if (rc) return rc;
+  rt::DeviceGuard dg;
+  if (hipSetDevice(device) != hipSuccess) return rt::set_error(RT_ERR_DEVICE, "rt_scene_plan_early");
+  rt::DeviceScene* ds = nullptr;
+  if ((rc = rt::ensure_scene(&sc->s, device, &ds))) return rc;
+  rt::StructurePlan sp;
+  if ((rc = rt::plan_structure(&sc->s, ds, rt::scene_ft_set(&sc->s), RT_MODE_FUSED, &sp))) return rc;
+  *early = sp.early ? 1 : 0;
+  return RT_OK;
+}
+
 int rt_device_count(void) {
   int n = 0;
   if (hipGetDeviceCount(&n) != hipSuccess) return 0;
diff --git a/include/rt_abi.h b/include/rt_abi.h
--- a/include/rt_abi.h
+++ b/include/rt_abi.h
@@ -246,6 +246,8 @@
                             int32_t* shade_n, int32_t* n_boxes);
 int rt_scene_lean_light(const rt_scene* s, int32_t* kind, float* block, int32_t* n_floats);
 int rt_scene_plan_light(rt_scene* s, int device, int32_t* kind);
+int rt_scene_lean_emitter(const rt_scene* s, int32_t* slot);
+int rt_scene_plan_early(rt_scene* s, int device, int32_t* early);
 
 enum {
   RT_FLAG_PROFILE = 1,
```

Result: faster. 26360, median of 6 (+3.3%).
